# AshishKumar4/FlaxDiff

Measured on AMD Instinct MI355X. Metric: train images/sec/node (64x64 uncond EDM UNet, bs=256), higher is better.
Workload: dtype bf16; 1 GPU; model=unet_64px_[64,128,256,512]_res2_heads4, global_batch=256, resolution=64, parallelism=dp1, schedule=EDM + KarrasPredictionTransform(sigma_data=0.5)

## Files before the change

### flaxdiff_amd/models/common.py

```python
from __future__ import annotations

import math
from typing import Callable, Optional

import torch
import torch.nn as nn
import torch.nn.functional as F

from .. import ops


_TRUNC_STD_CORRECTION = 0.87962566103423978


def variance_scaling_(tensor: torch.Tensor, fan_in: int, fan_out: int,
                      scale: float = 1.0, mode: str = "fan_in") -> torch.Tensor:
    if mode == "fan_in":
        denom = max(1, fan_in)
    elif mode == "fan_out":
        denom = max(1, fan_out)
    else:
        denom = max(1.0, (fan_in + fan_out) / 2)
    std = math.sqrt(max(scale, 1e-10) / denom) / _TRUNC_STD_CORRECTION
    with torch.no_grad():
        tensor.normal_(0.0, std)
        tensor.clamp_(-2 * std, 2 * std)
    return tensor


class _ShadowCast(torch.autograd.Function):

    @staticmethod
    def forward(ctx, p):
        return p._shadow_bf16

    @staticmethod
    def backward(ctx, dy):
        return dy.float()


def _cast(p: Optional[torch.Tensor], dtype) -> Optional[torch.Tensor]:
    if p is None:
        return None
    if p.dtype == dtype:
        return p
    if dtype == torch.bfloat16 and getattr(p, "_shadow_bf16", None) is not None:
        return _ShadowCast.apply(p)
    return p.to(dtype)



class Dense(nn.Module):
    def __init__(self, in_features: int, out_features: int, use_bias: bool = True,
                 kernel_scale: float = 1.0, zero_init: bool = False):
        super().__init__()
        self.in_features = in_features
        self.out_features = out_features
        w = torch.empty(in_features, out_features)
        if zero_init:
            nn.init.zeros_(w)
        else:
            variance_scaling_(w, in_features, out_features, scale=kernel_scale)
        self.weight = nn.Parameter(w)
        self.bias = nn.Parameter(torch.zeros(out_features)) if use_bias else None

    def forward(self, x: torch.Tensor, add: torch.Tensor = None) -> torch.Tensor:
        if x.is_cuda and x.dtype == torch.bfloat16:
            return ops.dense(x, self.weight, self.bias, add=add)
        return ops.dense(x, _cast(self.weight, x.dtype),
                         _cast(self.bias, x.dtype), add=add)



class GroupNorm(nn.Module):

    def __init__(self, num_groups: int, num_channels: int, eps: float = 1e-5):
        super().__init__()
        assert num_channels % num_groups == 0, (num_groups, num_channels)
        self.num_groups = num_groups
        self.eps = eps
        self.weight = nn.Parameter(torch.ones(num_channels))
        self.bias = nn.Parameter(torch.zeros(num_channels))

    def forward(self, x: torch.Tensor, silu: bool = False) -> torch.Tensor:
        if x.is_cuda:
            return ops.group_norm(x, self.num_groups, self.weight, self.bias,
                                  self.eps, silu)
        return ops.group_norm(x, self.num_groups, _cast(self.weight, x.dtype),
                              _cast(self.bias, x.dtype), self.eps, silu)

    def forward_fork(self, x: torch.Tensor, silu: bool = False):
        if x.is_cuda:
            return ops.group_norm_fork(x, self.num_groups, self.weight,
                                       self.bias, self.eps, silu)
        return self.forward(x, silu), x


class RMSNorm(nn.Module):
    def __init__(self, dim: int, eps: float = 1e-5):
        super().__init__()
        self.eps = eps
        self.weight = nn.Parameter(torch.ones(dim))

    def forward(self, x: torch.Tensor) -> torch.Tensor:
        if x.is_cuda:
            return ops.rms_norm(x, self.weight, self.eps)
        return ops.rms_norm(x, _cast(self.weight, x.dtype), self.eps)



class TimeEmbedding(nn.Module):

    def __init__(self, features: int, max_positions: int = 10000):
        super().__init__()
        self.features = features
        self.max_positions = max_positions

    def forward(self, t: torch.Tensor) -> torch.Tensor:
        return ops.sinusoidal_time_embedding(t, self.features, self.max_positions)


class FourierEmbedding(nn.Module):

    def __init__(self, features: int, scale: float = 16.0):
        super().__init__()
        g = torch.Generator().manual_seed(42)
        freqs = torch.randn(features // 2, generator=g) * scale
        self.register_buffer("freqs", freqs, persistent=True)

    def forward(self, t: torch.Tensor) -> torch.Tensor:
        return ops.fourier_time_embedding(t, self.freqs)


class TimeProjection(nn.Module):

    def __init__(self, in_features: int, features: int):
        super().__init__()
        self.dense1 = Dense(in_features, features)
        self.dense2 = Dense(features, features)

    def forward(self, x: torch.Tensor) -> torch.Tensor:
        x = F.gelu(self.dense1(x))
        x = F.gelu(self.dense2(x))
        return x



class Conv(nn.Module):

    def __init__(self, in_features: int, features: int, kernel_size=(3, 3),
                 strides=(1, 1), use_bias: bool = True):
        super().__init__()
        kh, kw = kernel_size if isinstance(kernel_size, (tuple, list)) \
            else (kernel_size, kernel_size)
        self.stride = strides[0] if isinstance(strides, (tuple, list)) else strides
        w = torch.empty(kh, kw, in_features, features)
        variance_scaling_(w, kh * kw * in_features, kh * kw * features)
        self.weight = nn.Parameter(w)
        self.bias = nn.Parameter(torch.zeros(features)) if use_bias else None

    def forward(self, x: torch.Tensor, add: torch.Tensor = None,
                badd: torch.Tensor = None) -> torch.Tensor:
        if x.is_cuda and x.dtype == torch.bfloat16:
            return ops.conv2d(x, self.weight, self.bias, stride=self.stride,
                              add=add, badd=badd)
        return ops.conv2d(x, _cast(self.weight, x.dtype), _cast(self.bias, x.dtype),
                          stride=self.stride, add=add, badd=badd)


class ConvTranspose(nn.Module):
    def __init__(self, in_features: int, features: int, kernel_size=(3, 3), strides=(2, 2)):
        super().__init__()
        kh, kw = kernel_size
        self.stride = strides[0]
        w = torch.empty(kh, kw, in_features, features)
        variance_scaling_(w, kh * kw * in_features, kh * kw * features)
        self.weight = nn.Parameter(w)
        self.bias = nn.Parameter(torch.zeros(features))

    def forward(self, x):
        return ops.conv2d_transpose(x, _cast(self.weight, x.dtype),
                                    _cast(self.bias, x.dtype), stride=self.stride)


class SeparableConv(nn.Module):

    def __init__(self, in_features: int, features: int, kernel_size=(3, 3),
                 strides=(1, 1), use_bias: bool = False):
        super().__init__()
        kh, kw = kernel_size
        self.stride = strides[0] if isinstance(strides, (tuple, list)) else strides
        dw = torch.empty(kh, kw, in_features, 1)
        variance_scaling_(dw, kh * kw, kh * kw)
        self.depthwise = nn.Parameter(dw)
        pw = torch.empty(1, 1, in_features, features)
        variance_scaling_(pw, in_features, features)
        self.pointwise = nn.Parameter(pw)
        self.bias = nn.Parameter(torch.zeros(features)) if use_bias else None

    def forward(self, x):
        x = ops.depthwise_conv2d(x, _cast(self.depthwise, x.dtype), None, self.stride)
        return ops.conv2d(x, _cast(self.pointwise, x.dtype), _cast(self.bias, x.dtype), 1)


class WeightStandardizedConv(nn.Module):

    def __init__(self, in_features: int, features: int, kernel_size=(3, 3), strides=(1, 1)):
        super().__init__()
        kh, kw = kernel_size
        self.stride = strides[0] if isinstance(strides, (tuple, list)) else strides
        w = torch.empty(kh, kw, in_features, features)
        variance_scaling_(w, kh * kw * in_features, kh * kw * features)
        self.weight = nn.Parameter(w)
        self.bias = nn.Parameter(torch.zeros(features))

    def forward(self, x):
        w = self.weight
        eps = 1e-5 if x.dtype == torch.float32 else 1e-3
        mean = w.mean(dim=(0, 1, 2), keepdim=True)
        var = w.var(dim=(0, 1, 2), unbiased=False, keepdim=True)
        w = (w - mean) / torch.sqrt(var + eps)
        return ops.conv2d(x, _cast(w, x.dtype), _cast(self.bias, x.dtype), self.stride)


def ConvLayer(conv_type: str, in_features: int, features: int, kernel_size=(3, 3),
              strides=(1, 1)) -> nn.Module:
    if conv_type == "conv":
        return Conv(in_features, features, kernel_size, strides)
    if conv_type == "w_conv":
        return WeightStandardizedConv(in_features, features, kernel_size, strides)
    if conv_type == "separable":
        return SeparableConv(in_features, features, kernel_size, strides)
    if conv_type == "conv_transpose":
        return ConvTranspose(in_features, features, kernel_size, strides)
    raise ValueError(f"unknown conv_type {conv_type}")


class PixelShuffle(nn.Module):

    def __init__(self, scale: int):
        super().__init__()
        self.scale = scale

    def forward(self, x):
        B, H, W, C = x.shape
        s = self.scale
        c = C // (s * s)
        x = x.reshape(B, H, W, s, s, c)
        x = x.permute(0, 1, 3, 2, 4, 5)
        return x.reshape(B, H * s, W * s, c)


class Upsample(nn.Module):

    def __init__(self, in_features: int, features: int, scale: int = 2,
                 activation: Callable = F.silu):
        super().__init__()
        assert scale == 2
        self.conv = Conv(in_features, features, (3, 3), (1, 1))

    def forward(self, x, residual=None):
        if x.is_cuda and x.dtype == torch.bfloat16:
            out = ops.conv2d_upsample2x(x, self.conv.weight, self.conv.bias)
        else:
            out = self.conv(ops.nearest_upsample_2x(x))
        if residual is not None:
            out = ops.cat_channels(out, residual)
        return out


class Downsample(nn.Module):

    def __init__(self, in_features: int, features: int, scale: int = 2,
                 activation: Callable = F.silu):
        super().__init__()
        assert scale == 2
        self.conv = Conv(in_features, features, (3, 3), (2, 2))

    def forward(self, x, residual=None):
        out = self.conv(x)
        if residual is not None:
            if residual.shape[1] > out.shape[1]:
                residual = ops.avg_pool_2x(residual)
            out = ops.cat_channels(out, residual)
        return out



class ResidualBlock(nn.Module):

    def __init__(self, conv_type: str, in_features: int, features: int,
                 temb_features: int, kernel_size=(3, 3), strides=(1, 1),
                 activation: Callable = F.silu, norm_groups: int = 8,
                 norm_epsilon: float = 1e-4):
        super().__init__()
        self.features = features
        self.activation = activation
        self._fused_silu = activation in (F.silu, torch.nn.functional.silu)
        if norm_groups > 0:
            self.norm1 = GroupNorm(norm_groups, in_features, eps=norm_epsilon)
            self.norm2 = GroupNorm(norm_groups, features, eps=norm_epsilon)
        else:
            self.norm1 = RMSNorm(in_features, eps=norm_epsilon)
            self.norm2 = RMSNorm(features, eps=norm_epsilon)
        self.conv1 = ConvLayer(conv_type, in_features, features, kernel_size, strides)
        self.temb_projection = Dense(temb_features, features)
        self.conv2 = ConvLayer(conv_type, features, features, kernel_size, strides)
        self.residual_conv = (ConvLayer(conv_type, in_features, features, (1, 1), (1, 1))
                              if in_features != features else None)

    def _norm_act(self, norm, x):
        if isinstance(norm, GroupNorm) and self._fused_silu:
            return norm(x, silu=True)
        return self.activation(norm(x))

    def forward(self, x: torch.Tensor, temb: torch.Tensor,
                textemb: torch.Tensor = None, extra_features: torch.Tensor = None):
        if isinstance(self.norm1, GroupNorm):
            out, residual = self.norm1.forward_fork(x, silu=self._fused_silu)
            if not self._fused_silu:
                out = self.activation(out)
        else:
            residual = x
            out = self._norm_act(self.norm1, x)
        t = self.temb_projection(temb.to(out.dtype))
        if isinstance(self.conv1, Conv):
            out = self.conv1(out, badd=t)
        else:
            out = self.conv1(out) + t[:, None, None, :]

        out = self._norm_act(self.norm2, out)
        if self.residual_conv is not None:
            residual = self.residual_conv(residual)
        if isinstance(self.conv2, Conv) and residual.shape[-1] == self.features:
            out = self.conv2(out, add=residual)
        else:
            out = self.conv2(out) + residual

        if extra_features is not None:
            out = ops.cat_channels(out, extra_features)
        return out


def l2norm(t: torch.Tensor, dim=1, eps=1e-6):
    return t / torch.clamp(t.norm(p=2, dim=dim, keepdim=True), min=eps)
```

### flaxdiff_amd/models/unet.py

```python
from __future__ import annotations

from typing import Callable, List, Optional, Sequence

import torch
import torch.nn as nn
import torch.nn.functional as F

from .. import ops
from .attention import TransformerBlock
from .common import (ConvLayer, Downsample, FourierEmbedding, GroupNorm,
                     RMSNorm, ResidualBlock, TimeProjection, Upsample)


def _make_attention(dim: int, attention_config: dict, context_dim: int,
                    default_fp32_softmax: bool = False) -> TransformerBlock:
    heads = attention_config["heads"]
    return TransformerBlock(
        in_channels=dim,
        heads=heads,
        dim_head=dim // heads,
        use_projection=attention_config.get("use_projection", False),
        use_self_and_cross=attention_config.get("use_self_and_cross", True),
        only_pure_attention=attention_config.get("only_pure_attention", True),
        force_fp32_for_softmax=attention_config.get("force_fp32_for_softmax",
                                                    default_fp32_softmax),
        norm_inputs=attention_config.get("norm_inputs", True),
        explicitly_add_residual=attention_config.get("explicitly_add_residual", True),
        context_dim=context_dim,
    )


class Unet(nn.Module):
    def __init__(self,
                 output_channels: int = 3,
                 in_channels: int = 3,
                 emb_features: int = 64 * 4,
                 feature_depths: Sequence[int] = (64, 128, 256, 512),
                 attention_configs: Sequence[Optional[dict]] = ({"heads": 8},) * 4,
                 num_res_blocks: int = 2,
                 num_middle_res_blocks: int = 1,
                 activation: Callable = F.silu,
                 norm_groups: int = 8,
                 context_dim: int = 768,
                 conv_type: str = "conv"):
        super().__init__()
        self.output_channels = output_channels
        self.emb_features = emb_features
        self.feature_depths = list(feature_depths)
        self.attention_configs = list(attention_configs)
        self.num_res_blocks = num_res_blocks
        self.num_middle_res_blocks = num_middle_res_blocks
        self.activation = activation
        self.norm_groups = norm_groups

        self.time_embed = FourierEmbedding(features=emb_features)
        self.time_proj = TimeProjection(emb_features, emb_features)

        f0 = self.feature_depths[0]
        self.conv_in = ConvLayer(conv_type, in_channels, f0, (3, 3), (1, 1))

        def res_block(cin, cout):
            return ResidualBlock(conv_type, cin, cout, emb_features,
                                 kernel_size=(3, 3), strides=(1, 1),
                                 activation=activation, norm_groups=norm_groups)

        ch = f0
        skip_channels: List[int] = [f0]
        self.down_blocks = nn.ModuleList()
        for i, (dim_out, att_cfg) in enumerate(zip(self.feature_depths, self.attention_configs)):
            dim_in = ch
            level = nn.ModuleDict()
            res_list = nn.ModuleList()
            attn_list = nn.ModuleList()
            for j in range(num_res_blocks):
                res_list.append(res_block(dim_in, dim_in))
                if att_cfg is not None and j == num_res_blocks - 1:
                    attn_list.append(_make_attention(dim_in, att_cfg, context_dim))
                else:
                    attn_list.append(nn.Identity())
                skip_channels.append(dim_in)
            level["res"] = res_list
            level["attn"] = attn_list
            if i != len(self.feature_depths) - 1:
                level["down"] = Downsample(dim_in, dim_out, scale=2, activation=activation)
                ch = dim_out
            self.down_blocks.append(level)

        middle_dim = self.feature_depths[-1]
        middle_att = self.attention_configs[-1]
        self.middle_res1 = nn.ModuleList()
        self.middle_attn = nn.ModuleList()
        self.middle_res2 = nn.ModuleList()
        for j in range(num_middle_res_blocks):
            self.middle_res1.append(res_block(ch, middle_dim))
            ch = middle_dim
            if middle_att is not None and j == num_middle_res_blocks - 1:
                cfg = dict(middle_att)
                cfg.setdefault("use_self_and_cross", False)
                self.middle_attn.append(_make_attention(middle_dim, cfg, context_dim))
            else:
                self.middle_attn.append(nn.Identity())
            self.middle_res2.append(res_block(middle_dim, middle_dim))

        self.up_blocks = nn.ModuleList()
        rev_depths = list(reversed(self.feature_depths))
        rev_attn = list(reversed(self.attention_configs))
        skips = list(skip_channels)
        for i, (dim_out, att_cfg) in enumerate(zip(rev_depths, rev_attn)):
            level = nn.ModuleDict()
            res_list = nn.ModuleList()
            attn_list = nn.ModuleList()
            for j in range(num_res_blocks):
                skip_ch = skips.pop()
                res_list.append(res_block(ch + skip_ch, dim_out))
                ch = dim_out
                if att_cfg is not None and j == num_res_blocks - 1:
                    attn_list.append(_make_attention(dim_out, att_cfg, context_dim))
                else:
                    attn_list.append(nn.Identity())
            level["res"] = res_list
            level["attn"] = attn_list
            if i != len(self.feature_depths) - 1:
                up_features = self.feature_depths[-i] if i > 0 else self.feature_depths[0]
                level["up"] = Upsample(ch, up_features, scale=2, activation=activation)
                ch = up_features
            self.up_blocks.append(level)

        self.conv_mid = ConvLayer(conv_type, ch, f0, (3, 3), (1, 1))
        final_skip = skips.pop()
        assert not skips
        self.final_residual = res_block(f0 + final_skip, f0)
        if norm_groups > 0:
            self.conv_out_norm = GroupNorm(norm_groups, f0, eps=1e-5)
        else:
            self.conv_out_norm = RMSNorm(f0, eps=1e-5)
        self.conv_out = ConvLayer(conv_type, f0, output_channels, (3, 3), (1, 1))

    def forward(self, x: torch.Tensor, temb: torch.Tensor,
                textcontext: torch.Tensor) -> torch.Tensor:
        temb = self.time_embed(temb).to(x.dtype)
        temb = self.time_proj(temb)

        x = self.conv_in(x)
        downs = [x]

        for level in self.down_blocks:
            for res, attn in zip(level["res"], level["attn"]):
                x = res(x, temb)
                if not isinstance(attn, nn.Identity):
                    x = attn(x, textcontext)
                downs.append(x)
            if "down" in level:
                x = level["down"](x)

        for res1, attn, res2 in zip(self.middle_res1, self.middle_attn, self.middle_res2):
            x = res1(x, temb)
            if not isinstance(attn, nn.Identity):
                x = attn(x, textcontext)
            x = res2(x, temb)

        for level in self.up_blocks:
            for res, attn in zip(level["res"], level["attn"]):
                x = ops.cat_channels(x, downs.pop())
                x = res(x, temb)
                if not isinstance(attn, nn.Identity):
                    x = attn(x, textcontext)
            if "up" in level:
                x = level["up"](x)

        x = self.conv_mid(x)
        x = ops.cat_channels(x, downs.pop())
        x = self.final_residual(x, temb)

        if isinstance(self.conv_out_norm, GroupNorm):
            x = self.conv_out_norm(x, silu=True)
        else:
            x = self.activation(self.conv_out_norm(x))
        return self.conv_out(x)
```

### flaxdiff_amd/ops/__init__.py

```python
from __future__ import annotations

import os
import weakref
from typing import Optional

import torch

from . import reference

_EXT = None
_EXT_ERR: Optional[str] = None


def _load_ext():
    global _EXT, _EXT_ERR
    if _EXT is not None or _EXT_ERR is not None:
        return _EXT
    try:
        from .hip import build as hip_build
        _EXT = hip_build.load_extension()
    except Exception as e:
        _EXT_ERR = f"{type(e).__name__}: {e}"
        _EXT = None
    return _EXT


def hip_available() -> bool:
    return _load_ext() is not None


def _require_ext():
    ext = _load_ext()
    if ext is None:
        raise RuntimeError(
            "flaxdiff_amd HIP extension is not available on a GPU tensor path "
            f"(build error: {_EXT_ERR}). Run __graft_entry__.build() / "
            "python -m flaxdiff_amd.ops.hip.build first — the GPU path never "
            "silently falls back to stock torch ops.")
    return ext


_FORCE_TORCH = os.environ.get("FLAXDIFF_FORCE_TORCH_OPS", "0") == "1"
_GEMM_LIB = os.environ.get("FD_GEMM_LIB", "0") == "1"


def _use_hip(x: torch.Tensor) -> bool:
    return x.is_cuda and not _FORCE_TORCH



_GRAD_HOOK_OWNERS: "weakref.WeakSet" = weakref.WeakSet()


def register_grad_hook_owner(owner) -> None:
    _GRAD_HOOK_OWNERS.add(owner)


def _sink_kinds() -> str:
    v = os.environ.get("FD_GRAD_SINK", "1")
    if v == "0":
        return ""
    return "wbgr" if v == "all" else "bgr"


def grad_sinks_active() -> bool:
    if not _sink_kinds():
        return False
    return not any(o.hooks_live for o in _GRAD_HOOK_OWNERS)


def _grad_sink(p: Optional[torch.Tensor], kind: str) -> Optional[torch.Tensor]:
    if p is None or kind not in _sink_kinds():
        return None
    sink = getattr(p, "_grad_sink", None)
    if sink is None or sink.dtype != torch.float32 or not grad_sinks_active():
        return None
    owner = getattr(p, "_grad_sink_owner", None)
    g = (p if owner is None else owner).grad
    if g is None or g.data_ptr() != sink.data_ptr() \
            or g.numel() != sink.numel() or not sink.is_contiguous():
        return None
    return sink



def _gn_save(ctx, x, gamma, beta, mean, rstd, groups, silu):
    ctx.save_for_backward(x, gamma, mean, rstd)
    ctx.groups = groups
    ctx.silu = silu
    ctx.beta = beta
    ctx.gamma_param = gamma


def _gn_backward(ctx, dy, add):
    x, gamma, mean, rstd = ctx.saved_tensors
    ext = _require_ext()
    has_beta = ctx.beta is not None
    beta = ctx.beta if has_beta else torch.zeros_like(gamma)
    if has_beta and ctx.needs_input_grad[1] and ctx.needs_input_grad[2]:
        sg, sb = _grad_sink(ctx.gamma_param, "g"), _grad_sink(ctx.beta, "g")
        if sg is not None and sb is not None:
            (dx,) = ext.gn_silu_bwd(dy.contiguous(), x, gamma, beta, mean,
                                    rstd, ctx.groups, ctx.silu, sg, sb, add)
            return dx, None, None
    dx, dgamma, dbeta = ext.gn_silu_bwd(dy.contiguous(), x, gamma, beta, mean,
                                        rstd, ctx.groups, ctx.silu,
                                        None, None, add)
    return dx, dgamma, (dbeta if has_beta else None)


class _GroupNormSiLUFn(torch.autograd.Function):
    @staticmethod
    def forward(ctx, x, gamma, beta, groups, eps, silu):
        ext = _require_ext()
        y, mean, rstd = ext.gn_silu_fwd(x, gamma, beta, groups, eps, silu)
        _gn_save(ctx, x, gamma, beta, mean, rstd, groups, silu)
        return y

    @staticmethod
    def backward(ctx, dy):
        return (*_gn_backward(ctx, dy, None), None, None, None)


def group_norm(x: torch.Tensor, groups: int, gamma: torch.Tensor,
               beta: torch.Tensor, eps: float = 1e-5, silu: bool = False) -> torch.Tensor:
    if _use_hip(x):
        return _GroupNormSiLUFn.apply(x.contiguous(), gamma, beta, groups, eps, silu)
    return reference.group_norm_nhwc(x, groups, gamma, beta, eps, silu)


class _GroupNormForkFn(torch.autograd.Function):

    @staticmethod
    def forward(ctx, x, gamma, beta, groups, eps, silu):
        ext = _require_ext()
        ctx.set_materialize_grads(False)
        y, mean, rstd = ext.gn_silu_fwd(x, gamma, beta, groups, eps, silu)
        _gn_save(ctx, x, gamma, beta, mean, rstd, groups, silu)
        return y, x

    @staticmethod
    def backward(ctx, dy, dx_pass):
        if dy is None:
            return dx_pass, None, None, None, None, None
        add = None
        if dx_pass is not None:
            add = dx_pass.to(ctx.saved_tensors[0].dtype).contiguous()
        return (*_gn_backward(ctx, dy, add), None, None, None)


def group_norm_fork_enabled() -> bool:
    return os.environ.get("FD_GN_FORK_ADD", "1") != "0"


def group_norm_fork(x: torch.Tensor, groups: int, gamma: torch.Tensor,
                    beta: torch.Tensor, eps: float = 1e-5, silu: bool = False):
    if _use_hip(x) and beta is not None and group_norm_fork_enabled():
        return _GroupNormForkFn.apply(x.contiguous(), gamma, beta, groups, eps, silu)
    return group_norm(x, groups, gamma, beta, eps, silu), x



class _RMSNormFn(torch.autograd.Function):
    @staticmethod
    def forward(ctx, x, gamma, eps):
        ext = _require_ext()
        y, rrms = ext.rms_norm_fwd(x, gamma, eps)
        ctx.save_for_backward(x, gamma, rrms)
        ctx.gamma_param = gamma
        return y

    @staticmethod
    def backward(ctx, dy):
        x, gamma, rrms = ctx.saved_tensors
        ext = _require_ext()
        sink = _grad_sink(ctx.gamma_param, "r") if ctx.needs_input_grad[1] else None
        if sink is not None:
            (dx,) = ext.rms_norm_bwd(dy.contiguous(), x, gamma, rrms, sink)
            return dx, None, None
        dx, dgamma = ext.rms_norm_bwd(dy.contiguous(), x, gamma, rrms)
        return dx, dgamma, None


def rms_norm(x: torch.Tensor, gamma: torch.Tensor, eps: float = 1e-5) -> torch.Tensor:
    if _use_hip(x):
        return _RMSNormFn.apply(x.contiguous(), gamma, eps)
    return reference.rms_norm(x, gamma, eps)



def _kernel_view(p: torch.Tensor) -> torch.Tensor:
    if p.dtype == torch.bfloat16:
        return p
    sh = getattr(p, "_shadow_bf16", None)
    if sh is not None:
        return sh
    return p.to(torch.bfloat16)


def _kernel_view_t(p: torch.Tensor) -> torch.Tensor:
    t = getattr(p, "_shadow_bf16_t", None)
    if t is not None:
        return t
    return _kernel_view(p).t().contiguous()


def transpose_shadows(src_flat, dst_flat, tiles):
    _require_ext().transpose_shadows(src_flat, dst_flat, tiles)


def _routable_param(p: Optional[torch.Tensor]) -> bool:
    return p is None or p.dtype == torch.bfloat16 or \
        getattr(p, "_shadow_bf16", None) is not None


def _save_params(ctx, w, b):
    ctx.has_bias = b is not None
    ctx.w_dtype = w.dtype
    ctx.b_dtype = b.dtype if b is not None else None
    ctx.w_param, ctx.b_param = w, b


def _param_grads(ctx, ext, dy, x, kh, kw, stride):
    dw = db = None
    b_param = ctx.b_param if ctx.has_bias and ctx.needs_input_grad[2] \
        else None
    if ctx.needs_input_grad[1]:
        dw, db = _wgrad(ext, dy, x, kh, kw, stride,
                        ctx.w_param, ctx.w_dtype, b_param, ctx.b_dtype)
    elif ctx.has_bias:
        db = _bias_grad(dy, b_param, ctx.b_dtype)
    return dw, db


class _Conv2dFn(torch.autograd.Function):
    @staticmethod
    def forward(ctx, x, w, b, stride, add, badd):
        ext = _require_ext()
        wk = _kernel_view(w)
        y = ext.conv2d_fwd(x, wk, b if b is not None else torch.Tensor(),
                           stride,
                           add if add is not None else torch.Tensor(),
                           badd if badd is not None else torch.Tensor())
        ctx.save_for_backward(x, wk)
        ctx.stride = stride
        ctx.has_add = add is not None
        ctx.has_badd = badd is not None
        _save_params(ctx, w, b)
        return y

    @staticmethod
    def backward(ctx, dy):
        x, wk = ctx.saved_tensors
        ext = _require_ext()
        dy = dy.contiguous()
        dx = ext.conv2d_dgrad(dy, wk, ctx.stride, x.shape[1], x.shape[2]) \
            if ctx.needs_input_grad[0] else None
        dw, db = _param_grads(ctx, ext, dy, x, wk.shape[0], wk.shape[1],
                              ctx.stride)
        dadd = dy if ctx.has_add else None
        dbadd = None
        if ctx.has_badd:
            B = dy.shape[0]
            dbadd = dy.reshape(B, -1, dy.shape[-1]).sum(1)
        return dx, dw, db, None, dadd, dbadd


class _DenseFn(torch.autograd.Function):

    @staticmethod
    def forward(ctx, x2d, w2d, b, add):
        wk = _kernel_view(w2d)
        if not _GEMM_LIB and x2d.shape[1] % 64 == 0:
            ext = _require_ext()
            bf = b if b is not None else torch.Tensor()
            if bf.numel() and bf.dtype != torch.float32:
                bf = bf.float()
            y = ext.gemm_nt(x2d, _kernel_view_t(w2d), bf,
                            add if add is not None else torch.Tensor())
        else:
            y = torch.matmul(x2d, wk)
            if b is not None:
                y = y + _kernel_view(b)
            if add is not None:
                y = y + add
        ctx.save_for_backward(x2d, wk)
        ctx.has_add = add is not None
        _save_params(ctx, w2d, b)
        return y

    @staticmethod
    def backward(ctx, dy):
        x2d, wk = ctx.saved_tensors
        dy = dy.contiguous()
        ext = _require_ext()
        if ctx.needs_input_grad[0]:
            if not _GEMM_LIB and dy.shape[1] % 64 == 0:
                dx = ext.gemm_dx(dy, wk)
            else:
                dx = torch.matmul(dy, wk.t())
        else:
            dx = None
        M = x2d.shape[0]
        dw, db = _param_grads(ctx, ext, dy.view(M, 1, 1, dy.shape[1]),
                              x2d.view(M, 1, 1, x2d.shape[1]), 1, 1, 1)
        if dw is not None:
            dw = dw.view(x2d.shape[1], dy.shape[1])
        dadd = dy if ctx.has_add else None
        return dx, dw, db, dadd


def dense(x: torch.Tensor, w: torch.Tensor, b: Optional[torch.Tensor] = None,
          add: Optional[torch.Tensor] = None) -> torch.Tensor:
    if _use_hip(x) and x.dtype == torch.bfloat16 and _routable_param(w) \
            and _routable_param(b):
        lead = x.shape[:-1]
        add2 = None
        if add is not None and add.dtype == torch.bfloat16:
            add2 = add.reshape(-1, w.shape[1]).contiguous()
        y = _DenseFn.apply(x.reshape(-1, x.shape[-1]).contiguous(), w, b, add2)
        y = y.reshape(*lead, w.shape[1])
        if add is not None and add2 is None:
            y = y + add
        return y
    if w.dtype != x.dtype:
        w = w.to(x.dtype)
    y = torch.matmul(x, w)
    if b is not None:
        y = y + b.to(y.dtype)
    if add is not None:
        y = y + add.to(y.dtype)
    return y


class _WL2LossFn(torch.autograd.Function):

    @staticmethod
    def forward(ctx, pred, target, wb):
        ctx.save_for_backward(pred, target, wb)
        return _require_ext().wl2_loss_fwd(pred, target, wb)

    @staticmethod
    def backward(ctx, go):
        pred, target, wb = ctx.saved_tensors
        dpred = _require_ext().wl2_loss_bwd(pred, target, wb,
                                            go.reshape(1).float())
        return dpred, None, None


def weighted_l2_loss(pred: torch.Tensor, target: torch.Tensor,
                     weights: torch.Tensor) -> torch.Tensor:
    if _use_hip(pred) and pred.dtype == torch.bfloat16 \
            and target.dtype == torch.bfloat16:
        wb = weights.reshape(weights.shape[0]).float().contiguous()
        return _WL2LossFn.apply(pred.contiguous(), target.contiguous(), wb)
    return (0.5 * (pred.float() - target.float()) ** 2
            * weights.to(torch.float32)).mean()


class _ConvUp2xFn(torch.autograd.Function):

    @staticmethod
    def forward(ctx, x, w, b):
        ext = _require_ext()
        wk = _kernel_view(w)
        y = ext.conv2d_fwd_up2x(x, wk, b if b is not None else torch.Tensor())
        if y is None or y.numel() == 0:
            raise _ConvUpIneligibleError
        ctx.save_for_backward(x, wk)
        _save_params(ctx, w, b)
        return y

    @staticmethod
    def backward(ctx, dy):
        x, wk = ctx.saved_tensors
        ext = _require_ext()
        dy = dy.contiguous()
        H2, W2 = x.shape[1] * 2, x.shape[2] * 2
        dx = None
        if ctx.needs_input_grad[0]:
            dx_up = ext.conv2d_dgrad(dy, wk, 1, H2, W2)
            dx = ext.upsample2x_bwd(dx_up)
        x_up = ext.upsample2x_fwd(x) if ctx.needs_input_grad[1] else None
        dw, db = _param_grads(ctx, ext, dy, x_up, 3, 3, 1)
        return dx, dw, db


class _ConvUpIneligibleError(Exception):
    pass


def conv2d_upsample2x(x: torch.Tensor, w: torch.Tensor,
                      b: Optional[torch.Tensor] = None) -> torch.Tensor:
    if _use_hip(x) and x.dtype == torch.bfloat16 and _routable_param(w) \
            and w.shape[0] == 3 and w.shape[1] == 3:
        try:
            return _ConvUp2xFn.apply(
                x.contiguous(), w.contiguous(),
                b.contiguous() if b is not None else None)
        except _ConvUpIneligibleError:
            pass
    return conv2d(nearest_upsample_2x(x), w, b, stride=1)


class _GEGLUFn(torch.autograd.Function):

    @staticmethod
    def forward(ctx, h):
        ctx.save_for_backward(h)
        return _require_ext().geglu_fwd(h)

    @staticmethod
    def backward(ctx, dy):
        (h,) = ctx.saved_tensors
        return _require_ext().geglu_bwd(dy.contiguous(), h)


def geglu(h: torch.Tensor) -> torch.Tensor:
    if _use_hip(h) and h.dtype == torch.bfloat16 and h.shape[-1] % 16 == 0:
        return _GEGLUFn.apply(h.contiguous())
    a, b = h.chunk(2, dim=-1)
    return a * torch.nn.functional.gelu(b)


class _Cat2Fn(torch.autograd.Function):

    @staticmethod
    def forward(ctx, a, b):
        ctx.ca = a.shape[-1]
        ctx.cb = b.shape[-1]
        return _require_ext().cat2_lastdim(a, b)

    @staticmethod
    def backward(ctx, dy):
        da, db = _require_ext().split2_lastdim(dy.contiguous(), ctx.ca, ctx.cb)
        return da, db


def cat_channels(a: torch.Tensor, b: torch.Tensor) -> torch.Tensor:
    if _use_hip(a) and a.dtype == torch.bfloat16 and b.dtype == torch.bfloat16 \
            and (a.shape[-1] + b.shape[-1]) % 8 == 0:
        return _Cat2Fn.apply(a.contiguous(), b.contiguous())
    return torch.cat([a, b], dim=-1)


def _wgrad(ext, dy, x, kh, kw, stride, w_param, w_dtype,
           b_param=None, b_dtype=None):
    want_db = b_dtype is not None
    w_sink = _grad_sink(w_param, "w") if w_dtype == torch.float32 else None
    b_sink = _grad_sink(b_param, "b") if b_dtype == torch.float32 else None
    dw, db, folded = ext.conv2d_wgrad(dy, x, kh, kw, stride, w_sink,
                                      want_db, b_sink)
    if dw is not None and w_dtype != torch.float32:
        dw = dw.to(w_dtype)
    if want_db and not folded:
        db = _bias_grad(dy, b_param, b_dtype)
    elif db is not None and b_dtype != torch.float32:
        db = db.to(b_dtype)
    return dw, db


def _bias_grad(dy: torch.Tensor, b_param: Optional[torch.Tensor] = None,
               b_dtype=torch.float32) -> Optional[torch.Tensor]:
    d2 = dy.reshape(-1, dy.shape[-1])
    C = d2.shape[1]
    if d2.is_cuda and d2.dtype == torch.bfloat16 and C % 8 == 0 and C <= 2048:
        sink = _grad_sink(b_param, "b") if b_dtype == torch.float32 else None
        db = _require_ext().colsum(d2.contiguous(), sink)
        if sink is not None:
            return None
    else:
        db = d2.float().sum(0)
    return db if b_dtype == torch.float32 else db.to(b_dtype)


def conv2d(x: torch.Tensor, w: torch.Tensor, b: Optional[torch.Tensor] = None,
           stride: int = 1, add: Optional[torch.Tensor] = None,
           badd: Optional[torch.Tensor] = None) -> torch.Tensor:
    kh, kw = w.shape[0], w.shape[1]
    if kh == 1 and kw == 1 and stride == 1:
        w2 = w.reshape(w.shape[2], w.shape[3])
        sh = getattr(w, "_shadow_bf16", None)
        if sh is not None and w.dtype != torch.bfloat16:
            w2._shadow_bf16 = sh.reshape(w.shape[2], w.shape[3])
            sht = getattr(w, "_shadow_bf16_t", None)
            if sht is not None:
                w2._shadow_bf16_t = sht
            sink = getattr(w, "_grad_sink", None)
            if sink is not None:
                w2._grad_sink = sink.reshape(w.shape[2], w.shape[3])
                w2._grad_sink_owner = w
        y = dense(x.reshape(-1, w.shape[2]), w2, b)
        y = y.reshape(*x.shape[:-1], w.shape[3])
        if badd is not None:
            y = y + badd[:, None, None, :].to(y.dtype)
        return y if add is None else y + add
    if _use_hip(x) and x.dtype == torch.bfloat16 and _routable_param(w):
        if add is not None and add.dtype != torch.bfloat16:
            add_in, add_out = None, add
        else:
            add_in, add_out = add, None
        if badd is not None and badd.dtype != torch.bfloat16:
            badd_in, badd_out = None, badd
        else:
            badd_in, badd_out = badd, None
        out = _Conv2dFn.apply(
            x.contiguous(), w.contiguous(),
            b.contiguous() if b is not None else None, stride,
            add_in.contiguous() if add_in is not None else None,
            badd_in.contiguous() if badd_in is not None else None)
        if badd_out is not None:
            out = out + badd_out[:, None, None, :].to(out.dtype)
        if add_out is not None:
            out = out + add_out
        return out
    if w.dtype != x.dtype:
        w = w.to(x.dtype)
    if b is not None and b.dtype != x.dtype:
        b = b.to(x.dtype)
    y = reference.conv2d_nhwc(x, w, b, stride=stride, padding="same")
    if badd is not None:
        y = y + badd[:, None, None, :].to(y.dtype)
    return y if add is None else y + add


class _ConvTransposeFn(torch.autograd.Function):

    @staticmethod
    def forward(ctx, x, wf, stride):
        ext = _require_ext()
        H2 = x.shape[1] * stride
        W2 = x.shape[2] * stride
        y = ext.conv2d_dgrad(x, wf, stride, H2, W2)
        ctx.save_for_backward(x, wf)
        ctx.stride = stride
        return y

    @staticmethod
    def backward(ctx, dout):
        x, wf = ctx.saved_tensors
        ext = _require_ext()
        dout = dout.contiguous()
        dx = ext.conv2d_fwd(dout, wf, torch.Tensor(), ctx.stride,
                            torch.Tensor(), torch.Tensor()) \
            if ctx.needs_input_grad[0] else None
        dwf = None
        if ctx.needs_input_grad[1]:
            dwf = ext.conv2d_wgrad(x, dout, wf.shape[0], wf.shape[1],
                                   ctx.stride)[0].to(wf.dtype)
        return dx, dwf, None


def conv2d_transpose(x: torch.Tensor, w: torch.Tensor, b: Optional[torch.Tensor] = None,
                     stride: int = 2) -> torch.Tensor:
    kh, kw = w.shape[0], w.shape[1]
    if _use_hip(x) and stride == 2 and kh == 3 and kw == 3:
        wf = w.permute(0, 1, 3, 2).contiguous()
        out = _ConvTransposeFn.apply(x.contiguous(), wf, stride)
        if b is not None:
            out = out + b
        return out
    return reference.conv2d_transpose_nhwc(x, w, b, stride)


class _DepthwiseConvFn(torch.autograd.Function):

    @staticmethod
    def forward(ctx, x, w, stride, dilation):
        ext = _require_ext()
        y = ext.dwconv_fwd(x, w, None, stride, dilation)
        ctx.save_for_backward(x, w)
        ctx.stride = stride
        ctx.dilation = dilation
        return y

    @staticmethod
    def backward(ctx, dy):
        x, w = ctx.saved_tensors
        ext = _require_ext()
        dy = dy.contiguous()
        dx = ext.dwconv_dgrad(dy, w, x.shape[1], x.shape[2],
                              ctx.stride, ctx.dilation)
        dw = ext.dwconv_wgrad(dy, x, ctx.stride, ctx.dilation)
        return dx, dw.to(w.dtype), None, None


def depthwise_conv2d(x: torch.Tensor, w: torch.Tensor, b: Optional[torch.Tensor] = None,
                     stride: int = 1, dilation: int = 1) -> torch.Tensor:
    if (_use_hip(x) and x.dtype == torch.bfloat16 and b is None
            and w.shape[0] == 3 and w.shape[1] == 3 and x.shape[-1] % 8 == 0):
        w3 = w.reshape(3, 3, -1).contiguous()
        return _DepthwiseConvFn.apply(x, w3, stride, dilation)
    return reference.depthwise_conv2d_nhwc(x, w, b, stride, dilation)



def _attn_view_ok(t: torch.Tensor) -> bool:
    if t.dim() != 4:
        return False
    if t.is_contiguous():
        return True
    if t.stride(3) != 1 or t.data_ptr() % 16 or t.stride(2) >= 2 ** 31:
        return False
    return all(st > 0 and st % 8 == 0 for st in t.stride()[:3])


def _attn_strided(q: torch.Tensor, k: torch.Tensor) -> bool:
    if os.environ.get("FD_ATTN_STRIDED", "1") == "0":
        return False
    if os.environ.get("FD_ATTN_BWD_V1"):
        return False
    return k.shape[2] <= 128 and q.shape[3] <= 64


def _attn_operand(t: torch.Tensor, strided: bool) -> torch.Tensor:
    return t if strided and _attn_view_ok(t) else t.contiguous()


class _AttentionFn(torch.autograd.Function):
    @staticmethod
    def forward(ctx, q, k, v, scale):
        ext = _require_ext()
        o, lse = ext.attn_fwd(q, k, v, scale)
        ctx.save_for_backward(q, k, v, lse)
        ctx.scale = scale
        return o

    @staticmethod
    def backward(ctx, do):
        q, k, v, lse = ctx.saved_tensors
        scale = ctx.scale
        use_v1 = os.environ.get("FD_ATTN_BWD_V1")
        dmax = 32 if use_v1 else 64
        if k.shape[2] <= 128 and q.shape[3] <= dmax:
            ext = _require_ext()
            fn = ext.attn_bwd_smallkv if use_v1 else ext.attn_bwd_smallkv_v2
            do = _attn_operand(do, not use_v1 and _attn_strided(q, k))
            dq, dk, dv = fn(q, k, v, do, lse, scale)
            return dq, dk, dv, None
        qf, kf, vf, dof = q.float(), k.float(), v.float(), do.float()
        s = torch.einsum("bhqd,bhkd->bhqk", qf, kf) * scale
        p = torch.exp(s - lse.unsqueeze(-1))
        dv = torch.einsum("bhqk,bhqd->bhkd", p, dof)
        dp = torch.einsum("bhqd,bhkd->bhqk", dof, vf)
        dsum = (dp * p).sum(-1, keepdim=True)
        ds = (dp - dsum) * p * scale
        dq = torch.einsum("bhqk,bhkd->bhqd", ds, kf)
        dk = torch.einsum("bhqk,bhqd->bhkd", ds, qf)
        return dq.to(q.dtype), dk.to(k.dtype), dv.to(v.dtype), None


def attention(q: torch.Tensor, k: torch.Tensor, v: torch.Tensor,
              scale: Optional[float] = None) -> torch.Tensor:
    if scale is None:
        scale = q.shape[-1] ** -0.5
    if _use_hip(q):
        D = q.shape[-1]
        if D % 8 == 0 and D <= 128:
            strided = _attn_strided(q, k)
            return _AttentionFn.apply(_attn_operand(q, strided),
                                      _attn_operand(k, strided),
                                      _attn_operand(v, strided), scale)
    return reference.attention(q, k, v, scale)



def forward_diffusion(x0, eps, signal_rate, noise_rate):
    if _use_hip(x0):
        ext = _require_ext()
        return ext.fwd_diffusion(x0, eps, signal_rate.reshape(-1).float().contiguous(),
                                 noise_rate.reshape(-1).float().contiguous())
    return reference.forward_diffusion(x0, eps, signal_rate, noise_rate)


def nearest_upsample_2x(x: torch.Tensor) -> torch.Tensor:
    if _use_hip(x):
        return _Upsample2xFn.apply(x.contiguous())
    return reference.nearest_upsample_2x_nhwc(x)


class _Upsample2xFn(torch.autograd.Function):
    @staticmethod
    def forward(ctx, x):
        ext = _require_ext()
        return ext.upsample2x_fwd(x)

    @staticmethod
    def backward(ctx, dy):
        ext = _require_ext()
        return ext.upsample2x_bwd(dy.contiguous())


def avg_pool_2x(x: torch.Tensor) -> torch.Tensor:
    return reference.avg_pool_2x_nhwc(x)


def sinusoidal_time_embedding(t: torch.Tensor, features: int,
                              max_positions: int = 10000) -> torch.Tensor:
    if _use_hip(t):
        ext = _require_ext()
        return ext.time_embed(t, torch.Tensor(), features, float(max_positions))
    return reference.sinusoidal_time_embedding(t, features, max_positions)


def fourier_time_embedding(t: torch.Tensor, freqs: torch.Tensor) -> torch.Tensor:
    if _use_hip(t):
        ext = _require_ext()
        return ext.time_embed(t, freqs, freqs.numel() * 2, 0.0)
    return reference.fourier_time_embedding(t, freqs)



class _S5ScanFn(torch.autograd.Function):

    @staticmethod
    def forward(ctx, a_ri, bu_ri):
        ext = _require_ext()
        x = ext.s5_scan_fwd(a_ri.contiguous(), bu_ri.contiguous())
        ctx.save_for_backward(a_ri, x)
        return x

    @staticmethod
    def backward(ctx, dx):
        a_ri, x = ctx.saved_tensors
        ext = _require_ext()
        dbu, dap = ext.s5_scan_bwd(a_ri.contiguous(), x, dx.contiguous())
        return dap.sum(dim=0), dbu


def s5_scan(a: torch.Tensor, bu: torch.Tensor) -> torch.Tensor:
    if bu.is_cuda and not _FORCE_TORCH:
        a_ri = torch.view_as_real(a.contiguous()).float()
        bu_ri = torch.view_as_real(bu.contiguous()).float()
        x = _S5ScanFn.apply(a_ri, bu_ri)
        return torch.view_as_complex(x)
    from ..models.ssm_dit import associative_scan_diag
    return associative_scan_diag(a.reshape(1, 1, -1).expand_as(bu), bu)


def fused_adamw_ema(params_f32, grads, exp_avg, exp_avg_sq, ema_f32, params_bf16,
                    *, lr, beta1, beta2, eps, weight_decay, step, ema_decay,
                    grad_scale: float = 1.0, scale_dev=None, skip_ctr=None,
                    step_dev=None):
    ext = _require_ext()
    ext.fused_adamw_ema(params_f32, grads, exp_avg, exp_avg_sq, ema_f32,
                        params_bf16 if params_bf16 is not None else torch.Tensor(),
                        lr, beta1, beta2, eps, weight_decay, step, ema_decay,
                        grad_scale, scale_dev, skip_ctr, step_dev)
```

### flaxdiff_amd/ops/hip/bindings.cpp

```cpp
#include <torch/extension.h>
#include <tuple>
#include <vector>

std::vector<torch::Tensor> gn_silu_fwd(torch::Tensor x, torch::Tensor gamma,
                                       torch::Tensor beta, long groups,
                                       double eps, bool silu);
std::vector<torch::Tensor> gn_silu_bwd(torch::Tensor dy, torch::Tensor x,
                                       torch::Tensor gamma, torch::Tensor beta,
                                       torch::Tensor mean, torch::Tensor rstd,
                                       long groups, bool silu,
                                       c10::optional<torch::Tensor> dgamma_sink,
                                       c10::optional<torch::Tensor> dbeta_sink,
                                       c10::optional<torch::Tensor> add);
std::vector<torch::Tensor> rms_norm_fwd(torch::Tensor x, torch::Tensor gamma,
                                        double eps);
std::vector<torch::Tensor> rms_norm_bwd(torch::Tensor dy, torch::Tensor x,
                                        torch::Tensor gamma, torch::Tensor rrms,
                                        c10::optional<torch::Tensor> dgamma_sink);
torch::Tensor conv2d_fwd(torch::Tensor x, torch::Tensor w, torch::Tensor bias,
                         long stride, torch::Tensor add, torch::Tensor badd);
torch::Tensor conv2d_fwd_up2x(torch::Tensor x, torch::Tensor w,
                              torch::Tensor bias);
torch::Tensor conv2d_dgrad(torch::Tensor dy, torch::Tensor w, long stride,
                           long H, long W);
std::tuple<torch::Tensor, torch::Tensor, bool>
conv2d_wgrad(torch::Tensor dy, torch::Tensor x, long kh, long kw, long stride,
             c10::optional<torch::Tensor> dw_sink, bool want_db,
             c10::optional<torch::Tensor> db_sink);
torch::Tensor dwconv_fwd(torch::Tensor x, torch::Tensor w,
                         c10::optional<torch::Tensor> bias,
                         int64_t stride, int64_t dilation);
torch::Tensor dwconv_dgrad(torch::Tensor dy, torch::Tensor w,
                           int64_t H, int64_t W, int64_t stride, int64_t dilation);
torch::Tensor dwconv_wgrad(torch::Tensor dy, torch::Tensor x,
                           int64_t stride, int64_t dilation);
std::vector<torch::Tensor> attn_fwd(torch::Tensor q, torch::Tensor k,
                                    torch::Tensor v, double scale);
std::vector<torch::Tensor> attn_bwd_smallkv(torch::Tensor q, torch::Tensor k,
                                            torch::Tensor v, torch::Tensor dout,
                                            torch::Tensor lse, double scale);
std::vector<torch::Tensor> attn_bwd_smallkv_v2(torch::Tensor q, torch::Tensor k,
                                               torch::Tensor v, torch::Tensor dout,
                                               torch::Tensor lse, double scale);
torch::Tensor fwd_diffusion(torch::Tensor x0, torch::Tensor eps,
                            torch::Tensor a, torch::Tensor s);
torch::Tensor upsample2x_fwd(torch::Tensor x);
torch::Tensor time_embed(torch::Tensor t, torch::Tensor freqs, long features,
                         double max_positions);
torch::Tensor upsample2x_bwd(torch::Tensor dy);
torch::Tensor colsum(torch::Tensor x, c10::optional<torch::Tensor> sink);
torch::Tensor cat2_lastdim(torch::Tensor a, torch::Tensor b);
std::vector<torch::Tensor> split2_lastdim(torch::Tensor dy, long Ca, long Cb);
torch::Tensor geglu_fwd(torch::Tensor h);
torch::Tensor geglu_bwd(torch::Tensor dy, torch::Tensor h);
torch::Tensor wl2_loss_fwd(torch::Tensor pred, torch::Tensor target,
                           torch::Tensor wb);
torch::Tensor wl2_loss_bwd(torch::Tensor pred, torch::Tensor target,
                           torch::Tensor wb, torch::Tensor go);
torch::Tensor s5_scan_fwd(torch::Tensor a, torch::Tensor bu);
std::vector<torch::Tensor> s5_scan_bwd(torch::Tensor a, torch::Tensor x,
                                       torch::Tensor dx);
torch::Tensor gemm_fwd(torch::Tensor x, torch::Tensor w, torch::Tensor bias);
torch::Tensor gemm_dx(torch::Tensor dy, torch::Tensor w);
torch::Tensor gemm_nt(torch::Tensor x, torch::Tensor wt, torch::Tensor bias,
                      torch::Tensor add);
void transpose_shadows(torch::Tensor src_flat, torch::Tensor dst_flat,
                       torch::Tensor tiles);
void fused_adamw_ema(torch::Tensor p, torch::Tensor g, torch::Tensor m,
                     torch::Tensor v, torch::Tensor ema, torch::Tensor p_bf16,
                     double lr, double beta1, double beta2, double eps,
                     double weight_decay, long step, double ema_decay,
                     double grad_scale,
                     c10::optional<torch::Tensor> scale_dev,
                     c10::optional<torch::Tensor> skip_ctr,
                     c10::optional<torch::Tensor> step_dev);

PYBIND11_MODULE(TORCH_EXTENSION_NAME, m) {
    m.def("gn_silu_fwd", &gn_silu_fwd, "fused GroupNorm+SiLU forward (NHWC)");
    m.def("gn_silu_bwd", &gn_silu_bwd, "fused GroupNorm+SiLU backward",
          py::arg("dy"), py::arg("x"), py::arg("gamma"), py::arg("beta"),
          py::arg("mean"), py::arg("rstd"), py::arg("groups"), py::arg("silu"),
          py::arg("dgamma_sink") = py::none(), py::arg("dbeta_sink") = py::none(),
          py::arg("add") = py::none());
    m.def("rms_norm_fwd", &rms_norm_fwd, "RMSNorm forward");
    m.def("rms_norm_bwd", &rms_norm_bwd, "RMSNorm backward",
          py::arg("dy"), py::arg("x"), py::arg("gamma"), py::arg("rrms"),
          py::arg("dgamma_sink") = py::none());
    m.def("conv2d_fwd", &conv2d_fwd, "implicit-GEMM NHWC conv forward");
    m.def("conv2d_fwd_up2x", &conv2d_fwd_up2x, "fused nearest-2x upsample + conv forward");
    m.def("conv2d_dgrad", &conv2d_dgrad, "implicit-GEMM NHWC conv dgrad");
    m.def("conv2d_wgrad", &conv2d_wgrad,
          "split-M NHWC conv wgrad (+ folded bias grad): (dw, db, folded)",
          py::arg("dy"), py::arg("x"), py::arg("kh"), py::arg("kw"),
          py::arg("stride"), py::arg("dw_sink") = py::none(),
          py::arg("want_db") = false, py::arg("db_sink") = py::none());
    m.def("dwconv_fwd", &dwconv_fwd, "3x3 depthwise NHWC conv forward");
    m.def("dwconv_dgrad", &dwconv_dgrad, "3x3 depthwise NHWC conv dgrad");
    m.def("dwconv_wgrad", &dwconv_wgrad, "3x3 depthwise NHWC conv wgrad (fp32)");
    m.def("attn_fwd", &attn_fwd, "flash attention forward (bf16, fp32 softmax)");
    m.def("attn_bwd_smallkv", &attn_bwd_smallkv,
          "fused attention backward for Skv<=128, D<=32");
    m.def("attn_bwd_smallkv_v2", &attn_bwd_smallkv_v2,
          "vectorized-LDS attention backward for Skv<=128, D<=64");
    m.def("fwd_diffusion", &fwd_diffusion, "forward-diffusion axpy");
    m.def("upsample2x_fwd", &upsample2x_fwd, "nearest 2x upsample");
    m.def("time_embed", &time_embed, "fused sinusoidal/Fourier time embedding");
    m.def("upsample2x_bwd", &upsample2x_bwd, "nearest 2x upsample backward");
    m.def("colsum", &colsum, "coalesced column sum (bias grads)",
          py::arg("x"), py::arg("sink") = py::none());
    m.def("cat2_lastdim", &cat2_lastdim, "fused last-dim 2-tensor concat");
    m.def("split2_lastdim", &split2_lastdim, "one-pass last-dim split (cat backward)");
    m.def("geglu_fwd", &geglu_fwd, "fused GEGLU forward");
    m.def("geglu_bwd", &geglu_bwd, "fused GEGLU backward");
    m.def("wl2_loss_fwd", &wl2_loss_fwd, "fused weighted L2 loss forward");
    m.def("wl2_loss_bwd", &wl2_loss_bwd, "fused weighted L2 loss backward");
    m.def("s5_scan_fwd", &s5_scan_fwd, "S5 diagonal scan forward");
    m.def("s5_scan_bwd", &s5_scan_bwd, "S5 diagonal scan backward");
    m.def("gemm_fwd", &gemm_fwd, "MFMA bf16 GEMM y = x@w (+bias)");
    m.def("gemm_dx", &gemm_dx, "MFMA bf16 GEMM dx = dy@w^T");
    m.def("gemm_nt", &gemm_nt, "MFMA bf16 GEMM y = x@wt^T (+bias)");
    m.def("transpose_shadows", &transpose_shadows,
          "batched 64x64 bf16 transpose (dense-weight shadow refresh)");
    m.def("fused_adamw_ema", &fused_adamw_ema, "fused AdamW + EMA flat step");
}
```

### flaxdiff_amd/ops/hip/conv2d_wgrad.hip

```cpp
#include <torch/extension.h>
#include <ATen/hip/HIPContext.h>
#include "common.h"
#include "host_util.h"

typedef __bf16 bf16v8w __attribute__((ext_vector_type(8)));

#define WG_TC 64
#define WG_TM 64
#define WG_ROW (WG_TM + 8)
#define WG_NTH 256
#define WG_MAXKW 3

union WBF8 { bf16v8w v; ushort u[8]; uint4 q; };

__device__ __forceinline__ int wg_swz(int col, int rkey) {
    return (col & 7) | ((((col >> 3) ^ rkey) & 7) << 3);
}

template <int TKW, bool DB>
__global__ __launch_bounds__(WG_NTH, 2)
void conv2d_wgrad_kernel(const ushort* __restrict__ X,
                         const ushort* __restrict__ dY,
                         float* __restrict__ dB,
                         float* __restrict__ WS,
                         const int H, const int W,
                         const int OH, const int OW,
                         const int KH, const int KW,
                         const int Ci, const int Co,
                         const int stride, const int pt, const int pl,
                         const long M, const long m_per_block,
                         const int nci, const int nco,
                         const FastDiv fdOW, const FastDiv fdOH) {
    __shared__ __attribute__((aligned(16))) ushort lds[(DB ? 2 : 1) * (1 + WG_MAXKW) * WG_TC * WG_ROW];
    ushort* YT = lds;
    ushort* XT = lds + WG_TC * WG_ROW;

    const int ci0 = (blockIdx.x % nci) * WG_TC;
    const int co0 = (blockIdx.x / nci) * WG_TC;
    const int r = blockIdx.y;
    const long m_lo = (long)blockIdx.z * m_per_block;
    const long m_hi = min(m_lo + m_per_block, M);

    const int tid = threadIdx.x;
    const int lane = tid & 63;
    const int wid = tid >> 6;
    const int wi = wid >> 1;
    const int wj = wid & 1;
    const int l31 = lane & 31;
    const int half = lane >> 5;

    f32x16 acc[TKW] = {};

    const bool do_bias = (dB != nullptr) && (r == 0) && (ci0 == 0);
    float db8[8] = {};

    if (DB && TKW == 3 && stride == 1) {
        constexpr int NREP = (WG_TM * WG_TC) / (WG_NTH * 8);
        WBF8 rY[NREP], rC[NREP], rE0, rE2;
        int owv[NREP];
        int e2mloc = -1;
        bool mv[NREP], e0v = false, e2v = false;

        auto load_tile = [&](long m0) {
            #pragma unroll
            for (int rep = 0; rep < NREP; ++rep) {
                const int lin = tid + rep * WG_NTH;
                const int mloc = lin >> 3;
                const int cov = (lin & 7) * 8;
                const int civ = cov;
                WBF8 vy; vy.q = make_uint4(0, 0, 0, 0);
                const long m = m0 + mloc;
                if (m < m_hi && co0 + cov < Co) {
                    const long srcY = m * Co + co0 + cov;
                    if (co0 + cov + 8 <= Co)
                        vy.q = *reinterpret_cast<const uint4*>(dY + srcY);
                    else
                        for (int j = 0; j < 8 && co0 + cov + j < Co; ++j)
                            vy.u[j] = dY[srcY + j];
                }
                rY[rep] = vy;
                WBF8 vc; vc.q = make_uint4(0, 0, 0, 0);
                int ow = 0;
                bool ih_ok = false;
                long rowbase = 0;
                if (m < m_hi) {
                    const unsigned mu = (unsigned)m;
                    const unsigned q1 = fd_div(mu, fdOW);
                    ow = (int)fd_mod(mu, q1, fdOW);
                    const unsigned q2 = fd_div(q1, fdOH);
                    const int oh = (int)fd_mod(q1, q2, fdOH);
                    const long b = (long)q2;
                    const int ih = oh + r - pt;
                    ih_ok = ih >= 0 && ih < H && ci0 + civ < Ci;
                    rowbase = ((b * H + ih) * (long)W) * Ci + ci0 + civ;
                    if (ih_ok) {
                        const long srcX = rowbase + (long)ow * Ci;
                        if (ci0 + civ + 8 <= Ci)
                            vc.q = *reinterpret_cast<const uint4*>(X + srcX);
                        else
                            for (int j = 0; j < 8 && ci0 + civ + j < Ci; ++j)
                                vc.u[j] = X[srcX + j];
                    }
                }
                rC[rep] = vc;
                owv[rep] = ow;
                mv[rep] = m < m_hi;
                if (rep == 0 && mloc == 0) {
                    e0v = mv[0] && ow >= 1;
                    rE0.q = make_uint4(0, 0, 0, 0);
                    if (e0v && ih_ok) {
                        const long srcX = rowbase + (long)(ow - 1) * Ci;
                        if (ci0 + civ + 8 <= Ci)
                            rE0.q = *reinterpret_cast<const uint4*>(X + srcX);
                        else
                            for (int j = 0; j < 8 && ci0 + civ + j < Ci; ++j)
                                rE0.u[j] = X[srcX + j];
                    }
                }
                const bool is_edge2 = (m == m_hi - 1) ||
                                      (mloc == WG_TM - 1 && m < m_hi);
                if (is_edge2) {
                    e2mloc = mloc;
                    e2v = ow + 1 < W;
                    rE2.q = make_uint4(0, 0, 0, 0);
                    if (e2v && ih_ok) {
                        const long srcX = rowbase + (long)(ow + 1) * Ci;
                        if (ci0 + civ + 8 <= Ci)
                            rE2.q = *reinterpret_cast<const uint4*>(X + srcX);
                        else
                            for (int j = 0; j < 8 && ci0 + civ + j < Ci; ++j)
                                rE2.u[j] = X[srcX + j];
                    }
                }
            }
        };

        auto store_tile = [&](ushort* YTb, ushort* XTb, long m0) {
            #pragma unroll
            for (int rep = 0; rep < NREP; ++rep) {
                const int lin = tid + rep * WG_NTH;
                const int mloc = lin >> 3;
                const int cov = (lin & 7) * 8;
                const int civ = cov;
                const int key = lin & 7;
                const int sm = wg_swz(mloc, key);
                #pragma unroll
                for (int j = 0; j < 8; ++j)
                    YTb[(cov + j) * WG_ROW + sm] = rY[rep].u[j];
                ushort* xt0 = XTb;
                ushort* xt1 = XTb + WG_TC * WG_ROW;
                ushort* xt2 = XTb + 2 * WG_TC * WG_ROW;
                const int ow = owv[rep];
                #pragma unroll
                for (int j = 0; j < 8; ++j)
                    xt1[(civ + j) * WG_ROW + sm] = rC[rep].u[j];
                if (mloc + 1 < WG_TM && ow + 1 < W) {
                    const int smp = wg_swz(mloc + 1, key);
                    #pragma unroll
                    for (int j = 0; j < 8; ++j)
                        xt0[(civ + j) * WG_ROW + smp] = rC[rep].u[j];
                }
                if (ow == 0) {
                    #pragma unroll
                    for (int j = 0; j < 8; ++j)
                        xt0[(civ + j) * WG_ROW + sm] = 0;
                }
                if (ow == W - 1) {
                    #pragma unroll
                    for (int j = 0; j < 8; ++j)
                        xt2[(civ + j) * WG_ROW + sm] = 0;
                }
                if (mloc >= 1 && ow >= 1) {
                    const int smm = wg_swz(mloc - 1, key);
                    #pragma unroll
                    for (int j = 0; j < 8; ++j)
                        xt2[(civ + j) * WG_ROW + smm] = rC[rep].u[j];
                }
                if (mloc == 0 && e0v) {
                    #pragma unroll
                    for (int j = 0; j < 8; ++j)
                        xt0[(civ + j) * WG_ROW + (key << 3)] = rE0.u[j];
                }
                if (mloc == e2mloc && e2v) {
                    #pragma unroll
                    for (int j = 0; j < 8; ++j)
                        xt2[(civ + j) * WG_ROW + sm] = rE2.u[j];
                }
            }
        };

        auto mfma_tile = [&](const ushort* YTb, const ushort* XTb) {
            const int keyY = (wj * 32 + l31) >> 3;
            const int keyX = (wi * 32 + l31) >> 3;
            #pragma unroll
            for (int kk = 0; kk < WG_TM / 16; ++kk) {
                const int k0 = kk * 16 + half * 8;
                bf16v8w b = reinterpret_cast<const WBF8*>(
                    YTb + (wj * 32 + l31) * WG_ROW + wg_swz(k0, keyY))->v;
                #pragma unroll
                for (int s = 0; s < TKW; ++s) {
                    bf16v8w a = reinterpret_cast<const WBF8*>(
                        XTb + s * WG_TC * WG_ROW + (wi * 32 + l31) * WG_ROW
                        + wg_swz(k0, keyX))->v;
                    acc[s] = __builtin_amdgcn_mfma_f32_32x32x16_bf16(a, b, acc[s], 0, 0, 0);
                }
            }
        };

        const int BUFSZ = (1 + WG_MAXKW) * WG_TC * WG_ROW;
        int buf = 0;
        long m0 = m_lo;
        if (m0 < m_hi) load_tile(m0);
        while (m0 < m_hi) {
            ushort* base = lds + buf * BUFSZ;
            store_tile(base, base + WG_TC * WG_ROW, m0);
            __syncthreads();
            const long m_next = m0 + WG_TM;
            e2mloc = -1; e2v = false; e0v = false;
            if (m_next < m_hi) load_tile(m_next);
            mfma_tile(base, base + WG_TC * WG_ROW);
            buf ^= 1;
            m0 = m_next;
        }
    } else {
    for (long m0 = m_lo; m0 < m_hi; m0 += WG_TM) {
        __syncthreads();
        #pragma unroll
        for (int rep = 0; rep < (WG_TM * WG_TC) / (WG_NTH * 8); ++rep) {
            const int lin = tid + rep * WG_NTH;
            const int mloc = lin >> 3;
            const int cov = (lin & 7) * 8;
            WBF8 val; val.q = make_uint4(0, 0, 0, 0);
            const long m = m0 + mloc;
            if (m < m_hi && co0 + cov < Co) {
                const long src = m * Co + co0 + cov;
                if (co0 + cov + 8 <= Co) {
                    val.q = *reinterpret_cast<const uint4*>(dY + src);
                } else {
                    for (int j = 0; j < 8 && co0 + cov + j < Co; ++j)
                        val.u[j] = dY[src + j];
                }
            }
            if (do_bias) {
                #pragma unroll
                for (int j = 0; j < 8; ++j)
                    db8[j] += bf2f(val.u[j]);
            }
            const int sm = wg_swz(mloc, lin & 7);
            #pragma unroll
            for (int j = 0; j < 8; ++j)
                YT[(cov + j) * WG_ROW + sm] = val.u[j];
        }
        if (TKW == 3 && stride == 1) {
            #pragma unroll
            for (int rep = 0; rep < (WG_TM * WG_TC) / (WG_NTH * 8); ++rep) {
                const int lin = tid + rep * WG_NTH;
                const int mloc = lin >> 3;
                const int civ = (lin & 7) * 8;
                WBF8 val; val.q = make_uint4(0, 0, 0, 0);
                WBF8 zero; zero.q = make_uint4(0, 0, 0, 0);
                const long m = m0 + mloc;
                int ow = 0;
                bool ih_ok = false;
                long rowbase = 0;
                if (m < m_hi) {
                    const unsigned mu = (unsigned)m;
                    const unsigned q1 = fd_div(mu, fdOW);
                    ow = (int)fd_mod(mu, q1, fdOW);
                    const unsigned q2 = fd_div(q1, fdOH);
                    const int oh = (int)fd_mod(q1, q2, fdOH);
                    const long b = (long)q2;
                    const int ih = oh + r - pt;
                    ih_ok = ih >= 0 && ih < H && ci0 + civ < Ci;
                    rowbase = ((b * H + ih) * (long)W) * Ci + ci0 + civ;
                    if (ih_ok) {
                        const long src = rowbase + (long)ow * Ci;
                        if (ci0 + civ + 8 <= Ci) {
                            val.q = *reinterpret_cast<const uint4*>(X + src);
                        } else {
                            for (int j = 0; j < 8 && ci0 + civ + j < Ci; ++j)
                                val.u[j] = X[src + j];
                        }
                    }
                }
                ushort* xt0 = XT;
                ushort* xt1 = XT + WG_TC * WG_ROW;
                ushort* xt2 = XT + 2 * WG_TC * WG_ROW;
                const int key = lin & 7;
                const int sm = wg_swz(mloc, key);
                #pragma unroll
                for (int j = 0; j < 8; ++j)
                    xt1[(civ + j) * WG_ROW + sm] = val.u[j];
                if (mloc + 1 < WG_TM && ow + 1 < W) {
                    const int smp = wg_swz(mloc + 1, key);
                    #pragma unroll
                    for (int j = 0; j < 8; ++j)
                        xt0[(civ + j) * WG_ROW + smp] = val.u[j];
                }
                if (ow == 0) {
                    #pragma unroll
                    for (int j = 0; j < 8; ++j)
                        xt0[(civ + j) * WG_ROW + sm] = 0;
                }
                if (ow == W - 1) {
                    #pragma unroll
                    for (int j = 0; j < 8; ++j)
                        xt2[(civ + j) * WG_ROW + sm] = 0;
                }
                if (mloc >= 1 && ow >= 1) {
                    const int smm = wg_swz(mloc - 1, key);
                    #pragma unroll
                    for (int j = 0; j < 8; ++j)
                        xt2[(civ + j) * WG_ROW + smm] = val.u[j];
                }
                if (mloc == 0 && m < m_hi && ow >= 1) {
                    WBF8 v2 = zero;
                    if (ih_ok) {
                        const long src = rowbase + (long)(ow - 1) * Ci;
                        if (ci0 + civ + 8 <= Ci)
                            v2.q = *reinterpret_cast<const uint4*>(X + src);
                        else
                            for (int j = 0; j < 8 && ci0 + civ + j < Ci; ++j)
                                v2.u[j] = X[src + j];
                    }
                    #pragma unroll
                    for (int j = 0; j < 8; ++j)
                        xt0[(civ + j) * WG_ROW + (key << 3)] = v2.u[j];
                }
                if ((mloc == WG_TM - 1 || m == m_hi - 1) && m < m_hi && ow + 1 < W) {
                    WBF8 v2 = zero;
                    if (ih_ok) {
                        const long src = rowbase + (long)(ow + 1) * Ci;
                        if (ci0 + civ + 8 <= Ci)
                            v2.q = *reinterpret_cast<const uint4*>(X + src);
                        else
                            for (int j = 0; j < 8 && ci0 + civ + j < Ci; ++j)
                                v2.u[j] = X[src + j];
                    }
                    #pragma unroll
                    for (int j = 0; j < 8; ++j)
                        xt2[(civ + j) * WG_ROW + sm] = v2.u[j];
                }
            }
        } else {
        #pragma unroll
        for (int s = 0; s < TKW; ++s) {
            ushort* xt = XT + s * WG_TC * WG_ROW;
            #pragma unroll
            for (int rep = 0; rep < (WG_TM * WG_TC) / (WG_NTH * 8); ++rep) {
                const int lin = tid + rep * WG_NTH;
                const int mloc = lin >> 3;
                const int civ = (lin & 7) * 8;
                WBF8 val; val.q = make_uint4(0, 0, 0, 0);
                const long m = m0 + mloc;
                if (m < m_hi) {
                    const unsigned mu = (unsigned)m;
                    const unsigned q1 = fd_div(mu, fdOW);
                    const int ow = (int)fd_mod(mu, q1, fdOW);
                    const unsigned q2 = fd_div(q1, fdOH);
                    const int oh = (int)fd_mod(q1, q2, fdOH);
                    const long b = (long)q2;
                    const int ih = oh * stride + r - pt;
                    const int iw = ow * stride + s - pl;
                    if (ih >= 0 && ih < H && iw >= 0 && iw < W && ci0 + civ < Ci) {
                        const long src = ((b * H + ih) * (long)W + iw) * Ci + ci0 + civ;
                        if (ci0 + civ + 8 <= Ci) {
                            val.q = *reinterpret_cast<const uint4*>(X + src);
                        } else {
                            for (int j = 0; j < 8 && ci0 + civ + j < Ci; ++j)
                                val.u[j] = X[src + j];
                        }
                    }
                }
                const int sm = wg_swz(mloc, lin & 7);
                #pragma unroll
                for (int j = 0; j < 8; ++j)
                    xt[(civ + j) * WG_ROW + sm] = val.u[j];
            }
        }
        }
        __syncthreads();

        const int keyY = (wj * 32 + l31) >> 3;
        const int keyX = (wi * 32 + l31) >> 3;
        #pragma unroll
        for (int kk = 0; kk < WG_TM / 16; ++kk) {
            const int k0 = kk * 16 + half * 8;
            bf16v8w b = reinterpret_cast<const WBF8*>(
                YT + (wj * 32 + l31) * WG_ROW + wg_swz(k0, keyY))->v;
            #pragma unroll
            for (int s = 0; s < TKW; ++s) {
                bf16v8w a = reinterpret_cast<const WBF8*>(
                    XT + s * WG_TC * WG_ROW + (wi * 32 + l31) * WG_ROW
                    + wg_swz(k0, keyX))->v;
                acc[s] = __builtin_amdgcn_mfma_f32_32x32x16_bf16(a, b, acc[s], 0, 0, 0);
            }
        }
    }

    }

    if (do_bias) {
        const int cov = co0 + (tid & 7) * 8;
        #pragma unroll
        for (int j = 0; j < 8; ++j)
            if (cov + j < Co && db8[j] != 0.f)
                atomicAdd(dB + cov + j, db8[j]);
    }

    const long tileC = (long)nci * WG_TC * nco * WG_TC;
    const int co = wj * 32 + l31;
    #pragma unroll
    for (int s = 0; s < TKW; ++s) {
        float* slot = WS + ((long)blockIdx.z * KH * KW + r * KW + s) * tileC
                    + (long)(ci0) * (nco * WG_TC) + co0 + co;
        #pragma unroll
        for (int reg = 0; reg < 16; ++reg) {
            const int ci = wi * 32 + (reg & 3) + 8 * (reg >> 2) + 4 * half;
            slot[(long)ci * (nco * WG_TC)] = acc[s][reg];
        }
    }
}

#define WRED_ZCHUNK 32

__global__ void wgrad_reduce_kernel(const float* __restrict__ WS,
                                    float* __restrict__ dW,
                                    const int Z, const int taps,
                                    const int Ci, const int Co,
                                    const int nci, const int nco,
                                    const bool accum_w,
                                    const float* __restrict__ WSB,
                                    float* __restrict__ dB,
                                    const bool accum_b) {
    const int padCo = nco * WG_TC;
    const long tileC = (long)nci * WG_TC * padCo;
    const long total = (long)taps * Ci * Co;
    const long items = total + (WSB != nullptr ? Co : 0);
    const int nzc = (Z + WRED_ZCHUNK - 1) / WRED_ZCHUNK;
    const long work = items * nzc;
    for (long w = (long)blockIdx.x * blockDim.x + threadIdx.x; w < work;
         w += (long)gridDim.x * blockDim.x) {
        const long i = w % items;
        const int zc = (int)(w / items);
        const int z0 = zc * WRED_ZCHUNK;
        const int z1 = min(Z, z0 + WRED_ZCHUNK);
        float v = 0.f;
        if (i < total) {
            const int co = (int)(i % Co);
            const int ci = (int)((i / Co) % Ci);
            const int t = (int)(i / ((long)Ci * Co));
            const long src = (long)t * tileC + (long)ci * padCo + co;
            for (int z = z0; z < z1; ++z)
                v += WS[(long)z * taps * tileC + src];
            if (nzc == 1)
                dW[i] = accum_w ? dW[i] + v : v;
            else
                atomicAdd(dW + i, v);
        } else {
            const int co = (int)(i - total);
            for (int z = z0; z < z1; ++z)
                v += WSB[(long)z * padCo + co];
            if (nzc == 1)
                dB[co] = accum_b ? dB[co] + v : v;
            else
                atomicAdd(dB + co, v);
        }
    }
}

typedef long Tr16Plan(int B, int H, int W, int Ci, int Co, int nci, int nco);
typedef void Tr16Launch(const void* x, const void* dy, float* ws, float* wsb,
                        int B, int H, int W, int Ci, int Co, int nci, int nco,
                        long Z, hipStream_t stream);
Tr16Plan dense_wgrad_v3_plan, conv2d_wgrad_w8_plan, conv2d_wgrad_v3_plan;
Tr16Launch dense_wgrad_v3_launch, conv2d_wgrad_w8_launch, conv2d_wgrad_v3_launch;

#define WG_FOLD_V3 1
#define WG_FOLD_DENSE 2
#define WG_FOLD_W8 4
#define WG_FOLD_DEFAULT (WG_FOLD_V3 | WG_FOLD_DENSE | WG_FOLD_W8)
static bool wgrad_fold_enabled(int family) {
    static const int mask = [] {
        const char* e = std::getenv("FD_WGRAD_BIAS_FOLD");
        return e ? atoi(e) : WG_FOLD_DEFAULT;
    }();
    return (mask & family) != 0;
}

struct WgradWs {
    torch::Tensor buf;
    float* ws;
    float* wsb;
};
static WgradWs wgrad_alloc_ws(const torch::Tensor& x, long Z, int taps,
                              int nci, int nco, bool fold) {
    const long main = Z * taps * (long)nci * WG_TC * nco * WG_TC;
    WgradWs w;
    w.buf = torch::empty({main + (fold ? Z * (long)nco * WG_TC : 0L)},
                         x.options().dtype(at::kFloat));
    w.ws = w.buf.data_ptr<float>();
    w.wsb = fold ? w.ws + main : nullptr;
    return w;
}

static std::tuple<torch::Tensor, torch::Tensor, bool>
wgrad_reduce_into(const WgradWs& w, long Z, int KH, int KW, int Ci, int Co,
                  int nci, int nco,
                  const c10::optional<torch::Tensor>& dw_sink,
                  const c10::optional<torch::Tensor>& db_sink,
                  hipStream_t stream) {
    const int taps = KH * KW;
    const long nzc = (Z + WRED_ZCHUNK - 1) / WRED_ZCHUNK;
    const bool fold = w.wsb != nullptr;
    auto opt = w.buf.options();
    auto fresh = [&](at::IntArrayRef shape) {
        return nzc == 1 ? torch::empty(shape, opt) : torch::zeros(shape, opt);
    };
    torch::Tensor dw, db;
    float* dwp;
    float* dbp = nullptr;
    if (fd_has(dw_sink)) {
        dwp = dw_sink->data_ptr<float>();
    } else {
        dw = fresh({KH, KW, Ci, Co});
        dwp = dw.data_ptr<float>();
    }
    if (fold && fd_has(db_sink)) {
        dbp = db_sink->data_ptr<float>();
    } else if (fold) {
        db = fresh({Co});
        dbp = db.data_ptr<float>();
    }
    const long total = ((long)taps * Ci * Co + (fold ? Co : 0)) * nzc;
    const int blocks = (int)std::min<long>((total + 255) / 256, 8192);
    hipLaunchKernelGGL(wgrad_reduce_kernel, dim3(blocks), dim3(256), 0, stream,
                       w.ws, dwp, (int)Z, taps, Ci, Co, nci, nco,
                       fd_has(dw_sink), w.wsb, dbp, fold && fd_has(db_sink));
    FD_CHECK_LAUNCH();
    return {dw, db, fold};
}

std::tuple<torch::Tensor, torch::Tensor, bool>
conv2d_wgrad(torch::Tensor dy, torch::Tensor x,
             long kh_, long kw_, long stride_,
             c10::optional<torch::Tensor> dw_sink, bool want_db,
             c10::optional<torch::Tensor> db_sink) {
    FD_FLUSH_STALE();
    TORCH_CHECK(x.is_cuda() && x.is_contiguous() && dy.is_contiguous());
    TORCH_CHECK(x.scalar_type() == at::kBFloat16 && dy.scalar_type() == at::kBFloat16);
    const int B = x.size(0), H = x.size(1), W = x.size(2), Ci = x.size(3);
    const int OH = dy.size(1), OW = dy.size(2), Co = dy.size(3);
    const int KH = (int)kh_, KW = (int)kw_;
    TORCH_CHECK(KW <= WG_MAXKW, "conv2d_wgrad supports KW<=3, got ", KW);
    const int stride = (int)stride_;
    fd_check_sink(dw_sink, (long)KH * KW * Ci * Co, x, "conv2d_wgrad: dw");
    fd_check_sink(db_sink, Co, x, "conv2d_wgrad: db");
    TORCH_CHECK(want_db || !fd_has(db_sink),
                "conv2d_wgrad: db sink given without want_db");

    const int nci = (Ci + WG_TC - 1) / WG_TC;
    const int nco = (Co + WG_TC - 1) / WG_TC;
    const int taps = KH * KW;
    auto stream = at::hip::getCurrentHIPStream();

    static const bool use_v3 = std::getenv("FD_WGRAD_NO_V3") == nullptr;
    const bool same = OH == H && OW == W;
    const bool k1 = KH == 1 && KW == 1 && same;
    const bool k3same = KH == 3 && KW == 3 && same;
    const struct { bool shape_ok; int fold_bit; Tr16Plan* plan; Tr16Launch* launch; }
    families[] = {
        {k1, WG_FOLD_DENSE, dense_wgrad_v3_plan, dense_wgrad_v3_launch},
        {k3same, WG_FOLD_W8, conv2d_wgrad_w8_plan, conv2d_wgrad_w8_launch},
        {k3same, WG_FOLD_V3, conv2d_wgrad_v3_plan, conv2d_wgrad_v3_launch},
    };
    for (const auto& f : families) {
        if (!(use_v3 && stride == 1 && f.shape_ok)) continue;
        const long Z = f.plan(B, H, W, Ci, Co, nci, nco);
        if (Z == 0) continue;
        auto w = wgrad_alloc_ws(x, Z, taps, nci, nco,
                                want_db && wgrad_fold_enabled(f.fold_bit));
        f.launch(x.data_ptr(), dy.data_ptr(), w.ws, w.wsb,
                 B, H, W, Ci, Co, nci, nco, Z, stream);
        return wgrad_reduce_into(w, Z, KH, KW, Ci, Co, nci, nco,
                                 dw_sink, db_sink, stream);
    }

    const int pt = std::max((OH - 1) * stride + KH - H, 0) / 2;
    const int pl = std::max((OW - 1) * stride + KW - W, 0) / 2;
    const long M = (long)B * OH * OW;

    long splitm = std::max<long>(1, 1024 / std::max(1, nci * nco * KH));
    splitm = std::min(splitm, (M + WG_TM - 1) / WG_TM);
    long m_per_block = (M + splitm - 1) / splitm;
    m_per_block = ((m_per_block + WG_TM - 1) / WG_TM) * WG_TM;
    splitm = (M + m_per_block - 1) / m_per_block;

    auto w = wgrad_alloc_ws(x, splitm, taps, nci, nco, false);
    float* db_ptr = nullptr;

    dim3 grid(nci * nco, KH, (unsigned)splitm);
    TORCH_CHECK(M < (1ll << 31), "M must fit in 32 bits");
    auto launch = [&](auto kern) {
        hipLaunchKernelGGL(kern, grid, dim3(WG_NTH), 0, stream,
                           (const ushort*)x.data_ptr(), (const ushort*)dy.data_ptr(),
                           db_ptr, w.ws,
                           H, W, OH, OW, KH, KW, Ci, Co,
                           stride, pt, pl, M, m_per_block, nci, nco,
                           make_fastdiv(OW), make_fastdiv(OH));
    };
    static const bool use_db = std::getenv("FD_WGRAD_NO_DB") == nullptr;
    if (KW == 3 && stride == 1 && use_db) launch(conv2d_wgrad_kernel<3, true>);
    else if (KW == 3) launch(conv2d_wgrad_kernel<3, false>);
    else if (KW == 2) launch(conv2d_wgrad_kernel<2, false>);
    else launch(conv2d_wgrad_kernel<1, false>);
    FD_CHECK_LAUNCH();

    return wgrad_reduce_into(w, splitm, KH, KW, Ci, Co, nci, nco,
                             dw_sink, db_sink, stream);
}
```

### flaxdiff_amd/ops/hip/conv2d_wgrad_v3.hip

```cpp
#include <torch/extension.h>
#include <ATen/hip/HIPContext.h>
#include "common.h"
#include "host_util.h"

typedef __bf16 bf16v8g __attribute__((ext_vector_type(8)));
typedef __attribute__((__vector_size__(4 * sizeof(__bf16)))) __bf16 bf16x4g;

#define WGV3_NTH 256

union GFRAG { bf16v8g v8; bf16x4g v4[2]; };

__device__ __forceinline__ bf16x4g wgv3_tr(const ushort* p) {
    return __builtin_amdgcn_ds_read_tr16_b64_v4bf16(
        (__attribute__((address_space(3))) bf16x4g*)p);
}

__device__ __forceinline__ void wgv3_glds16(const ushort* src, ushort* dst) {
    __builtin_amdgcn_global_load_lds(
        (const __attribute__((address_space(1))) void*)src,
        (__attribute__((address_space(3))) void*)dst, 16, 0, 0);
}

__device__ __forceinline__ void wgv3_glds4(const ushort* src, ushort* dst) {
    __builtin_amdgcn_global_load_lds(
        (const __attribute__((address_space(1))) void*)src,
        (__attribute__((address_space(3))) void*)dst, 4, 0, 0);
}

__device__ __forceinline__ bf16v8g wgv3_ones() {
    bf16v8g o;
    #pragma unroll
    for (int j = 0; j < 8; ++j) o[j] = (__bf16)1.0f;
    return o;
}

static __host__ __device__ constexpr int wgv3_npos(int n) {
    return n + ((12 - (n & 7)) & 7);
}

template <int W, int RPT, int LOOK, bool BIAS>
__global__ __launch_bounds__(WGV3_NTH, 2)
void conv2d_wgrad_v3_kernel(
        const ushort* __restrict__ X,
        const ushort* __restrict__ dY,
        float* __restrict__ WS,
        float* __restrict__ WSB,
        const int H,
        const int Ci, const int Co,
        const int nci, const int nco,
        const long BH,
        const long rows_per_block) {
    constexpr int MT = RPT * W;
    constexpr int NPOS_X = wgv3_npos(W + 2);
    constexpr int NPOS_Y = wgv3_npos(MT);
    constexpr int PS_X = NPOS_X * 16;
    constexpr int PS_Y = NPOS_Y * 16;
    constexpr int SLAB = 4 * PS_X;
    constexpr int YTILE = 4 * PS_Y;
    constexpr int RING = RPT * (LOOK + 1) + 2;
    constexpr int DBUF = LOOK + 1;
    constexpr int G_X = (W >= 32) ? (W / 32) : 2;
    constexpr int G_Y = MT / 32;
    constexpr int NG = RPT * G_X + G_Y;
    constexpr int KQ = W / 16;

    extern __shared__ __attribute__((aligned(16))) ushort ldsv3[];
    ushort* Xr = ldsv3;
    ushort* Yr = ldsv3 + RING * SLAB;

    const int tid = threadIdx.x;
    const int lane = tid & 63;
    const int wid = tid >> 6;
    const int wi = wid >> 1;
    const int wj = wid & 1;
    const int ci0 = (blockIdx.x % nci) * 64;
    const int co0 = (blockIdx.x / nci) * 64;

    const long row_lo = (long)blockIdx.z * rows_per_block;
    const long row_hi = (row_lo + rows_per_block < BH) ? row_lo + rows_per_block : BH;
    const int ntiles = (int)((row_hi - row_lo) / RPT);

    for (int i = tid; i < RING * 4 * 2 * 16; i += WGV3_NTH) {
        const int c = i & 15;
        const int e = (i >> 4) & 1;
        const int p = (i >> 5) & 3;
        const int sl = i >> 7;
        Xr[sl * SLAB + p * PS_X + (e ? (W + 1) : 0) * 16 + c] = 0;
    }
    __syncthreads();

    auto issue_slab = [&](long g) {
        const long gc = g < 0 ? 0 : (g >= BH ? BH - 1 : g);
        ushort* dst0 = Xr + (int)(gc % RING) * SLAB + wid * PS_X + 16;
        const ushort* src0 = X + (gc * W) * (long)Ci + ci0 + wid * 16;
        if (W >= 32) {
            #pragma unroll
            for (int c = 0; c < G_X; ++c) {
                const ushort* s = src0 + (long)(c * 32 + (lane >> 1)) * Ci
                                + (lane & 1) * 8;
                wgv3_glds16(s, dst0 + c * 32 * 16);
            }
        } else {
            #pragma unroll
            for (int c = 0; c < 2; ++c) {
                const ushort* s = src0 + (long)(c * 8 + (lane >> 3)) * Ci
                                + (lane & 7) * 2;
                wgv3_glds4(s, dst0 + c * 8 * 16);
            }
        }
    };
    auto issue_ytile = [&](int t) {
        const int tc = t >= ntiles ? ntiles - 1 : t;
        ushort* dst0 = Yr + (tc % DBUF) * YTILE + wid * PS_Y;
        const ushort* src0 = dY + (row_lo + (long)tc * RPT) * W * (long)Co
                           + co0 + wid * 16;
        #pragma unroll
        for (int c = 0; c < G_Y; ++c) {
            const ushort* s = src0 + (long)(c * 32 + (lane >> 1)) * Co
                            + (lane & 1) * 8;
            wgv3_glds16(s, dst0 + c * 32 * 16);
        }
    };

    {
        const long b0 = row_lo;
        for (int i = 0; i < RPT + 2; ++i) issue_slab(b0 - 1 + i);
        issue_ytile(0);
        #pragma unroll
        for (int l = 1; l < LOOK; ++l) {
            #pragma unroll
            for (int k = 0; k < RPT; ++k)
                issue_slab(b0 - 1 + (RPT + 2) + (long)(l - 1) * RPT + k);
            issue_ytile(l);
        }
    }

    const int ltrX = ((lane >> 4) & 1) * PS_X + ((lane >> 5) << 3) * 16
                   + (lane & 15) * 4;
    const int ltrY = ((lane >> 4) & 1) * PS_Y + ((lane >> 5) << 3) * 16
                   + (lane & 15) * 4;
    const int abase_w = wi * 2 * PS_X + ltrX;
    const int bbase_w = wj * 2 * PS_Y + ltrY;

    f32x16 acc[9] = {};
    const bool do_bias = BIAS && ci0 == 0 && wi == 0;
    f32x16 accb = {};
    const bf16v8g ones = wgv3_ones();

    for (int t = 0; t < ntiles; ++t) {
        asm volatile("s_waitcnt vmcnt(%0)" :: "i"((LOOK - 1) * NG) : "memory");
        __builtin_amdgcn_s_barrier();

        {
            const long bL = row_lo + (long)(t + LOOK) * RPT;
            #pragma unroll
            for (int k = 0; k < RPT; ++k) issue_slab(bL + 1 + k);
            issue_ytile(t + LOOK);
        }

        const long base = row_lo + (long)t * RPT;
        const int oh0 = (int)(base % H);
        const int ybuf = (t % DBUF) * YTILE;

        #pragma unroll
        for (int rr = 0; rr < RPT; ++rr) {
            const int oh = oh0 + rr;
            const long g = base + rr;
            const int slot_m = (int)((g - 1 + RING) % RING) * SLAB;
            const int slot_c = (int)(g % RING) * SLAB;
            const int slot_p = (int)((g + 1) % RING) * SLAB;
            const bool r0ok = oh > 0;
            const bool r2ok = oh < H - 1;
            #pragma unroll
            for (int kq = 0; kq < KQ; ++kq) {
                GFRAG b;
                {
                    const ushort* bp = Yr + ybuf + bbase_w
                                     + (rr * W + kq * 16) * 16;
                    b.v4[0] = wgv3_tr(bp);
                    b.v4[1] = wgv3_tr(bp + 64);
                }
                if (BIAS && do_bias)
                    accb = __builtin_amdgcn_mfma_f32_32x32x16_bf16(
                        ones, b.v8, accb, 0, 0, 0);
                #pragma unroll
                for (int r = 0; r < 3; ++r) {
                    if (r == 0 && !r0ok) continue;
                    if (r == 2 && !r2ok) continue;
                    const int slot = (r == 0) ? slot_m
                                  : (r == 1) ? slot_c : slot_p;
                    #pragma unroll
                    for (int s = 0; s < 3; ++s) {
                        GFRAG a;
                        const ushort* ap = Xr + slot + abase_w
                                         + (kq * 16 + s) * 16;
                        a.v4[0] = wgv3_tr(ap);
                        a.v4[1] = wgv3_tr(ap + 64);
                        acc[r * 3 + s] = __builtin_amdgcn_mfma_f32_32x32x16_bf16(
                            a.v8, b.v8, acc[r * 3 + s], 0, 0, 0);
                    }
                }
            }
        }
    }
    asm volatile("s_waitcnt vmcnt(0)" ::: "memory");

    const long tileC = (long)nci * 64 * nco * 64;
    const int l31 = lane & 31;
    const int half = lane >> 5;
    const int co = wj * 32 + l31;
    #pragma unroll
    for (int tap = 0; tap < 9; ++tap) {
        float* slot = WS + ((long)blockIdx.z * 9 + tap) * tileC
                    + (long)ci0 * (nco * 64) + co0 + co;
        #pragma unroll
        for (int reg = 0; reg < 16; ++reg) {
            const int ci = wi * 32 + (reg & 3) + 8 * (reg >> 2) + 4 * half;
            slot[(long)ci * (nco * 64)] = acc[tap][reg];
        }
    }
    if (BIAS && do_bias && half == 0)
        WSB[(long)blockIdx.z * (nco * 64) + co0 + co] = accb[0];
}

template <int W, int RPT, int LOOK>
static size_t wgv3_smem() {
    constexpr int MT = RPT * W;
    constexpr int RING = RPT * (LOOK + 1) + 2;
    constexpr int DBUF = LOOK + 1;
    return (size_t)(RING * 4 * wgv3_npos(W + 2) * 16
                  + DBUF * 4 * wgv3_npos(MT) * 16) * sizeof(ushort);
}

static int wgv3_rpt(int W) {
    switch (W) {
        case 16: return 4;
        case 32: return 2;
        case 64: return 1;
        case 128: return 1;
        default: return 0;
    }
}


template <auto KernNoBias, auto KernBias, typename... Args>
static void wgv3_launch_fold(bool fold, dim3 grid, size_t smem,
                             hipStream_t stream, Args... args) {
    if (fold)
        fd_launch_lds<KernBias>(grid, dim3(WGV3_NTH), smem, stream, args...);
    else
        fd_launch_lds<KernNoBias>(grid, dim3(WGV3_NTH), smem, stream, args...);
    FD_CHECK_LAUNCH();
}

static long wgv3_split(long target, int nci, int nco, long ntiles) {
    long splitm = std::max<long>(1, target / std::max(1, nci * nco));
    splitm = std::min(splitm, ntiles);
    const long tiles_per_block = (ntiles + splitm - 1) / splitm;
    return (ntiles + tiles_per_block - 1) / tiles_per_block;
}

long conv2d_wgrad_v3_plan(int B, int H, int W, int Ci, int Co,
                          int nci, int nco) {
    if (Ci % 64 || Co % 64) return 0;
    const int rpt = wgv3_rpt(W);
    if (!rpt) return 0;
    if (H % rpt || ((long)B * H) % rpt) return 0;
    static const long target = [] {
        const char* e = std::getenv("FD_WGRAD_SPLIT");
        return e ? atol(e) : 512L;
    }();
    return wgv3_split(target, nci, nco, (long)B * H / rpt);
}

void conv2d_wgrad_v3_launch(const void* x, const void* dy, float* ws,
                            float* wsb, int B, int H, int W, int Ci, int Co,
                            int nci, int nco, long splitm, hipStream_t stream) {
    FD_FLUSH_STALE();
    const int rpt = wgv3_rpt(W);
    const long BH = (long)B * H;
    const long ntiles = BH / rpt;
    const long tiles_per_block = (ntiles + splitm - 1) / splitm;
    const long rows_per_block = tiles_per_block * rpt;
    dim3 grid((unsigned)(nci * nco), 1, (unsigned)splitm);
    #define WGV3_CASE(W_, RPT_, LOOK_)                                        \
        case W_:                                                              \
            wgv3_launch_fold<conv2d_wgrad_v3_kernel<W_, RPT_, LOOK_, false>,  \
                             conv2d_wgrad_v3_kernel<W_, RPT_, LOOK_, true>>(  \
                wsb != nullptr, grid, wgv3_smem<W_, RPT_, LOOK_>(), stream,   \
                (const ushort*)x, (const ushort*)dy, ws, wsb,                 \
                H, Ci, Co, nci, nco, BH, rows_per_block);                     \
            break
    switch (W) {
        WGV3_CASE(16, 4, 2);
        WGV3_CASE(32, 2, 2);
        WGV3_CASE(64, 1, 2);
        WGV3_CASE(128, 1, 1);
    }
    #undef WGV3_CASE
}


template <int LOOK, bool BIAS>
__global__ __launch_bounds__(WGV3_NTH, 2)
void dense_wgrad_v3_kernel(
        const ushort* __restrict__ X,
        const ushort* __restrict__ dY,
        float* __restrict__ WS,
        float* __restrict__ WSB,
        const int Ci, const int Co,
        const int nci, const int nco,
        const long M, const long m_per_block) {
    constexpr int MT = 64;
    constexpr int NPOS = wgv3_npos(MT);
    constexpr int PS = NPOS * 16;
    constexpr int TILE = 4 * PS;
    constexpr int DBUF = LOOK + 2;
    constexpr int NG = 4;

    extern __shared__ __attribute__((aligned(16))) ushort dlds[];
    ushort* Xr = dlds;
    ushort* Yr = dlds + DBUF * TILE;

    const int tid = threadIdx.x;
    const int lane = tid & 63;
    const int wid = tid >> 6;
    const int wi = wid >> 1;
    const int wj = wid & 1;
    const int ci0 = (blockIdx.x % nci) * 64;
    const int co0 = (blockIdx.x / nci) * 64;

    const long m_lo = (long)blockIdx.z * m_per_block;
    const long m_hi = (m_lo + m_per_block < M) ? m_lo + m_per_block : M;
    const int ntiles = (int)((m_hi - m_lo) / MT);

    auto issue = [&](int t) {
        const int tc = t >= ntiles ? ntiles - 1 : t;
        const long mb = m_lo + (long)tc * MT;
        ushort* dx0 = Xr + (tc % DBUF) * TILE + wid * PS;
        ushort* dy0 = Yr + (tc % DBUF) * TILE + wid * PS;
        const ushort* sx = X + mb * Ci + ci0 + wid * 16;
        const ushort* sy = dY + mb * Co + co0 + wid * 16;
        #pragma unroll
        for (int c = 0; c < 2; ++c) {
            wgv3_glds16(sx + (long)(c * 32 + (lane >> 1)) * Ci + (lane & 1) * 8,
                        dx0 + c * 32 * 16);
            wgv3_glds16(sy + (long)(c * 32 + (lane >> 1)) * Co + (lane & 1) * 8,
                        dy0 + c * 32 * 16);
        }
    };

    #pragma unroll
    for (int l = 0; l < LOOK; ++l) issue(l);

    const int ltr = ((lane >> 4) & 1) * PS + ((lane >> 5) << 3) * 16
                  + (lane & 15) * 4;
    const int abase = wi * 2 * PS + ltr;
    const int bbase = wj * 2 * PS + ltr;

    f32x16 acc = {};
    const bool do_bias = BIAS && ci0 == 0 && wi == 0;
    f32x16 accb = {};
    const bf16v8g ones = wgv3_ones();
    for (int t = 0; t < ntiles; ++t) {
        asm volatile("s_waitcnt vmcnt(%0)" :: "i"((LOOK - 1) * NG) : "memory");
        __builtin_amdgcn_s_barrier();
        issue(t + LOOK);
        const int xb = (t % DBUF) * TILE;
        const int yb = xb;
        #pragma unroll
        for (int kq = 0; kq < MT / 16; ++kq) {
            GFRAG a, b;
            const ushort* ap = Xr + xb + abase + kq * 16 * 16;
            const ushort* bp = Yr + yb + bbase + kq * 16 * 16;
            a.v4[0] = wgv3_tr(ap);
            a.v4[1] = wgv3_tr(ap + 64);
            b.v4[0] = wgv3_tr(bp);
            b.v4[1] = wgv3_tr(bp + 64);
            acc = __builtin_amdgcn_mfma_f32_32x32x16_bf16(a.v8, b.v8, acc, 0, 0, 0);
            if (BIAS && do_bias)
                accb = __builtin_amdgcn_mfma_f32_32x32x16_bf16(
                    ones, b.v8, accb, 0, 0, 0);
        }
    }
    asm volatile("s_waitcnt vmcnt(0)" ::: "memory");

    const long tileC = (long)nci * 64 * nco * 64;
    const int l31 = lane & 31;
    const int half = lane >> 5;
    const int co = wj * 32 + l31;
    float* slot = WS + (long)blockIdx.z * tileC
                + (long)ci0 * (nco * 64) + co0 + co;
    #pragma unroll
    for (int reg = 0; reg < 16; ++reg) {
        const int ci = wi * 32 + (reg & 3) + 8 * (reg >> 2) + 4 * half;
        slot[(long)ci * (nco * 64)] = acc[reg];
    }
    if (BIAS && do_bias && half == 0)
        WSB[(long)blockIdx.z * (nco * 64) + co0 + co] = accb[0];
}

long dense_wgrad_v3_plan(int B, int H, int W, int Ci, int Co, int nci, int nco) {
    const long M = (long)B * H * W;
    if (Ci % 64 || Co % 64 || M % 64) return 0;
    return wgv3_split(1024, nci, nco, M / 64);
}

void dense_wgrad_v3_launch(const void* x, const void* dy, float* ws,
                           float* wsb, int B, int H, int W, int Ci, int Co,
                           int nci, int nco, long splitm, hipStream_t stream) {
    FD_FLUSH_STALE();
    constexpr int LOOK = 2;
    const long M = (long)B * H * W;
    const long ntiles = M / 64;
    const long tiles_per_block = (ntiles + splitm - 1) / splitm;
    const long m_per_block = tiles_per_block * 64;
    constexpr size_t smem = (size_t)2 * (LOOK + 2) * 4 * wgv3_npos(64) * 16
                          * sizeof(ushort);
    dim3 grid((unsigned)(nci * nco), 1, (unsigned)splitm);
    wgv3_launch_fold<dense_wgrad_v3_kernel<LOOK, false>,
                     dense_wgrad_v3_kernel<LOOK, true>>(
        wsb != nullptr, grid, smem, stream, (const ushort*)x,
        (const ushort*)dy, ws, wsb, Ci, Co, nci, nco, M, m_per_block);
}


#define W8_KPOS 112
#define W8_GUARD 12
#define W8_NPX 140
#define W8_NPY 116

template <int LOOK, bool BIAS>
__global__ __launch_bounds__(WGV3_NTH, 2)
void conv2d_wgrad_w8_kernel(
        const ushort* __restrict__ X,
        const ushort* __restrict__ dY,
        float* __restrict__ WS,
        float* __restrict__ WSB,
        const int Ci, const int Co,
        const int nci, const int nco,
        const long NIMG, const long imgs_per_block) {
    constexpr int PS_X = W8_NPX * 16;
    constexpr int PS_Y = W8_NPY * 16;
    constexpr int XTILE = 4 * PS_X;
    constexpr int YTILE = 4 * PS_Y;
    constexpr int DBUF = LOOK + 1;
    constexpr int NG = 16;

    extern __shared__ __attribute__((aligned(16))) ushort w8lds[];
    ushort* Xr = w8lds;
    ushort* Yr = w8lds + DBUF * XTILE;

    const int tid = threadIdx.x;
    const int lane = tid & 63;
    const int wid = tid >> 6;
    const int wi = wid >> 1;
    const int wj = wid & 1;
    const int ci0 = (blockIdx.x % nci) * 64;
    const int co0 = (blockIdx.x / nci) * 64;

    const long img_lo = (long)blockIdx.z * imgs_per_block;
    const long img_hi = (img_lo + imgs_per_block < NIMG)
                      ? img_lo + imgs_per_block : NIMG;
    const int ntiles = (int)(img_hi - img_lo);

    for (int i = tid; i < DBUF * (XTILE + YTILE); i += WGV3_NTH)
        w8lds[i] = 0;
    __syncthreads();

    auto issue = [&](int t) {
        const int tc = t >= ntiles ? ntiles - 1 : t;
        const long img = img_lo + tc;
        ushort* dx0 = Xr + (tc % DBUF) * XTILE + wid * PS_X;
        ushort* dy0 = Yr + (tc % DBUF) * YTILE + wid * PS_Y;
        const ushort* sx = X + img * 64 * (long)Ci + ci0 + wid * 16;
        const ushort* sy = dY + img * 64 * (long)Co + co0 + wid * 16;
        #pragma unroll
        for (int r = 0; r < 8; ++r) {
            const int pos = (r + 1) * 10 + 1;
            const ushort* sxr = sx + (long)(r * 8 + (lane >> 3)) * Ci
                              + (lane & 7) * 2;
            const ushort* syr = sy + (long)(r * 8 + (lane >> 3)) * Co
                              + (lane & 7) * 2;
            wgv3_glds4(sxr, dx0 + (W8_GUARD + pos) * 16);
            wgv3_glds4(syr, dy0 + pos * 16);
        }
    };

    #pragma unroll
    for (int l = 0; l < LOOK; ++l) issue(l);

    const int ltrX = ((lane >> 4) & 1) * PS_X + ((lane >> 5) << 3) * 16
                   + (lane & 15) * 4;
    const int ltrY = ((lane >> 4) & 1) * PS_Y + ((lane >> 5) << 3) * 16
                   + (lane & 15) * 4;
    const int abase_w = wi * 2 * PS_X + ltrX + W8_GUARD * 16;
    const int bbase_w = wj * 2 * PS_Y + ltrY;

    f32x16 acc[9] = {};
    const bool do_bias = BIAS && ci0 == 0 && wi == 0;
    f32x16 accb = {};
    const bf16v8g ones = wgv3_ones();
    for (int t = 0; t < ntiles; ++t) {
        asm volatile("s_waitcnt vmcnt(%0)" :: "i"((LOOK - 1) * NG) : "memory");
        __builtin_amdgcn_s_barrier();
        issue(t + LOOK);
        const int xb = (t % DBUF) * XTILE;
        const int yb = (t % DBUF) * YTILE;
        #pragma unroll
        for (int kq = 0; kq < W8_KPOS / 16; ++kq) {
            GFRAG b;
            const ushort* bp = Yr + yb + bbase_w + kq * 16 * 16;
            b.v4[0] = wgv3_tr(bp);
            b.v4[1] = wgv3_tr(bp + 64);
            if (BIAS && do_bias)
                accb = __builtin_amdgcn_mfma_f32_32x32x16_bf16(
                    ones, b.v8, accb, 0, 0, 0);
            #pragma unroll
            for (int r = 0; r < 3; ++r) {
                #pragma unroll
                for (int s = 0; s < 3; ++s) {
                    const int off = (r - 1) * 10 + (s - 1);
                    GFRAG a;
                    const ushort* ap = Xr + xb + abase_w
                                     + (kq * 16 + off) * 16;
                    a.v4[0] = wgv3_tr(ap);
                    a.v4[1] = wgv3_tr(ap + 64);
                    acc[r * 3 + s] = __builtin_amdgcn_mfma_f32_32x32x16_bf16(
                        a.v8, b.v8, acc[r * 3 + s], 0, 0, 0);
                }
            }
        }
    }
    asm volatile("s_waitcnt vmcnt(0)" ::: "memory");

    const long tileC = (long)nci * 64 * nco * 64;
    const int l31 = lane & 31;
    const int half = lane >> 5;
    const int co = wj * 32 + l31;
    #pragma unroll
    for (int tap = 0; tap < 9; ++tap) {
        float* slot = WS + ((long)blockIdx.z * 9 + tap) * tileC
                    + (long)ci0 * (nco * 64) + co0 + co;
        #pragma unroll
        for (int reg = 0; reg < 16; ++reg) {
            const int ci = wi * 32 + (reg & 3) + 8 * (reg >> 2) + 4 * half;
            slot[(long)ci * (nco * 64)] = acc[tap][reg];
        }
    }
    if (BIAS && do_bias && half == 0)
        WSB[(long)blockIdx.z * (nco * 64) + co0 + co] = accb[0];
}

long conv2d_wgrad_w8_plan(int B, int H, int W, int Ci, int Co, int nci, int nco) {
    if (H != 8 || W != 8) return 0;
    if (Ci % 64 || Co % 64) return 0;
    return wgv3_split(512, nci, nco, B);
}

void conv2d_wgrad_w8_launch(const void* x, const void* dy, float* ws,
                            float* wsb, int B, int H, int W, int Ci, int Co,
                            int nci, int nco, long splitm, hipStream_t stream) {
    FD_FLUSH_STALE();
    constexpr int LOOK = 1;
    const long NIMG = B;
    const long ipb = (NIMG + splitm - 1) / splitm;
    constexpr size_t smem = (size_t)(LOOK + 1) * 4 * (W8_NPX + W8_NPY) * 16
                          * sizeof(ushort);
    dim3 grid((unsigned)(nci * nco), 1, (unsigned)splitm);
    wgv3_launch_fold<conv2d_wgrad_w8_kernel<LOOK, false>,
                     conv2d_wgrad_w8_kernel<LOOK, true>>(
        wsb != nullptr, grid, smem, stream, (const ushort*)x,
        (const ushort*)dy, ws, wsb, Ci, Co, nci, nco, NIMG, ipb);
}
```

### flaxdiff_amd/ops/hip/gemm_bf16.hip

```cpp
#include <torch/extension.h>
#include <ATen/hip/HIPContext.h>
#include "common.h"
#include "host_util.h"

typedef __bf16 bf16v8m __attribute__((ext_vector_type(8)));
typedef __attribute__((__vector_size__(4 * sizeof(__bf16)))) __bf16 bf16x4m;

#define GM_NTH 256
#define GM_BK 64

union MBF8 { bf16v8m v; ushort u[8]; uint4 q; ushort4 h4[2]; };

__device__ __forceinline__ void gm_glds16(const ushort* src, ushort* dst) {
    __builtin_amdgcn_global_load_lds(
        (const __attribute__((address_space(1))) void*)src,
        (__attribute__((address_space(3))) void*)dst, 16, 0, 0);
}

__device__ __forceinline__ bf16x4m gm_tr(const ushort* p) {
    return __builtin_amdgcn_ds_read_tr16_b64_v4bf16(
        (__attribute__((address_space(3))) bf16x4m*)p);
}

template <bool BT, int BMT, int BNT, int LOOK>
__global__ __launch_bounds__(GM_NTH, 2)
void gemm_bf16_kernel(const ushort* __restrict__ X,
                      const ushort* __restrict__ W,
                      const float* __restrict__ bias,
                      const ushort* __restrict__ addp,
                      ushort* __restrict__ Y,
                      const long M, const int N, const int K,
                      const long mt_lo_stride) {
    constexpr int WMW = BMT / 64;
    constexpr int XTILE = BMT * GM_BK;
    constexpr int KP = (BNT == 128) ? 68 : 64;
    constexpr int WTILE = BT ? (BNT * GM_BK) : ((BNT / 16) * KP * 16);
    constexpr int DBUF = LOOK + 1;
    constexpr int NGX = BMT / 32;
    constexpr int NGW = BNT / 32;
    constexpr int NG = NGX + NGW;

    extern __shared__ __attribute__((aligned(16))) ushort gmlds[];
    ushort* Xr = gmlds;
    ushort* Wr = gmlds + DBUF * XTILE;

    const int tid = threadIdx.x;
    const int lane = tid & 63;
    const int wid = tid >> 6;
    const int wn = wid / WMW;
    const int wm = wid % WMW;
    const int half = lane >> 5;
    const int l31 = lane & 31;
    const int n_base = blockIdx.y * BNT;
    const int ksl = K / GM_BK;

    const long mt0 = (long)blockIdx.x * mt_lo_stride;
    const long mtiles = (M + BMT - 1) / BMT;
    const long mt1 = (mt0 + mt_lo_stride < mtiles) ? mt0 + mt_lo_stride : mtiles;
    const int nsteps = (int)(mt1 - mt0) * ksl;
    if (nsteps <= 0) return;

    auto issue = [&](int f) {
        const int fc = f >= nsteps ? nsteps - 1 : f;
        const long mb = (mt0 + fc / ksl) * BMT;
        const int k0 = (fc % ksl) * GM_BK;
        const int buf = fc % DBUF;
        ushort* xd = Xr + buf * XTILE;
        #pragma unroll
        for (int i = 0; i < NGX; ++i) {
            const int row0 = (wid + i * 4) * 8;
            const int r8 = lane >> 3;
            long m = mb + row0 + r8;
            m = m < M ? m : M - 1;
            const int key = (row0 + r8) & 7;
            gm_glds16(X + m * K + k0 + (((lane & 7) ^ key) << 3),
                      xd + row0 * GM_BK);
        }
        ushort* wd = Wr + buf * WTILE;
        if (BT) {
            #pragma unroll
            for (int i = 0; i < NGW; ++i) {
                const int row0 = (wid + i * 4) * 8;
                const int r8 = lane >> 3;
                int n = n_base + row0 + r8;
                n = n < N ? n : N - 1;
                const int key = (row0 + r8) & 7;
                gm_glds16(W + (long)n * K + k0 + (((lane & 7) ^ key) << 3),
                          wd + row0 * GM_BK);
            }
        } else {
            #pragma unroll
            for (int i = 0; i < NGW; ++i) {
                const int pi = wid + i * 4;
                const int p = pi >> 1;
                const int kr0 = (pi & 1) * 32;
                int nc = n_base + p * 16 + (lane & 1) * 8;
                if (nc + 8 > N) nc = N - 8;
                gm_glds16(W + (long)(k0 + kr0 + (lane >> 1)) * N + nc,
                          wd + p * KP * 16 + kr0 * 16);
            }
        }
    };

    #pragma unroll
    for (int l = 0; l < LOOK; ++l) issue(l);

    const int ltr = ((lane >> 4) & 1) * KP * 16 + ((lane >> 5) << 3) * 16
                  + (lane & 15) * 4;

    constexpr int NFN = 2;
    f32x16 acc[NFN][2] = {};

    long cur_mt = mt0;
    for (int f = 0; f < nsteps; ++f) {
        asm volatile("s_waitcnt vmcnt(%0)" :: "i"((LOOK - 1) * NG) : "memory");
        __builtin_amdgcn_s_barrier();
        issue(f + LOOK);
        const int buf = f % DBUF;
        const ushort* Xb = Xr + buf * XTILE;
        const ushort* Wb = Wr + buf * WTILE;

        #pragma unroll
        for (int kk = 0; kk < GM_BK / 16; ++kk) {
            const int k0 = kk * 16 + half * 8;
            const int ch = k0 >> 3;
            MBF8 a0, a1;
            if (BT) {
                const int ar0 = wn * 64 + l31;
                a0 = *reinterpret_cast<const MBF8*>(
                    Wb + ar0 * GM_BK + ((ch ^ (ar0 & 7)) << 3));
                if (NFN == 2) {
                    const int ar1 = ar0 + 32;
                    a1 = *reinterpret_cast<const MBF8*>(
                        Wb + ar1 * GM_BK + ((ch ^ (ar1 & 7)) << 3));
                }
            } else {
                const ushort* ap = Wb + wn * 4 * KP * 16 + ltr + kk * 16 * 16;
                bf16x4m t0 = gm_tr(ap), t1 = gm_tr(ap + 64);
                a0.h4[0] = *reinterpret_cast<ushort4*>(&t0);
                a0.h4[1] = *reinterpret_cast<ushort4*>(&t1);
                if (NFN == 2) {
                    const ushort* ap2 = ap + 2 * KP * 16;
                    bf16x4m t2 = gm_tr(ap2), t3 = gm_tr(ap2 + 64);
                    a1.h4[0] = *reinterpret_cast<ushort4*>(&t2);
                    a1.h4[1] = *reinterpret_cast<ushort4*>(&t3);
                }
            }
            const int br0 = wm * 64 + l31;
            const int br1 = br0 + 32;
            const bf16v8m b0 = reinterpret_cast<const MBF8*>(
                Xb + br0 * GM_BK + ((ch ^ (br0 & 7)) << 3))->v;
            const bf16v8m b1 = reinterpret_cast<const MBF8*>(
                Xb + br1 * GM_BK + ((ch ^ (br1 & 7)) << 3))->v;
            acc[0][0] = __builtin_amdgcn_mfma_f32_32x32x16_bf16(a0.v, b0, acc[0][0], 0, 0, 0);
            acc[0][1] = __builtin_amdgcn_mfma_f32_32x32x16_bf16(a0.v, b1, acc[0][1], 0, 0, 0);
            if (NFN == 2) {
                acc[1][0] = __builtin_amdgcn_mfma_f32_32x32x16_bf16(a1.v, b0, acc[1][0], 0, 0, 0);
                acc[1][1] = __builtin_amdgcn_mfma_f32_32x32x16_bf16(a1.v, b1, acc[1][1], 0, 0, 0);
            }
        }

        if ((f % ksl) == ksl - 1) {
            const long m_base = cur_mt * BMT;
            #pragma unroll
            for (int fm = 0; fm < 2; ++fm) {
                const long m = m_base + wm * 64 + fm * 32 + l31;
                if (m < M) {
                    ushort* yrow = Y + m * N;
                    #pragma unroll
                    for (int fn = 0; fn < NFN; ++fn) {
                        #pragma unroll
                        for (int qq = 0; qq < 4; ++qq) {
                            const int n0 = n_base + wn * 64 + fn * 32 + qq * 8
                                         + half * 4;
                            if (n0 >= N) continue;
                            float v0 = acc[fn][fm][qq * 4 + 0];
                            float v1 = acc[fn][fm][qq * 4 + 1];
                            float v2 = acc[fn][fm][qq * 4 + 2];
                            float v3 = acc[fn][fm][qq * 4 + 3];
                            if (bias) {
                                v0 += bias[n0];
                                v1 += (n0 + 1 < N) ? bias[n0 + 1] : 0.f;
                                v2 += (n0 + 2 < N) ? bias[n0 + 2] : 0.f;
                                v3 += (n0 + 3 < N) ? bias[n0 + 3] : 0.f;
                            }
                            if (addp && n0 + 4 <= N) {
                                const ushort4 av = *reinterpret_cast<
                                    const ushort4*>(addp + m * N + n0);
                                v0 += bf2f(av.x); v1 += bf2f(av.y);
                                v2 += bf2f(av.z); v3 += bf2f(av.w);
                            } else if (addp) {
                                for (int j = 0; j < 4 && n0 + j < N; ++j) {
                                    const float av = bf2f(addp[m * N + n0 + j]);
                                    if (j == 0) v0 += av;
                                    else if (j == 1) v1 += av;
                                    else if (j == 2) v2 += av;
                                    else v3 += av;
                                }
                            }
                            if (n0 + 4 <= N) {
                                ushort4 pk;
                                pk.x = f2bf(v0); pk.y = f2bf(v1);
                                pk.z = f2bf(v2); pk.w = f2bf(v3);
                                *reinterpret_cast<ushort4*>(yrow + n0) = pk;
                            } else {
                                const float vs[4] = {v0, v1, v2, v3};
                                for (int j = 0; j < 4 && n0 + j < N; ++j)
                                    yrow[n0 + j] = f2bf(vs[j]);
                            }
                        }
                    }
                }
            }
            #pragma unroll
            for (int a = 0; a < NFN; ++a) {
                acc[a][0] = (f32x16){};
                acc[a][1] = (f32x16){};
            }
            ++cur_mt;
        }
    }
    asm volatile("s_waitcnt vmcnt(0)" ::: "memory");
}

torch::Tensor gemm_fwd(torch::Tensor x, torch::Tensor w, torch::Tensor bias) {
    FD_FLUSH_STALE();
    TORCH_CHECK(x.is_cuda() && x.is_contiguous() && w.is_contiguous());
    TORCH_CHECK(x.scalar_type() == at::kBFloat16 && w.scalar_type() == at::kBFloat16);
    const long M = x.size(0);
    const int K = x.size(1), N = w.size(1);
    TORCH_CHECK(w.size(0) == K && K % GM_BK == 0);
    auto y = torch::empty({M, (long)N}, x.options());
    const float* bias_ptr = nullptr;
    torch::Tensor bias_f;
    if (bias.defined() && bias.numel()) {
        bias_f = bias.to(at::kFloat).contiguous();
        bias_ptr = bias_f.data_ptr<float>();
    }
    const int bmt = (N <= 64) ? 256 : 128;
    const int bnt = 128 * 128 / bmt;
    const long mtiles = (M + bmt - 1) / bmt;
    const int ntiles = (N + bnt - 1) / bnt;
    long bm = std::max<long>(1, std::min<long>(mtiles, 768 / std::max(1, ntiles)));
    const long tpb = (mtiles + bm - 1) / bm;
    bm = (mtiles + tpb - 1) / tpb;
    auto stream = at::hip::getCurrentHIPStream();
    dim3 grid((unsigned)bm, (unsigned)ntiles);
    if (bmt == 256) {
        constexpr size_t smem = 2 * (256 * 64 + 4 * 64 * 16) * sizeof(ushort);
        fd_launch_lds<gemm_bf16_kernel<false, 256, 64, 1>>(grid, dim3(GM_NTH), smem, stream,
                           (const ushort*)x.data_ptr(), (const ushort*)w.data_ptr(),
                           bias_ptr, nullptr, (ushort*)y.data_ptr(), M, N, K, tpb);
    } else {
        constexpr size_t smem = 2 * (128 * 64 + 8 * 68 * 16) * sizeof(ushort);
        fd_launch_lds<gemm_bf16_kernel<false, 128, 128, 1>>(grid, dim3(GM_NTH), smem, stream,
                           (const ushort*)x.data_ptr(), (const ushort*)w.data_ptr(),
                           bias_ptr, nullptr, (ushort*)y.data_ptr(), M, N, K, tpb);
    }
    FD_CHECK_LAUNCH();
    return y;
}

torch::Tensor gemm_dx(torch::Tensor dy, torch::Tensor w) {
    FD_FLUSH_STALE();
    TORCH_CHECK(dy.is_cuda() && dy.is_contiguous() && w.is_contiguous());
    const long M = dy.size(0);
    const int N = dy.size(1), K = w.size(0);
    TORCH_CHECK(w.size(1) == N && N % GM_BK == 0);
    auto dx = torch::empty({M, (long)K}, dy.options());
    const int bmt = (K <= 64) ? 256 : 128;
    const int bnt = 128 * 128 / bmt;
    const long mtiles = (M + bmt - 1) / bmt;
    const int ntiles = (K + bnt - 1) / bnt;
    long bm = std::max<long>(1, std::min<long>(mtiles, 768 / std::max(1, ntiles)));
    const long tpb = (mtiles + bm - 1) / bm;
    bm = (mtiles + tpb - 1) / tpb;
    auto stream = at::hip::getCurrentHIPStream();
    dim3 grid((unsigned)bm, (unsigned)ntiles);
    if (bmt == 256) {
        constexpr size_t smem = 2 * (256 * 64 + 64 * 64) * sizeof(ushort);
        fd_launch_lds<gemm_bf16_kernel<true, 256, 64, 1>>(grid, dim3(GM_NTH), smem, stream,
                           (const ushort*)dy.data_ptr(), (const ushort*)w.data_ptr(),
                           nullptr, nullptr, (ushort*)dx.data_ptr(), M, K, N, tpb);
    } else {
        constexpr size_t smem = 2 * (128 * 64 + 128 * 64) * sizeof(ushort);
        fd_launch_lds<gemm_bf16_kernel<true, 128, 128, 1>>(grid, dim3(GM_NTH), smem, stream,
                           (const ushort*)dy.data_ptr(), (const ushort*)w.data_ptr(),
                           nullptr, nullptr, (ushort*)dx.data_ptr(), M, K, N, tpb);
    }
    FD_CHECK_LAUNCH();
    return dx;
}

torch::Tensor gemm_nt(torch::Tensor x, torch::Tensor wt, torch::Tensor bias,
                      torch::Tensor addt) {
    FD_FLUSH_STALE();
    TORCH_CHECK(x.is_cuda() && x.is_contiguous() && wt.is_contiguous());
    const long M = x.size(0);
    const int K = x.size(1), N = wt.size(0);
    TORCH_CHECK(wt.size(1) == K && K % GM_BK == 0);
    auto y = torch::empty({M, (long)N}, x.options());
    const float* bias_ptr = nullptr;
    torch::Tensor bias_f;
    if (bias.defined() && bias.numel()) {
        bias_f = bias.to(at::kFloat).contiguous();
        bias_ptr = bias_f.data_ptr<float>();
    }
    const ushort* add_ptr = nullptr;
    if (addt.defined() && addt.numel()) {
        TORCH_CHECK(addt.is_contiguous() && addt.numel() == M * N &&
                    addt.scalar_type() == at::kBFloat16,
                    "gemm_nt add tensor must be bf16 [M, N]");
        add_ptr = (const ushort*)addt.data_ptr();
    }
    const int bmt = (N <= 64) ? 256 : 128;
    const int bnt = 128 * 128 / bmt;
    const long mtiles = (M + bmt - 1) / bmt;
    const int ntiles = (N + bnt - 1) / bnt;
    long bm = std::max<long>(1, std::min<long>(mtiles, 768 / std::max(1, ntiles)));
    const long tpb = (mtiles + bm - 1) / bm;
    bm = (mtiles + tpb - 1) / tpb;
    auto stream = at::hip::getCurrentHIPStream();
    dim3 grid((unsigned)bm, (unsigned)ntiles);
    if (bmt == 256) {
        constexpr size_t smem = 2 * (256 * 64 + 64 * 64) * sizeof(ushort);
        fd_launch_lds<gemm_bf16_kernel<true, 256, 64, 1>>(grid, dim3(GM_NTH), smem, stream,
                           (const ushort*)x.data_ptr(), (const ushort*)wt.data_ptr(),
                           bias_ptr, add_ptr, (ushort*)y.data_ptr(), M, N, K, tpb);
    } else {
        constexpr size_t smem = 2 * (128 * 64 + 128 * 64) * sizeof(ushort);
        fd_launch_lds<gemm_bf16_kernel<true, 128, 128, 1>>(grid, dim3(GM_NTH), smem, stream,
                           (const ushort*)x.data_ptr(), (const ushort*)wt.data_ptr(),
                           bias_ptr, add_ptr, (ushort*)y.data_ptr(), M, N, K, tpb);
    }
    FD_CHECK_LAUNCH();
    return y;
}

__global__ void transpose_shadows_kernel(const ushort* __restrict__ src_base,
                                         ushort* __restrict__ dst_base,
                                         const int* __restrict__ tiles,
                                         const int ntiles2) {
    __shared__ ushort tsm[64][65];
    for (int t = blockIdx.x; t < ntiles2; t += gridDim.x) {
        const int* rec = tiles + (long)t * 4;
        const long soff = (unsigned)rec[0];
        const long doff = (unsigned)rec[1];
        const int N = rec[2];
        const int K = rec[3];
        const int lane = threadIdx.x & 63;
        const int w = threadIdx.x >> 6;
        __syncthreads();
        #pragma unroll
        for (int r = 0; r < 16; ++r) {
            const int row = w * 16 + r;
            tsm[row][lane] = src_base[soff + (long)row * N + lane];
        }
        __syncthreads();
        #pragma unroll
        for (int r = 0; r < 16; ++r) {
            const int row = w * 16 + r;
            dst_base[doff + (long)row * K + lane] = tsm[lane][row];
        }
    }
}

void transpose_shadows(torch::Tensor src_flat, torch::Tensor dst_flat,
                       torch::Tensor tiles) {
    FD_FLUSH_STALE();
    TORCH_CHECK(src_flat.is_cuda() && tiles.scalar_type() == at::kInt);
    const int n = tiles.size(0);
    if (!n) return;
    auto stream = at::hip::getCurrentHIPStream();
    const int blocks = std::min(n, 2048);
    hipLaunchKernelGGL(transpose_shadows_kernel, dim3(blocks), dim3(256), 0,
                       stream, (const ushort*)src_flat.data_ptr(),
                       (ushort*)dst_flat.data_ptr(), tiles.data_ptr<int>(), n);
    FD_CHECK_LAUNCH();
}
```

### flaxdiff_amd/ops/hip/gn_silu.hip

```cpp
#include <torch/extension.h>
#include <ATen/hip/HIPContext.h>
#include "common.h"
#include "host_util.h"

template <typename T, bool SILU>
__global__ void gn_silu_fwd_kernel(const T* __restrict__ x,
                                   const float* __restrict__ gamma,
                                   const float* __restrict__ beta,
                                   T* __restrict__ y,
                                   float* __restrict__ mean_out,
                                   float* __restrict__ rstd_out,
                                   int S, int C, int G, float eps) {
    const int b = blockIdx.x / G;
    const int g = blockIdx.x % G;
    const int Cg = C / G;
    const long base = (long)b * S * C + (long)g * Cg;
    const long n = (long)S * Cg;

    __shared__ float scratch[4];

    float s1 = 0.f, s2 = 0.f;
    for (long i = threadIdx.x; i < n; i += blockDim.x) {
        const int s = i / Cg, c = i % Cg;
        const float v = ElemIO<T>::ld(x + base + (long)s * C + c);
        s1 += v; s2 += v * v;
    }
    s1 = block_reduce_sum<256>(s1, scratch);
    s2 = block_reduce_sum<256>(s2, scratch);
    const float mean = s1 / n;
    const float var = fmaxf(s2 / n - mean * mean, 0.f);
    const float rstd = rsqrtf(var + eps);
    if (threadIdx.x == 0) {
        mean_out[blockIdx.x] = mean;
        rstd_out[blockIdx.x] = rstd;
    }

    for (long i = threadIdx.x; i < n; i += blockDim.x) {
        const int s = i / Cg, c = i % Cg;
        const long idx = base + (long)s * C + c;
        const float xn = (ElemIO<T>::ld(x + idx) - mean) * rstd;
        float z = xn * gamma[g * Cg + c] + beta[g * Cg + c];
        if (SILU) z = z / (1.f + expf(-z));
        ElemIO<T>::st(y + idx, z);
    }
}

template <typename T, bool SILU, bool HAS_ADD>
__global__ void gn_silu_bwd_kernel(const T* __restrict__ dy,
                                   const T* __restrict__ x,
                                   const float* __restrict__ gamma,
                                   const float* __restrict__ beta,
                                   const float* __restrict__ mean_in,
                                   const float* __restrict__ rstd_in,
                                   T* __restrict__ dx,
                                   float* __restrict__ dgamma,
                                   float* __restrict__ dbeta,
                                   const T* __restrict__ add,
                                   int S, int C, int G) {
    const int b = blockIdx.x / G;
    const int g = blockIdx.x % G;
    const int Cg = C / G;
    const long base = (long)b * S * C + (long)g * Cg;
    const long n = (long)S * Cg;
    const float mean = mean_in[blockIdx.x];
    const float rstd = rstd_in[blockIdx.x];

    extern __shared__ __attribute__((aligned(16))) char smem_raw[];
    float* dg_loc = reinterpret_cast<float*>(smem_raw);
    float* db_loc = dg_loc + Cg;
    float* scratch = db_loc + Cg;
    for (int c = threadIdx.x; c < Cg; c += blockDim.x) {
        dg_loc[c] = 0.f; db_loc[c] = 0.f;
    }
    __syncthreads();

    const int nsub = blockDim.x / Cg;
    const bool active = threadIdx.x < nsub * Cg;
    const int c = threadIdx.x % Cg;
    const int s0 = threadIdx.x / Cg;
    const float gam = gamma[g * Cg + c];
    const float bet = SILU ? beta[g * Cg + c] : 0.f;

    float s1 = 0.f, s2 = 0.f, dg_p = 0.f, db_p = 0.f;
    if (active) {
        for (int s = s0; s < S; s += nsub) {
            const long idx = base + (long)s * C + c;
            const float xn = (ElemIO<T>::ld(x + idx) - mean) * rstd;
            float dz = ElemIO<T>::ld(dy + idx);
            if (SILU) {
                const float z = xn * gam + bet;
                const float sig = 1.f / (1.f + expf(-z));
                dz *= sig * (1.f + z * (1.f - sig));
            }
            dg_p += dz * xn;
            db_p += dz;
            const float dzg = dz * gam;
            s1 += dzg;
            s2 += dzg * xn;
        }
    }
    s1 = block_reduce_sum<256>(s1, scratch);
    s2 = block_reduce_sum<256>(s2, scratch);
    const float inv_n = 1.f / n;

    if (active) {
        for (int s = s0; s < S; s += nsub) {
            const long idx = base + (long)s * C + c;
            const float xn = (ElemIO<T>::ld(x + idx) - mean) * rstd;
            float dz = ElemIO<T>::ld(dy + idx);
            if (SILU) {
                const float z = xn * gam + bet;
                const float sig = 1.f / (1.f + expf(-z));
                dz *= sig * (1.f + z * (1.f - sig));
            }
            float dxv = rstd * (dz * gam - (s1 + xn * s2) * inv_n);
            if (HAS_ADD) dxv += ElemIO<T>::ld(add + idx);
            ElemIO<T>::st(dx + idx, dxv);
        }
        atomicAdd(dg_loc + c, dg_p);
        atomicAdd(db_loc + c, db_p);
    }

    __syncthreads();
    for (int cc = threadIdx.x; cc < Cg; cc += blockDim.x) {
        atomicAdd(dgamma + g * Cg + cc, dg_loc[cc]);
        atomicAdd(dbeta + g * Cg + cc, db_loc[cc]);
    }
}

union GNV8 { uint4 q; ushort u[8]; };


#define GN3_NTH 256

template <bool SILU>
__global__ void gn3_fwd_stats_kernel(const ushort* __restrict__ x,
                                     float* __restrict__ sums,
                                     const int S, const int C, const int G,
                                     const int Cg, const int chunk_rows,
                                     const FastDiv fdCg) {
    extern __shared__ float sm[];
    const int b = blockIdx.x;
    const int s0 = blockIdx.y * chunk_rows;
    const int s1lim = min(s0 + chunk_rows, S);
    const int tpr = C >> 3;
    const int nsub = GN3_NTH / tpr;
    const bool active = (int)threadIdx.x < nsub * tpr && nsub > 0;
    const int c8 = (threadIdx.x % tpr) * 8;
    const int srow = threadIdx.x / tpr;
    for (int i = threadIdx.x; i < 2 * G; i += GN3_NTH) sm[i] = 0.f;
    __syncthreads();

    float a1 = 0.f, a2 = 0.f;
    if (active) {
        for (int s = s0 + srow; s < s1lim; s += nsub) {
            GNV8 pk;
            pk.q = *reinterpret_cast<const uint4*>(
                x + ((long)b * S + s) * C + c8);
            #pragma unroll
            for (int j = 0; j < 8; ++j) {
                const float v = bf2f(pk.u[j]);
                a1 += v; a2 += v * v;
            }
        }
        const int g = (int)fd_div((unsigned)c8, fdCg);
        atomicAdd(sm + g * 2 + 0, a1);
        atomicAdd(sm + g * 2 + 1, a2);
    }
    __syncthreads();
    for (int i = threadIdx.x; i < 2 * G; i += GN3_NTH)
        if (sm[i] != 0.f) atomicAdd(sums + (long)b * 2 * G + i, sm[i]);
}

template <bool SILU>
__global__ void gn3_fwd_apply_kernel(const ushort* __restrict__ x,
                                     const float* __restrict__ sums,
                                     const float* __restrict__ gamma,
                                     const float* __restrict__ beta,
                                     ushort* __restrict__ y,
                                     float* __restrict__ mean_out,
                                     float* __restrict__ rstd_out,
                                     const int S, const int C, const int G,
                                     const int Cg, const int chunk_rows,
                                     const float eps, const FastDiv fdCg) {
    extern __shared__ float sm[];
    float* mr = sm;
    float* gam = sm + 2 * G;
    float* bet = gam + C;
    const int b = blockIdx.x;
    const int s0 = blockIdx.y * chunk_rows;
    const int s1lim = min(s0 + chunk_rows, S);
    const long base = ((long)b * S + s0) * C;
    const long n = (long)(s1lim - s0) * C;
    const float inv_n = 1.f / ((long)S * Cg);
    for (int g = threadIdx.x; g < G; g += GN3_NTH) {
        const float m = sums[(long)b * 2 * G + g * 2 + 0] * inv_n;
        const float var = fmaxf(sums[(long)b * 2 * G + g * 2 + 1] * inv_n - m * m, 0.f);
        mr[g * 2 + 0] = m;
        mr[g * 2 + 1] = rsqrtf(var + eps);
        if (blockIdx.y == 0) {
            mean_out[(long)b * G + g] = m;
            rstd_out[(long)b * G + g] = mr[g * 2 + 1];
        }
    }
    for (int c = threadIdx.x; c < C; c += GN3_NTH) {
        gam[c] = gamma[c];
        bet[c] = beta[c];
    }
    __syncthreads();

    unsigned cc = (unsigned)((threadIdx.x * 8) % C);
    const unsigned cstep = (unsigned)((GN3_NTH * 8) % C);
    for (long i = (long)threadIdx.x * 8; i < n; i += GN3_NTH * 8) {
        const unsigned c0 = cc;
        cc += cstep; if (cc >= (unsigned)C) cc -= C;
        const int g = (int)fd_div(c0, fdCg);
        const float m = mr[g * 2 + 0], r = mr[g * 2 + 1];
        GNV8 pk, out;
        pk.q = *reinterpret_cast<const uint4*>(x + base + i);
        #pragma unroll
        for (int j = 0; j < 8; ++j) {
            float z = (bf2f(pk.u[j]) - m) * r * gam[c0 + j] + bet[c0 + j];
            if (SILU) z = z / (1.f + __expf(-z));
            out.u[j] = f2bf(z);
        }
        *reinterpret_cast<uint4*>(y + base + i) = out.q;
    }
}

template <bool SILU>
__global__ void gn3_bwd_stats_kernel(const ushort* __restrict__ dy,
                                     const ushort* __restrict__ x,
                                     const float* __restrict__ gamma,
                                     const float* __restrict__ beta,
                                     const float* __restrict__ mean_in,
                                     const float* __restrict__ rstd_in,
                                     float* __restrict__ gsums,
                                     float* __restrict__ dgamma,
                                     float* __restrict__ dbeta,
                                     const int S, const int C, const int G,
                                     const int Cg, const int chunk_rows,
                                     const FastDiv fdCg) {
    extern __shared__ float sm[];
    float* ss = sm;
    float* dgl = ss + 2 * G;
    float* dbl = dgl + C;
    const int b = blockIdx.x;
    const int s0 = blockIdx.y * chunk_rows;
    const int s1lim = min(s0 + chunk_rows, S);
    const int tpr = C >> 3;
    const int nsub = GN3_NTH / tpr;
    const bool active = (int)threadIdx.x < nsub * tpr && nsub > 0;
    const int c8 = (threadIdx.x % tpr) * 8;
    const int srow = threadIdx.x / tpr;
    for (int i = threadIdx.x; i < 2 * G; i += GN3_NTH) ss[i] = 0.f;
    for (int c = threadIdx.x; c < C; c += GN3_NTH) { dgl[c] = 0.f; dbl[c] = 0.f; }
    __syncthreads();

    if (active) {
        const int g = (int)fd_div((unsigned)c8, fdCg);
        const float m = mean_in[(long)b * G + g];
        const float r = rstd_in[(long)b * G + g];
        float g8[8], b8[8], dg8[8] = {}, db8[8] = {};
        #pragma unroll
        for (int j = 0; j < 8; ++j) {
            g8[j] = gamma[c8 + j];
            b8[j] = SILU ? beta[c8 + j] : 0.f;
        }
        float a1 = 0.f, a2 = 0.f;
        for (int s = s0 + srow; s < s1lim; s += nsub) {
            const long idx = ((long)b * S + s) * C + c8;
            GNV8 xv, dv;
            xv.q = *reinterpret_cast<const uint4*>(x + idx);
            dv.q = *reinterpret_cast<const uint4*>(dy + idx);
            #pragma unroll
            for (int j = 0; j < 8; ++j) {
                const float xn = (bf2f(xv.u[j]) - m) * r;
                float dz = bf2f(dv.u[j]);
                if (SILU) {
                    const float z = xn * g8[j] + b8[j];
                    const float sig = 1.f / (1.f + __expf(-z));
                    dz *= sig * (1.f + z * (1.f - sig));
                }
                dg8[j] += dz * xn;
                db8[j] += dz;
                const float dzg = dz * g8[j];
                a1 += dzg;
                a2 += dzg * xn;
            }
        }
        atomicAdd(ss + g * 2 + 0, a1);
        atomicAdd(ss + g * 2 + 1, a2);
        #pragma unroll
        for (int j = 0; j < 8; ++j) {
            atomicAdd(dgl + c8 + j, dg8[j]);
            atomicAdd(dbl + c8 + j, db8[j]);
        }
    }
    __syncthreads();
    for (int i = threadIdx.x; i < 2 * G; i += GN3_NTH)
        if (ss[i] != 0.f) atomicAdd(gsums + (long)b * 2 * G + i, ss[i]);
    for (int c = threadIdx.x; c < C; c += GN3_NTH) {
        if (dgl[c] != 0.f) atomicAdd(dgamma + c, dgl[c]);
        if (dbl[c] != 0.f) atomicAdd(dbeta + c, dbl[c]);
    }
}

template <bool SILU, bool HAS_ADD>
__global__ void gn3_bwd_apply_kernel(const ushort* __restrict__ dy,
                                     const ushort* __restrict__ x,
                                     const float* __restrict__ gamma,
                                     const float* __restrict__ beta,
                                     const float* __restrict__ mean_in,
                                     const float* __restrict__ rstd_in,
                                     const float* __restrict__ gsums,
                                     const ushort* __restrict__ add,
                                     ushort* __restrict__ dx,
                                     const int S, const int C, const int G,
                                     const int Cg, const int chunk_rows,
                                     const FastDiv fdCg) {
    extern __shared__ float sm[];
    float* mrs = sm;
    float* gam = sm + 4 * G;
    float* bet = gam + C;
    const int b = blockIdx.x;
    const int s0 = blockIdx.y * chunk_rows;
    const int s1lim = min(s0 + chunk_rows, S);
    const long base = ((long)b * S + s0) * C;
    const long n = (long)(s1lim - s0) * C;
    for (int g = threadIdx.x; g < G; g += GN3_NTH) {
        mrs[g * 4 + 0] = mean_in[(long)b * G + g];
        mrs[g * 4 + 1] = rstd_in[(long)b * G + g];
        mrs[g * 4 + 2] = gsums[(long)b * 2 * G + g * 2 + 0];
        mrs[g * 4 + 3] = gsums[(long)b * 2 * G + g * 2 + 1];
    }
    for (int c = threadIdx.x; c < C; c += GN3_NTH) {
        gam[c] = gamma[c];
        bet[c] = SILU ? beta[c] : 0.f;
    }
    __syncthreads();
    const float inv_n = 1.f / ((long)S * Cg);

    unsigned cc = (unsigned)((threadIdx.x * 8) % C);
    const unsigned cstep = (unsigned)((GN3_NTH * 8) % C);
    for (long i = (long)threadIdx.x * 8; i < n; i += GN3_NTH * 8) {
        const unsigned c0 = cc;
        cc += cstep; if (cc >= (unsigned)C) cc -= C;
        const int g = (int)fd_div(c0, fdCg);
        const float m = mrs[g * 4 + 0], r = mrs[g * 4 + 1];
        const float s1 = mrs[g * 4 + 2], s2 = mrs[g * 4 + 3];
        GNV8 xv, dv, av, out;
        xv.q = *reinterpret_cast<const uint4*>(x + base + i);
        dv.q = *reinterpret_cast<const uint4*>(dy + base + i);
        if (HAS_ADD) av.q = *reinterpret_cast<const uint4*>(add + base + i);
        #pragma unroll
        for (int j = 0; j < 8; ++j) {
            const float xn = (bf2f(xv.u[j]) - m) * r;
            float dz = bf2f(dv.u[j]);
            if (SILU) {
                const float z = xn * gam[c0 + j] + bet[c0 + j];
                const float sig = 1.f / (1.f + __expf(-z));
                dz *= sig * (1.f + z * (1.f - sig));
            }
            float dxv = r * (dz * gam[c0 + j] - (s1 + xn * s2) * inv_n);
            if (HAS_ADD) dxv += bf2f(av.u[j]);
            out.u[j] = f2bf(dxv);
        }
        *reinterpret_cast<uint4*>(dx + base + i) = out.q;
    }
}


std::vector<torch::Tensor> gn_silu_fwd(torch::Tensor x, torch::Tensor gamma,
                                       torch::Tensor beta, long groups,
                                       double eps, bool silu) {
    FD_FLUSH_STALE();
    TORCH_CHECK(x.is_cuda() && x.is_contiguous());
    const int B = x.size(0);
    const int C = x.size(-1);
    const long S = x.numel() / ((long)B * C);
    const int G = (int)groups;
    TORCH_CHECK(C % G == 0, "channels not divisible by groups");

    auto y = torch::empty_like(x);
    auto f32opt = x.options().dtype(at::kFloat);
    auto mean = torch::empty({(long)B * G}, f32opt);
    auto rstd = torch::empty({(long)B * G}, f32opt);
    auto gamma_f = gamma.to(at::kFloat).contiguous();
    auto beta_f = beta.to(at::kFloat).contiguous();
    auto stream = at::hip::getCurrentHIPStream();
    dim3 grid(B * G), block(256);

    const int Cg_f = C / G;
    #define LAUNCH_FWD(T, SILU_) \
        hipLaunchKernelGGL((gn_silu_fwd_kernel<T, SILU_>), grid, block, 0, stream, \
            (const T*)x.data_ptr(), gamma_f.data_ptr<float>(), beta_f.data_ptr<float>(), \
            (T*)y.data_ptr(), mean.data_ptr<float>(), rstd.data_ptr<float>(), \
            (int)S, C, G, (float)eps)
    if (x.scalar_type() == at::kBFloat16 && Cg_f % 8 == 0 && C <= 2048) {
        auto sums = torch::zeros({(long)B * 2 * G}, f32opt);
        const int chunk_rows = std::max(1, 32768 / C);
        dim3 g3(B, (S + chunk_rows - 1) / chunk_rows);
        const FastDiv fdCg = make_fastdiv(Cg_f);
        #define L_STATS(SILU_) hipLaunchKernelGGL((gn3_fwd_stats_kernel<SILU_>),             g3, dim3(GN3_NTH), 2 * G * sizeof(float), stream,             (const ushort*)x.data_ptr(), sums.data_ptr<float>(),             (int)S, C, G, Cg_f, chunk_rows, fdCg)
        #define L_APPLY(SILU_) hipLaunchKernelGGL((gn3_fwd_apply_kernel<SILU_>),             g3, dim3(GN3_NTH), (2 * G + 2 * C) * sizeof(float), stream,             (const ushort*)x.data_ptr(), sums.data_ptr<float>(),             gamma_f.data_ptr<float>(), beta_f.data_ptr<float>(),             (ushort*)y.data_ptr(), mean.data_ptr<float>(), rstd.data_ptr<float>(),             (int)S, C, G, Cg_f, chunk_rows, (float)eps, fdCg)
        if (silu) { L_STATS(true); L_APPLY(true); }
        else { L_STATS(false); L_APPLY(false); }
        #undef L_STATS
        #undef L_APPLY
    } else if (x.scalar_type() == at::kBFloat16) {
        if (silu) LAUNCH_FWD(ushort, true); else LAUNCH_FWD(ushort, false);
    } else {
        if (silu) LAUNCH_FWD(float, true); else LAUNCH_FWD(float, false);
    }
    #undef LAUNCH_FWD
    FD_CHECK_LAUNCH();
    return {y, mean, rstd};
}

std::vector<torch::Tensor> gn_silu_bwd(torch::Tensor dy, torch::Tensor x,
                                       torch::Tensor gamma, torch::Tensor beta,
                                       torch::Tensor mean, torch::Tensor rstd,
                                       long groups, bool silu,
                                       c10::optional<torch::Tensor> dgamma_sink,
                                       c10::optional<torch::Tensor> dbeta_sink,
                                       c10::optional<torch::Tensor> add) {
    FD_FLUSH_STALE();
    const int B = x.size(0);
    const int C = x.size(-1);
    const long S = x.numel() / ((long)B * C);
    const int G = (int)groups;
    const int Cg = C / G;
    TORCH_CHECK(Cg <= 256, "gn_silu_bwd: channels-per-group > 256 unsupported");

    const bool has_sink = fd_has(dgamma_sink);
    TORCH_CHECK(has_sink == fd_has(dbeta_sink),
                "gn_silu_bwd: pass both dgamma and dbeta sinks or neither");
    fd_check_sink(dgamma_sink, C, x, "gn_silu_bwd: dgamma");
    fd_check_sink(dbeta_sink, C, x, "gn_silu_bwd: dbeta");

    const bool has_add = fd_has(add);
    if (has_add)
        TORCH_CHECK(add->is_cuda() && add->device() == x.device() &&
                    add->is_contiguous() && add->sizes() == x.sizes() &&
                    add->scalar_type() == x.scalar_type(),
                    "gn_silu_bwd: add must be a contiguous tensor of x's "
                    "shape, dtype and device");
    const void* add_p = has_add ? add->data_ptr() : nullptr;

    auto dx = torch::empty_like(x);
    auto f32opt = x.options().dtype(at::kFloat);
    const long ngs = 2L * x.size(0) * G;
    auto zflat = torch::zeros({(has_sink ? 0L : 2L * C) + ngs}, f32opt);
    auto dgamma = has_sink ? *dgamma_sink : zflat.narrow(0, 0, C);
    auto dbeta = has_sink ? *dbeta_sink : zflat.narrow(0, C, C);
    auto gamma_f = gamma.to(at::kFloat).contiguous();
    auto beta_f = beta.to(at::kFloat).contiguous();
    auto stream = at::hip::getCurrentHIPStream();
    dim3 grid(B * G), block(256);
    const size_t smem = (2 * Cg + 4) * sizeof(float);

    #define LAUNCH_BWD_(T, SILU_, ADD_) \
        hipLaunchKernelGGL((gn_silu_bwd_kernel<T, SILU_, ADD_>), grid, block, smem, stream, \
            (const T*)dy.data_ptr(), (const T*)x.data_ptr(), gamma_f.data_ptr<float>(), \
            beta_f.data_ptr<float>(), mean.data_ptr<float>(), rstd.data_ptr<float>(), \
            (T*)dx.data_ptr(), dgamma.data_ptr<float>(), dbeta.data_ptr<float>(), \
            (const T*)add_p, (int)S, C, G)
    #define LAUNCH_BWD(T, SILU_) \
        do { if (has_add) LAUNCH_BWD_(T, SILU_, true); \
             else LAUNCH_BWD_(T, SILU_, false); } while (0)
    if (x.scalar_type() == at::kBFloat16 && Cg % 8 == 0 && C <= 2048) {
        auto gsums = zflat.narrow(0, has_sink ? 0L : 2L * C, ngs);
        static const long btarget = std::getenv("FD_GN_BLOCKS")
            ? atol(std::getenv("FD_GN_BLOCKS")) : 768L;
        const long bwant = std::max(1L, btarget / std::max(1, B));
        const int chunk_rows = std::max((int)((S + bwant - 1) / bwant),
                                        std::max(1, 32768 / C));
        dim3 g3(B, ((int)S + chunk_rows - 1) / chunk_rows);
        const FastDiv fdCg = make_fastdiv(Cg);
        #define L_BSTATS(SILU_) hipLaunchKernelGGL((gn3_bwd_stats_kernel<SILU_>),             g3, dim3(GN3_NTH), (4 * G + 4 * C) * sizeof(float), stream,             (const ushort*)dy.data_ptr(), (const ushort*)x.data_ptr(),             gamma_f.data_ptr<float>(), beta_f.data_ptr<float>(),             mean.data_ptr<float>(), rstd.data_ptr<float>(),             gsums.data_ptr<float>(), dgamma.data_ptr<float>(), dbeta.data_ptr<float>(),             (int)S, C, G, Cg, chunk_rows, fdCg)
        #define L_BAPPLY(SILU_, ADD_) hipLaunchKernelGGL((gn3_bwd_apply_kernel<SILU_, ADD_>),             g3, dim3(GN3_NTH), (4 * G + 2 * C) * sizeof(float), stream,             (const ushort*)dy.data_ptr(), (const ushort*)x.data_ptr(),             gamma_f.data_ptr<float>(), beta_f.data_ptr<float>(),             mean.data_ptr<float>(), rstd.data_ptr<float>(),             gsums.data_ptr<float>(), (const ushort*)add_p, (ushort*)dx.data_ptr(),             (int)S, C, G, Cg, chunk_rows, fdCg)
        if (silu) {
            L_BSTATS(true);
            if (has_add) L_BAPPLY(true, true); else L_BAPPLY(true, false);
        } else {
            L_BSTATS(false);
            if (has_add) L_BAPPLY(false, true); else L_BAPPLY(false, false);
        }
        #undef L_BSTATS
        #undef L_BAPPLY
    } else if (x.scalar_type() == at::kBFloat16) {
        if (silu) LAUNCH_BWD(ushort, true); else LAUNCH_BWD(ushort, false);
    } else {
        if (silu) LAUNCH_BWD(float, true); else LAUNCH_BWD(float, false);
    }
    #undef LAUNCH_BWD
    #undef LAUNCH_BWD_
    FD_CHECK_LAUNCH();
    if (has_sink) return {dx};
    return {dx, dgamma.to(gamma.scalar_type()), dbeta.to(gamma.scalar_type())};
}
```

Baseline: 5426 images/s.

## Fuse skip concat into GroupNorm and residual 1x1 projection via virtual cat

Decoder residual blocks now receive the skip tensor separately, and the GroupNorm+SiLU and the 1x1 residual projection read the two inputs as one virtual concatenation instead of materializing a channel cat. The backward kernels (GN bwd, dense wgrad) are extended with dual-input pointers, and the upsample conv wgrad now reads the low-resolution input directly instead of materializing the 2x upsample. This removes concat and upsample copy traffic in both passes, at the cost of more kernel variants and fallback paths when shapes are not eligible.

```diff
diff --git a/flaxdiff_amd/models/common.py b/flaxdiff_amd/models/common.py
--- a/flaxdiff_amd/models/common.py
+++ b/flaxdiff_amd/models/common.py
@@ -314,9 +314,30 @@
             return norm(x, silu=True)
         return self.activation(norm(x))
 
+    def _virtual_cat_ok(self, x, skip) -> bool:
+        rc = self.residual_conv
+        return isinstance(self.norm1, GroupNorm) and isinstance(rc, Conv) \
+            and rc.stride == 1 and ops.virtual_cat_eligible(
+                x, skip, self.norm1.num_groups, self.norm1.weight,
+                self.norm1.bias, rc.weight, rc.bias)
+
     def forward(self, x: torch.Tensor, temb: torch.Tensor,
-                textemb: torch.Tensor = None, extra_features: torch.Tensor = None):
-        if isinstance(self.norm1, GroupNorm):
+                textemb: torch.Tensor = None, extra_features: torch.Tensor = None,
+                skip: torch.Tensor = None):
+        residual_done = False
+        if skip is not None and not self._virtual_cat_ok(x, skip):
+            x = ops.cat_channels(x, skip)
+            skip = None
+        if skip is not None:
+            rc = self.residual_conv
+            out, residual = ops.group_norm_cat_dense(
+                x, skip, self.norm1.num_groups, self.norm1.weight,
+                self.norm1.bias, self.norm1.eps, self._fused_silu,
+                rc.weight, rc.bias)
+            residual_done = True
+            if not self._fused_silu:
+                out = self.activation(out)
+        elif isinstance(self.norm1, GroupNorm):
             out, residual = self.norm1.forward_fork(x, silu=self._fused_silu)
             if not self._fused_silu:
                 out = self.activation(out)
@@ -330,7 +351,7 @@
             out = self.conv1(out) + t[:, None, None, :]
 
         out = self._norm_act(self.norm2, out)
-        if self.residual_conv is not None:
+        if self.residual_conv is not None and not residual_done:
             residual = self.residual_conv(residual)
         if isinstance(self.conv2, Conv) and residual.shape[-1] == self.features:
             out = self.conv2(out, add=residual)
diff --git a/flaxdiff_amd/models/unet.py b/flaxdiff_amd/models/unet.py
--- a/flaxdiff_amd/models/unet.py
+++ b/flaxdiff_amd/models/unet.py
@@ -161,16 +161,14 @@
 
         for level in self.up_blocks:
             for res, attn in zip(level["res"], level["attn"]):
-                x = ops.cat_channels(x, downs.pop())
-                x = res(x, temb)
+                x = res(x, temb, skip=downs.pop())
                 if not isinstance(attn, nn.Identity):
                     x = attn(x, textcontext)
             if "up" in level:
                 x = level["up"](x)
 
         x = self.conv_mid(x)
-        x = ops.cat_channels(x, downs.pop())
-        x = self.final_residual(x, temb)
+        x = self.final_residual(x, temb, skip=downs.pop())
 
         if isinstance(self.conv_out_norm, GroupNorm):
             x = self.conv_out_norm(x, silu=True)
diff --git a/flaxdiff_amd/ops/__init__.py b/flaxdiff_amd/ops/__init__.py
--- a/flaxdiff_amd/ops/__init__.py
+++ b/flaxdiff_amd/ops/__init__.py
@@ -221,13 +221,14 @@
     ctx.w_param, ctx.b_param = w, b
 
 
-def _param_grads(ctx, ext, dy, x, kh, kw, stride):
+def _param_grads(ctx, ext, dy, x, kh, kw, stride, x_up2x=False):
     dw = db = None
     b_param = ctx.b_param if ctx.has_bias and ctx.needs_input_grad[2] \
         else None
     if ctx.needs_input_grad[1]:
         dw, db = _wgrad(ext, dy, x, kh, kw, stride,
-                        ctx.w_param, ctx.w_dtype, b_param, ctx.b_dtype)
+                        ctx.w_param, ctx.w_dtype, b_param, ctx.b_dtype,
+                        x_up2x=x_up2x)
     elif ctx.has_bias:
         db = _bias_grad(dy, b_param, ctx.b_dtype)
     return dw, db
@@ -381,8 +382,7 @@
         if ctx.needs_input_grad[0]:
             dx_up = ext.conv2d_dgrad(dy, wk, 1, H2, W2)
             dx = ext.upsample2x_bwd(dx_up)
-        x_up = ext.upsample2x_fwd(x) if ctx.needs_input_grad[1] else None
-        dw, db = _param_grads(ctx, ext, dy, x_up, 3, 3, 1)
+        dw, db = _param_grads(ctx, ext, dy, x, 3, 3, 1, x_up2x=True)
         return dx, dw, db
 
 
@@ -444,13 +444,107 @@
     return torch.cat([a, b], dim=-1)
 
 
+
+def virtual_cat_enabled() -> bool:
+    return os.environ.get("FD_VIRTUAL_CAT", "1") != "0"
+
+
+def virtual_cat_eligible(a: torch.Tensor, b: torch.Tensor, groups: int,
+                         gamma: torch.Tensor, beta: Optional[torch.Tensor],
+                         w: torch.Tensor, bias: Optional[torch.Tensor]) -> bool:
+    if not (virtual_cat_enabled() and group_norm_fork_enabled()
+            and _use_hip(a) and not _GEMM_LIB):
+        return False
+    if a.dtype != torch.bfloat16 or b.dtype != torch.bfloat16 \
+            or a.dim() != 4 or a.shape[:-1] != b.shape[:-1] or beta is None:
+        return False
+    ca, cb = a.shape[-1], b.shape[-1]
+    c = ca + cb
+    if w.dim() != 4 or w.shape[0] != 1 or w.shape[1] != 1 or w.shape[2] != c \
+            or not (_routable_param(w) and _routable_param(bias)):
+        return False
+    return ca % 64 == 0 and cb % 64 == 0 and w.shape[3] % 64 == 0 \
+        and groups > 0 and c % groups == 0 and (c // groups) % 8 == 0 \
+        and c <= 2048 and gamma.numel() == c
+
+
+class _GNCatDenseFn(torch.autograd.Function):
+
+    @staticmethod
+    def forward(ctx, a, b, gamma, beta, groups, eps, silu, w, bias):
+        ext = _require_ext()
+        ctx.set_materialize_grads(False)
+        ca, cb, n = a.shape[-1], b.shape[-1], w.shape[3]
+        h, mean, rstd = ext.gn_silu_fwd(a, gamma, beta, groups, eps, silu, b)
+        bf = bias if bias is not None else torch.Tensor()
+        if bf.numel() and bf.dtype != torch.float32:
+            bf = bf.float()
+        wt = getattr(w, "_shadow_bf16_t", None)
+        if wt is None:
+            wt = _kernel_view(w).reshape(ca + cb, n).t().contiguous()
+        r = ext.gemm_nt(a.view(-1, ca), wt, bf, torch.Tensor(), b.view(-1, cb))
+        ctx.save_for_backward(a, b, gamma, mean, rstd,
+                              _kernel_view(w).reshape(ca + cb, n))
+        ctx.groups, ctx.silu = groups, silu
+        ctx.beta, ctx.gamma_param = beta, gamma
+        _save_params(ctx, w, bias)
+        return h, r.view(*a.shape[:-1], n)
+
+    @staticmethod
+    def backward(ctx, dh, dr):
+        a, b, gamma, mean, rstd, wk = ctx.saved_tensors
+        ext = _require_ext()
+        ca, cb = a.shape[-1], b.shape[-1]
+        M = a.numel() // ca
+        add = dw = dbias = None
+        if dr is not None:
+            dr2 = dr.contiguous().view(M, -1)
+            if ctx.needs_input_grad[0] or ctx.needs_input_grad[1]:
+                add = ext.gemm_dx(dr2, wk).view(*a.shape[:-1], ca + cb)
+            b_param = ctx.b_param if ctx.has_bias and ctx.needs_input_grad[8] \
+                else None
+            if ctx.needs_input_grad[7]:
+                dw, dbias = _wgrad(ext, dr2.view(M, 1, 1, -1),
+                                   a.view(M, 1, 1, ca), 1, 1, 1,
+                                   ctx.w_param, ctx.w_dtype, b_param,
+                                   ctx.b_dtype if b_param is not None else None,
+                                   x2=b.view(M, 1, 1, cb))
+            elif b_param is not None:
+                dbias = _bias_grad(dr2, b_param, ctx.b_dtype)
+        if dh is None:
+            da = db = None
+            if add is not None:
+                da, db = ext.split2_lastdim(add, ca, cb)
+            return da, db, None, None, None, None, None, dw, dbias
+        dh = dh.contiguous()
+        if ctx.needs_input_grad[2] and ctx.needs_input_grad[3]:
+            sg, sb = _grad_sink(ctx.gamma_param, "g"), _grad_sink(ctx.beta, "g")
+            if sg is not None and sb is not None:
+                da, db = ext.gn_silu_bwd(dh, a, gamma, ctx.beta, mean, rstd,
+                                         ctx.groups, ctx.silu, sg, sb, add, b)
+                return da, db, None, None, None, None, None, dw, dbias
+        da, db, dgamma, dbeta = ext.gn_silu_bwd(
+            dh, a, gamma, ctx.beta, mean, rstd, ctx.groups, ctx.silu,
+            None, None, add, b)
+        return da, db, dgamma, dbeta, None, None, None, dw, dbias
+
+
+def group_norm_cat_dense(a: torch.Tensor, b: torch.Tensor, groups: int,
+                         gamma: torch.Tensor, beta: torch.Tensor, eps: float,
+                         silu: bool, w: torch.Tensor,
+                         bias: Optional[torch.Tensor]):
+    return _GNCatDenseFn.apply(a.contiguous(), b.contiguous(), gamma, beta,
+                               groups, eps, silu, w, bias)
+
+
 def _wgrad(ext, dy, x, kh, kw, stride, w_param, w_dtype,
-           b_param=None, b_dtype=None):
+           b_param=None, b_dtype=None, x_up2x=False, x2=None):
     want_db = b_dtype is not None
     w_sink = _grad_sink(w_param, "w") if w_dtype == torch.float32 else None
     b_sink = _grad_sink(b_param, "b") if b_dtype == torch.float32 else None
+    extra = (x_up2x, x2) if x2 is not None else (True,) if x_up2x else ()
     dw, db, folded = ext.conv2d_wgrad(dy, x, kh, kw, stride, w_sink,
-                                      want_db, b_sink)
+                                      want_db, b_sink, *extra)
     if dw is not None and w_dtype != torch.float32:
         dw = dw.to(w_dtype)
     if want_db and not folded:
diff --git a/flaxdiff_amd/ops/hip/bindings.cpp b/flaxdiff_amd/ops/hip/bindings.cpp
--- a/flaxdiff_amd/ops/hip/bindings.cpp
+++ b/flaxdiff_amd/ops/hip/bindings.cpp
@@ -4,14 +4,16 @@
 
 std::vector<torch::Tensor> gn_silu_fwd(torch::Tensor x, torch::Tensor gamma,
                                        torch::Tensor beta, long groups,
-                                       double eps, bool silu);
+                                       double eps, bool silu,
+                                       c10::optional<torch::Tensor> x_b);
 std::vector<torch::Tensor> gn_silu_bwd(torch::Tensor dy, torch::Tensor x,
                                        torch::Tensor gamma, torch::Tensor beta,
                                        torch::Tensor mean, torch::Tensor rstd,
                                        long groups, bool silu,
                                        c10::optional<torch::Tensor> dgamma_sink,
                                        c10::optional<torch::Tensor> dbeta_sink,
-                                       c10::optional<torch::Tensor> add);
+                                       c10::optional<torch::Tensor> add,
+                                       c10::optional<torch::Tensor> x_b);
 std::vector<torch::Tensor> rms_norm_fwd(torch::Tensor x, torch::Tensor gamma,
                                         double eps);
 std::vector<torch::Tensor> rms_norm_bwd(torch::Tensor dy, torch::Tensor x,
@@ -26,7 +28,8 @@
 std::tuple<torch::Tensor, torch::Tensor, bool>
 conv2d_wgrad(torch::Tensor dy, torch::Tensor x, long kh, long kw, long stride,
              c10::optional<torch::Tensor> dw_sink, bool want_db,
-             c10::optional<torch::Tensor> db_sink);
+             c10::optional<torch::Tensor> db_sink, bool x_up2x,
+             c10::optional<torch::Tensor> x2);
 torch::Tensor dwconv_fwd(torch::Tensor x, torch::Tensor w,
                          c10::optional<torch::Tensor> bias,
                          int64_t stride, int64_t dilation);
@@ -63,7 +66,7 @@
 torch::Tensor gemm_fwd(torch::Tensor x, torch::Tensor w, torch::Tensor bias);
 torch::Tensor gemm_dx(torch::Tensor dy, torch::Tensor w);
 torch::Tensor gemm_nt(torch::Tensor x, torch::Tensor wt, torch::Tensor bias,
-                      torch::Tensor add);
+                      torch::Tensor add, c10::optional<torch::Tensor> x2);
 void transpose_shadows(torch::Tensor src_flat, torch::Tensor dst_flat,
                        torch::Tensor tiles);
 void fused_adamw_ema(torch::Tensor p, torch::Tensor g, torch::Tensor m,
@@ -76,12 +79,14 @@
                      c10::optional<torch::Tensor> step_dev);
 
 PYBIND11_MODULE(TORCH_EXTENSION_NAME, m) {
-    m.def("gn_silu_fwd", &gn_silu_fwd, "fused GroupNorm+SiLU forward (NHWC)");
+    m.def("gn_silu_fwd", &gn_silu_fwd, "fused GroupNorm+SiLU forward (NHWC)",
+          py::arg("x"), py::arg("gamma"), py::arg("beta"), py::arg("groups"),
+          py::arg("eps"), py::arg("silu"), py::arg("x_b") = py::none());
     m.def("gn_silu_bwd", &gn_silu_bwd, "fused GroupNorm+SiLU backward",
           py::arg("dy"), py::arg("x"), py::arg("gamma"), py::arg("beta"),
           py::arg("mean"), py::arg("rstd"), py::arg("groups"), py::arg("silu"),
           py::arg("dgamma_sink") = py::none(), py::arg("dbeta_sink") = py::none(),
-          py::arg("add") = py::none());
+          py::arg("add") = py::none(), py::arg("x_b") = py::none());
     m.def("rms_norm_fwd", &rms_norm_fwd, "RMSNorm forward");
     m.def("rms_norm_bwd", &rms_norm_bwd, "RMSNorm backward",
           py::arg("dy"), py::arg("x"), py::arg("gamma"), py::arg("rrms"),
@@ -93,7 +98,8 @@
           "split-M NHWC conv wgrad (+ folded bias grad): (dw, db, folded)",
           py::arg("dy"), py::arg("x"), py::arg("kh"), py::arg("kw"),
           py::arg("stride"), py::arg("dw_sink") = py::none(),
-          py::arg("want_db") = false, py::arg("db_sink") = py::none());
+          py::arg("want_db") = false, py::arg("db_sink") = py::none(),
+          py::arg("x_up2x") = false, py::arg("x2") = py::none());
     m.def("dwconv_fwd", &dwconv_fwd, "3x3 depthwise NHWC conv forward");
     m.def("dwconv_dgrad", &dwconv_dgrad, "3x3 depthwise NHWC conv dgrad");
     m.def("dwconv_wgrad", &dwconv_wgrad, "3x3 depthwise NHWC conv wgrad (fp32)");
@@ -118,7 +124,9 @@
     m.def("s5_scan_bwd", &s5_scan_bwd, "S5 diagonal scan backward");
     m.def("gemm_fwd", &gemm_fwd, "MFMA bf16 GEMM y = x@w (+bias)");
     m.def("gemm_dx", &gemm_dx, "MFMA bf16 GEMM dx = dy@w^T");
-    m.def("gemm_nt", &gemm_nt, "MFMA bf16 GEMM y = x@wt^T (+bias)");
+    m.def("gemm_nt", &gemm_nt, "MFMA bf16 GEMM y = x@wt^T (+bias)",
+          py::arg("x"), py::arg("wt"), py::arg("bias"), py::arg("add"),
+          py::arg("x2") = py::none());
     m.def("transpose_shadows", &transpose_shadows,
           "batched 64x64 bf16 transpose (dense-weight shadow refresh)");
     m.def("fused_adamw_ema", &fused_adamw_ema, "fused AdamW + EMA flat step");
diff --git a/flaxdiff_amd/ops/hip/conv2d_wgrad.hip b/flaxdiff_amd/ops/hip/conv2d_wgrad.hip
--- a/flaxdiff_amd/ops/hip/conv2d_wgrad.hip
+++ b/flaxdiff_amd/ops/hip/conv2d_wgrad.hip
@@ -475,6 +475,13 @@
                         long Z, hipStream_t stream);
 Tr16Plan dense_wgrad_v3_plan, conv2d_wgrad_w8_plan, conv2d_wgrad_v3_plan;
 Tr16Launch dense_wgrad_v3_launch, conv2d_wgrad_w8_launch, conv2d_wgrad_v3_launch;
+Tr16Launch conv2d_wgrad_v3_up_launch;
+torch::Tensor upsample2x_fwd(torch::Tensor x);
+torch::Tensor cat2_lastdim(torch::Tensor a, torch::Tensor b);
+void dense_wgrad_v3_split_launch(const void* x, const void* x2, int Ca,
+                                 const void* dy, float* ws, float* wsb,
+                                 int B, int H, int W, int Ci, int Co,
+                                 int nci, int nco, long Z, hipStream_t stream);
 
 #define WG_FOLD_V3 1
 #define WG_FOLD_DENSE 2
@@ -545,12 +552,55 @@
 conv2d_wgrad(torch::Tensor dy, torch::Tensor x,
              long kh_, long kw_, long stride_,
              c10::optional<torch::Tensor> dw_sink, bool want_db,
-             c10::optional<torch::Tensor> db_sink) {
+             c10::optional<torch::Tensor> db_sink, bool x_up2x,
+             c10::optional<torch::Tensor> x2) {
     FD_FLUSH_STALE();
+    const void* x2_ptr = nullptr;
+    int x2_Ca = 0;
+    if (fd_has(x2)) {
+        TORCH_CHECK(!x_up2x && kh_ == 1 && kw_ == 1 && stride_ == 1,
+                    "conv2d_wgrad: x2 is for the 1x1 stride-1 case");
+        TORCH_CHECK(x2->is_cuda() && x2->is_contiguous() && x.is_contiguous() &&
+                    x2->scalar_type() == at::kBFloat16 && x2->dim() == x.dim() &&
+                    x2->sizes().slice(0, x.dim() - 1) ==
+                        x.sizes().slice(0, x.dim() - 1),
+                    "conv2d_wgrad: x2 must be bf16 with x's leading dims");
+        const int Ca = x.size(3), Cb = x2->size(3);
+        const bool ok = Ca % WG_TC == 0 && Cb % WG_TC == 0
+            && std::getenv("FD_WGRAD_NO_V3") == nullptr
+            && dense_wgrad_v3_plan(x.size(0), x.size(1), x.size(2), Ca + Cb,
+                                   dy.size(3), 1, 1) != 0;
+        if (ok) {
+            x2_ptr = x2->data_ptr();
+            x2_Ca = Ca;
+        } else {
+            x = cat2_lastdim(x, *x2);
+        }
+    }
     TORCH_CHECK(x.is_cuda() && x.is_contiguous() && dy.is_contiguous());
     TORCH_CHECK(x.scalar_type() == at::kBFloat16 && dy.scalar_type() == at::kBFloat16);
-    const int B = x.size(0), H = x.size(1), W = x.size(2), Ci = x.size(3);
+    if (x_up2x) {
+        TORCH_CHECK(x.dim() == 4 && dy.dim() == 4 && dy.size(0) == x.size(0)
+                    && dy.size(1) == 2 * x.size(1) && dy.size(2) == 2 * x.size(2),
+                    "conv2d_wgrad: x_up2x needs dy at twice x's height and width");
+        static const bool remap = [] {
+            const char* e = std::getenv("FD_WGRAD_UP_REMAP");
+            return !(e && atoi(e) == 0);
+        }();
+        const int uB = x.size(0), uH = dy.size(1), uW = dy.size(2);
+        const int uCi = x.size(3), uCo = dy.size(3);
+        const bool v3_ok = remap && kh_ == 3 && kw_ == 3 && stride_ == 1
+            && std::getenv("FD_WGRAD_NO_V3") == nullptr
+            && conv2d_wgrad_v3_plan(uB, uH, uW, uCi, uCo, 1, 1) != 0;
+        if (!v3_ok) {
+            x = upsample2x_fwd(x);
+            x_up2x = false;
+        }
+    }
+    const int B = x.size(0);
+    const int Ci = x.size(3) + (x2_ptr ? (int)x2->size(3) : 0);
     const int OH = dy.size(1), OW = dy.size(2), Co = dy.size(3);
+    const int H = x_up2x ? OH : (int)x.size(1), W = x_up2x ? OW : (int)x.size(2);
     const int KH = (int)kh_, KW = (int)kw_;
     TORCH_CHECK(KW <= WG_MAXKW, "conv2d_wgrad supports KW<=3, got ", KW);
     const int stride = (int)stride_;
@@ -576,16 +626,26 @@
     };
     for (const auto& f : families) {
         if (!(use_v3 && stride == 1 && f.shape_ok)) continue;
+        if (x_up2x && f.launch != conv2d_wgrad_v3_launch) continue;
+        if (x2_ptr && f.launch != dense_wgrad_v3_launch) continue;
         const long Z = f.plan(B, H, W, Ci, Co, nci, nco);
         if (Z == 0) continue;
         auto w = wgrad_alloc_ws(x, Z, taps, nci, nco,
                                 want_db && wgrad_fold_enabled(f.fold_bit));
-        f.launch(x.data_ptr(), dy.data_ptr(), w.ws, w.wsb,
-                 B, H, W, Ci, Co, nci, nco, Z, stream);
+        if (x2_ptr)
+            dense_wgrad_v3_split_launch(x.data_ptr(), x2_ptr, x2_Ca,
+                                        dy.data_ptr(), w.ws, w.wsb, B, H, W,
+                                        Ci, Co, nci, nco, Z, stream);
+        else
+            (x_up2x ? conv2d_wgrad_v3_up_launch : f.launch)(
+                     x.data_ptr(), dy.data_ptr(), w.ws, w.wsb,
+                     B, H, W, Ci, Co, nci, nco, Z, stream);
         return wgrad_reduce_into(w, Z, KH, KW, Ci, Co, nci, nco,
                                  dw_sink, db_sink, stream);
     }
 
+    TORCH_CHECK(!x_up2x && !x2_ptr,
+                "conv2d_wgrad: x_up2x / x2 reached the generic route");
     const int pt = std::max((OH - 1) * stride + KH - H, 0) / 2;
     const int pl = std::max((OW - 1) * stride + KW - W, 0) / 2;
     const long M = (long)B * OH * OW;
diff --git a/flaxdiff_amd/ops/hip/conv2d_wgrad_v3.hip b/flaxdiff_amd/ops/hip/conv2d_wgrad_v3.hip
--- a/flaxdiff_amd/ops/hip/conv2d_wgrad_v3.hip
+++ b/flaxdiff_amd/ops/hip/conv2d_wgrad_v3.hip
@@ -38,7 +38,7 @@
     return n + ((12 - (n & 7)) & 7);
 }
 
-template <int W, int RPT, int LOOK, bool BIAS>
+template <int W, int RPT, int LOOK, bool BIAS, bool UP = false>
 __global__ __launch_bounds__(WGV3_NTH, 2)
 void conv2d_wgrad_v3_kernel(
         const ushort* __restrict__ X,
@@ -92,18 +92,22 @@
     auto issue_slab = [&](long g) {
         const long gc = g < 0 ? 0 : (g >= BH ? BH - 1 : g);
         ushort* dst0 = Xr + (int)(gc % RING) * SLAB + wid * PS_X + 16;
-        const ushort* src0 = X + (gc * W) * (long)Ci + ci0 + wid * 16;
+        const ushort* src0 = X + (UP ? (gc >> 1) * (W / 2) : gc * W) * (long)Ci
+                           + ci0 + wid * 16;
+        constexpr int PSH = UP ? 1 : 0;
         if (W >= 32) {
             #pragma unroll
             for (int c = 0; c < G_X; ++c) {
-                const ushort* s = src0 + (long)(c * 32 + (lane >> 1)) * Ci
+                const ushort* s = src0
+                                + (long)((c * 32 + (lane >> 1)) >> PSH) * Ci
                                 + (lane & 1) * 8;
                 wgv3_glds16(s, dst0 + c * 32 * 16);
             }
         } else {
             #pragma unroll
             for (int c = 0; c < 2; ++c) {
-                const ushort* s = src0 + (long)(c * 8 + (lane >> 3)) * Ci
+                const ushort* s = src0
+                                + (long)((c * 8 + (lane >> 3)) >> PSH) * Ci
                                 + (lane & 7) * 2;
                 wgv3_glds4(s, dst0 + c * 8 * 16);
             }
@@ -273,7 +277,7 @@
     return wgv3_split(target, nci, nco, (long)B * H / rpt);
 }
 
-void conv2d_wgrad_v3_launch(const void* x, const void* dy, float* ws,
+static void wgv3_launch_any(bool up, const void* x, const void* dy, float* ws,
                             float* wsb, int B, int H, int W, int Ci, int Co,
                             int nci, int nco, long splitm, hipStream_t stream) {
     FD_FLUSH_STALE();
@@ -283,13 +287,17 @@
     const long tiles_per_block = (ntiles + splitm - 1) / splitm;
     const long rows_per_block = tiles_per_block * rpt;
     dim3 grid((unsigned)(nci * nco), 1, (unsigned)splitm);
+    #define WGV3_LAUNCH(W_, RPT_, LOOK_, UP_)                                 \
+        wgv3_launch_fold<                                                     \
+            conv2d_wgrad_v3_kernel<W_, RPT_, LOOK_, false, UP_>,              \
+            conv2d_wgrad_v3_kernel<W_, RPT_, LOOK_, true, UP_>>(              \
+            wsb != nullptr, grid, wgv3_smem<W_, RPT_, LOOK_>(), stream,       \
+            (const ushort*)x, (const ushort*)dy, ws, wsb,                     \
+            H, Ci, Co, nci, nco, BH, rows_per_block)
     #define WGV3_CASE(W_, RPT_, LOOK_)                                        \
         case W_:                                                              \
-            wgv3_launch_fold<conv2d_wgrad_v3_kernel<W_, RPT_, LOOK_, false>,  \
-                             conv2d_wgrad_v3_kernel<W_, RPT_, LOOK_, true>>(  \
-                wsb != nullptr, grid, wgv3_smem<W_, RPT_, LOOK_>(), stream,   \
-                (const ushort*)x, (const ushort*)dy, ws, wsb,                 \
-                H, Ci, Co, nci, nco, BH, rows_per_block);                     \
+            if (up) WGV3_LAUNCH(W_, RPT_, LOOK_, true);                       \
+            else WGV3_LAUNCH(W_, RPT_, LOOK_, false);                         \
             break
     switch (W) {
         WGV3_CASE(16, 4, 2);
@@ -298,10 +306,26 @@
         WGV3_CASE(128, 1, 1);
     }
     #undef WGV3_CASE
-}
-
-
-template <int LOOK, bool BIAS>
+    #undef WGV3_LAUNCH
+}
+
+void conv2d_wgrad_v3_launch(const void* x, const void* dy, float* ws,
+                            float* wsb, int B, int H, int W, int Ci, int Co,
+                            int nci, int nco, long splitm, hipStream_t stream) {
+    wgv3_launch_any(false, x, dy, ws, wsb, B, H, W, Ci, Co, nci, nco, splitm,
+                    stream);
+}
+
+void conv2d_wgrad_v3_up_launch(const void* x, const void* dy, float* ws,
+                               float* wsb, int B, int H, int W, int Ci, int Co,
+                               int nci, int nco, long splitm,
+                               hipStream_t stream) {
+    wgv3_launch_any(true, x, dy, ws, wsb, B, H, W, Ci, Co, nci, nco, splitm,
+                    stream);
+}
+
+
+template <int LOOK, bool BIAS, bool XSPLIT = false>
 __global__ __launch_bounds__(WGV3_NTH, 2)
 void dense_wgrad_v3_kernel(
         const ushort* __restrict__ X,
@@ -310,7 +334,9 @@
         float* __restrict__ WSB,
         const int Ci, const int Co,
         const int nci, const int nco,
-        const long M, const long m_per_block) {
+        const long M, const long m_per_block,
+        const ushort* __restrict__ X2,
+        const int Ca) {
     constexpr int MT = 64;
     constexpr int NPOS = wgv3_npos(MT);
     constexpr int PS = NPOS * 16;
@@ -334,16 +360,24 @@
     const long m_hi = (m_lo + m_per_block < M) ? m_lo + m_per_block : M;
     const int ntiles = (int)((m_hi - m_lo) / MT);
 
+    const ushort* xsrc = X + ci0;
+    int xstride = Ci;
+    if (XSPLIT) {
+        const bool second = ci0 >= Ca;
+        xsrc = second ? X2 + (ci0 - Ca) : X + ci0;
+        xstride = second ? Ci - Ca : Ca;
+    }
+
     auto issue = [&](int t) {
         const int tc = t >= ntiles ? ntiles - 1 : t;
         const long mb = m_lo + (long)tc * MT;
         ushort* dx0 = Xr + (tc % DBUF) * TILE + wid * PS;
         ushort* dy0 = Yr + (tc % DBUF) * TILE + wid * PS;
-        const ushort* sx = X + mb * Ci + ci0 + wid * 16;
+        const ushort* sx = xsrc + mb * xstride + wid * 16;
         const ushort* sy = dY + mb * Co + co0 + wid * 16;
         #pragma unroll
         for (int c = 0; c < 2; ++c) {
-            wgv3_glds16(sx + (long)(c * 32 + (lane >> 1)) * Ci + (lane & 1) * 8,
+            wgv3_glds16(sx + (long)(c * 32 + (lane >> 1)) * xstride + (lane & 1) * 8,
                         dx0 + c * 32 * 16);
             wgv3_glds16(sy + (long)(c * 32 + (lane >> 1)) * Co + (lane & 1) * 8,
                         dy0 + c * 32 * 16);
@@ -406,9 +440,11 @@
     return wgv3_split(1024, nci, nco, M / 64);
 }
 
-void dense_wgrad_v3_launch(const void* x, const void* dy, float* ws,
-                           float* wsb, int B, int H, int W, int Ci, int Co,
-                           int nci, int nco, long splitm, hipStream_t stream) {
+void dense_wgrad_v3_split_launch(const void* x, const void* x2, int Ca,
+                                 const void* dy, float* ws, float* wsb,
+                                 int B, int H, int W, int Ci, int Co,
+                                 int nci, int nco, long splitm,
+                                 hipStream_t stream) {
     FD_FLUSH_STALE();
     constexpr int LOOK = 2;
     const long M = (long)B * H * W;
@@ -418,10 +454,25 @@
     constexpr size_t smem = (size_t)2 * (LOOK + 2) * 4 * wgv3_npos(64) * 16
                           * sizeof(ushort);
     dim3 grid((unsigned)(nci * nco), 1, (unsigned)splitm);
-    wgv3_launch_fold<dense_wgrad_v3_kernel<LOOK, false>,
-                     dense_wgrad_v3_kernel<LOOK, true>>(
-        wsb != nullptr, grid, smem, stream, (const ushort*)x,
-        (const ushort*)dy, ws, wsb, Ci, Co, nci, nco, M, m_per_block);
+    if (x2)
+        wgv3_launch_fold<dense_wgrad_v3_kernel<LOOK, false, true>,
+                         dense_wgrad_v3_kernel<LOOK, true, true>>(
+            wsb != nullptr, grid, smem, stream, (const ushort*)x,
+            (const ushort*)dy, ws, wsb, Ci, Co, nci, nco, M, m_per_block,
+            (const ushort*)x2, Ca);
+    else
+        wgv3_launch_fold<dense_wgrad_v3_kernel<LOOK, false>,
+                         dense_wgrad_v3_kernel<LOOK, true>>(
+            wsb != nullptr, grid, smem, stream, (const ushort*)x,
+            (const ushort*)dy, ws, wsb, Ci, Co, nci, nco, M, m_per_block,
+            (const ushort*)nullptr, 0);
+}
+
+void dense_wgrad_v3_launch(const void* x, const void* dy, float* ws,
+                           float* wsb, int B, int H, int W, int Ci, int Co,
+                           int nci, int nco, long splitm, hipStream_t stream) {
+    dense_wgrad_v3_split_launch(x, nullptr, 0, dy, ws, wsb, B, H, W, Ci, Co,
+                                nci, nco, splitm, stream);
 }
 
 
diff --git a/flaxdiff_amd/ops/hip/gemm_bf16.hip b/flaxdiff_amd/ops/hip/gemm_bf16.hip
--- a/flaxdiff_amd/ops/hip/gemm_bf16.hip
+++ b/flaxdiff_amd/ops/hip/gemm_bf16.hip
@@ -22,7 +22,7 @@
         (__attribute__((address_space(3))) bf16x4m*)p);
 }
 
-template <bool BT, int BMT, int BNT, int LOOK>
+template <bool BT, int BMT, int BNT, int LOOK, bool XSPLIT = false>
 __global__ __launch_bounds__(GM_NTH, 2)
 void gemm_bf16_kernel(const ushort* __restrict__ X,
                       const ushort* __restrict__ W,
@@ -30,7 +30,9 @@
                       const ushort* __restrict__ addp,
                       ushort* __restrict__ Y,
                       const long M, const int N, const int K,
-                      const long mt_lo_stride) {
+                      const long mt_lo_stride,
+                      const ushort* __restrict__ X2,
+                      const int Ka) {
     constexpr int WMW = BMT / 64;
     constexpr int XTILE = BMT * GM_BK;
     constexpr int KP = (BNT == 128) ? 68 : 64;
@@ -66,6 +68,13 @@
         const int k0 = (fc % ksl) * GM_BK;
         const int buf = fc % DBUF;
         ushort* xd = Xr + buf * XTILE;
+        const ushort* xs = X + k0;
+        int xstride = K;
+        if (XSPLIT) {
+            const bool second = k0 >= Ka;
+            xs = second ? X2 + (k0 - Ka) : X + k0;
+            xstride = second ? K - Ka : Ka;
+        }
         #pragma unroll
         for (int i = 0; i < NGX; ++i) {
             const int row0 = (wid + i * 4) * 8;
@@ -73,7 +82,7 @@
             long m = mb + row0 + r8;
             m = m < M ? m : M - 1;
             const int key = (row0 + r8) & 7;
-            gm_glds16(X + m * K + k0 + (((lane & 7) ^ key) << 3),
+            gm_glds16(xs + m * xstride + (((lane & 7) ^ key) << 3),
                       xd + row0 * GM_BK);
         }
         ushort* wd = Wr + buf * WTILE;
@@ -250,12 +259,14 @@
         constexpr size_t smem = 2 * (256 * 64 + 4 * 64 * 16) * sizeof(ushort);
         fd_launch_lds<gemm_bf16_kernel<false, 256, 64, 1>>(grid, dim3(GM_NTH), smem, stream,
                            (const ushort*)x.data_ptr(), (const ushort*)w.data_ptr(),
-                           bias_ptr, nullptr, (ushort*)y.data_ptr(), M, N, K, tpb);
+                           bias_ptr, nullptr, (ushort*)y.data_ptr(), M, N, K, tpb,
+                           (const ushort*)nullptr, 0);
     } else {
         constexpr size_t smem = 2 * (128 * 64 + 8 * 68 * 16) * sizeof(ushort);
         fd_launch_lds<gemm_bf16_kernel<false, 128, 128, 1>>(grid, dim3(GM_NTH), smem, stream,
                            (const ushort*)x.data_ptr(), (const ushort*)w.data_ptr(),
-                           bias_ptr, nullptr, (ushort*)y.data_ptr(), M, N, K, tpb);
+                           bias_ptr, nullptr, (ushort*)y.data_ptr(), M, N, K, tpb,
+                           (const ushort*)nullptr, 0);
     }
     FD_CHECK_LAUNCH();
     return y;
@@ -281,23 +292,37 @@
         constexpr size_t smem = 2 * (256 * 64 + 64 * 64) * sizeof(ushort);
         fd_launch_lds<gemm_bf16_kernel<true, 256, 64, 1>>(grid, dim3(GM_NTH), smem, stream,
                            (const ushort*)dy.data_ptr(), (const ushort*)w.data_ptr(),
-                           nullptr, nullptr, (ushort*)dx.data_ptr(), M, K, N, tpb);
+                           nullptr, nullptr, (ushort*)dx.data_ptr(), M, K, N, tpb,
+                           (const ushort*)nullptr, 0);
     } else {
         constexpr size_t smem = 2 * (128 * 64 + 128 * 64) * sizeof(ushort);
         fd_launch_lds<gemm_bf16_kernel<true, 128, 128, 1>>(grid, dim3(GM_NTH), smem, stream,
                            (const ushort*)dy.data_ptr(), (const ushort*)w.data_ptr(),
-                           nullptr, nullptr, (ushort*)dx.data_ptr(), M, K, N, tpb);
+                           nullptr, nullptr, (ushort*)dx.data_ptr(), M, K, N, tpb,
+                           (const ushort*)nullptr, 0);
     }
     FD_CHECK_LAUNCH();
     return dx;
 }
 
 torch::Tensor gemm_nt(torch::Tensor x, torch::Tensor wt, torch::Tensor bias,
-                      torch::Tensor addt) {
+                      torch::Tensor addt, c10::optional<torch::Tensor> x2) {
     FD_FLUSH_STALE();
     TORCH_CHECK(x.is_cuda() && x.is_contiguous() && wt.is_contiguous());
     const long M = x.size(0);
-    const int K = x.size(1), N = wt.size(0);
+    const bool split = fd_has(x2);
+    const int Ka = x.size(1);
+    const ushort* x2_ptr = nullptr;
+    if (split) {
+        TORCH_CHECK(x2->is_cuda() && x2->device() == x.device() &&
+                    x2->is_contiguous() && x2->dim() == 2 && x2->size(0) == M &&
+                    x2->scalar_type() == at::kBFloat16 &&
+                    x.scalar_type() == at::kBFloat16 &&
+                    Ka % GM_BK == 0 && x2->size(1) % GM_BK == 0,
+                    "gemm_nt: x2 must be bf16 [M, Kb] with Ka, Kb % 64 == 0");
+        x2_ptr = (const ushort*)x2->data_ptr();
+    }
+    const int K = Ka + (split ? (int)x2->size(1) : 0), N = wt.size(0);
     TORCH_CHECK(wt.size(1) == K && K % GM_BK == 0);
     auto y = torch::empty({M, (long)N}, x.options());
     const float* bias_ptr = nullptr;
@@ -322,17 +347,21 @@
     bm = (mtiles + tpb - 1) / tpb;
     auto stream = at::hip::getCurrentHIPStream();
     dim3 grid((unsigned)bm, (unsigned)ntiles);
+    #define GM_NT_LAUNCH(BMT_, BNT_, SPLIT_)                                   \
+        fd_launch_lds<gemm_bf16_kernel<true, BMT_, BNT_, 1, SPLIT_>>(          \
+            grid, dim3(GM_NTH),                                                \
+            (size_t)2 * (BMT_ * 64 + BNT_ * 64) * sizeof(ushort), stream,      \
+            (const ushort*)x.data_ptr(), (const ushort*)wt.data_ptr(),         \
+            bias_ptr, add_ptr, (ushort*)y.data_ptr(), M, N, K, tpb,            \
+            x2_ptr, Ka)
     if (bmt == 256) {
-        constexpr size_t smem = 2 * (256 * 64 + 64 * 64) * sizeof(ushort);
-        fd_launch_lds<gemm_bf16_kernel<true, 256, 64, 1>>(grid, dim3(GM_NTH), smem, stream,
-                           (const ushort*)x.data_ptr(), (const ushort*)wt.data_ptr(),
-                           bias_ptr, add_ptr, (ushort*)y.data_ptr(), M, N, K, tpb);
+        if (split) GM_NT_LAUNCH(256, 64, true);
+        else GM_NT_LAUNCH(256, 64, false);
     } else {
-        constexpr size_t smem = 2 * (128 * 64 + 128 * 64) * sizeof(ushort);
-        fd_launch_lds<gemm_bf16_kernel<true, 128, 128, 1>>(grid, dim3(GM_NTH), smem, stream,
-                           (const ushort*)x.data_ptr(), (const ushort*)wt.data_ptr(),
-                           bias_ptr, add_ptr, (ushort*)y.data_ptr(), M, N, K, tpb);
-    }
+        if (split) GM_NT_LAUNCH(128, 128, true);
+        else GM_NT_LAUNCH(128, 128, false);
+    }
+    #undef GM_NT_LAUNCH
     FD_CHECK_LAUNCH();
     return y;
 }
diff --git a/flaxdiff_amd/ops/hip/gn_silu.hip b/flaxdiff_amd/ops/hip/gn_silu.hip
--- a/flaxdiff_amd/ops/hip/gn_silu.hip
+++ b/flaxdiff_amd/ops/hip/gn_silu.hip
@@ -131,14 +131,25 @@
 union GNV8 { uint4 q; ushort u[8]; };
 
 
+
 #define GN3_NTH 256
 
-template <bool SILU>
+template <bool DUAL, typename P>
+__device__ __forceinline__ P* gn3_src(P* xa, P* xb, const long row,
+                                      const int c8, const int C, const int Ca) {
+    if (DUAL)
+        return c8 < Ca ? xa + row * Ca + c8 : xb + row * (C - Ca) + (c8 - Ca);
+    return xa + row * C + c8;
+}
+
+template <bool SILU, bool DUAL = false>
 __global__ void gn3_fwd_stats_kernel(const ushort* __restrict__ x,
                                      float* __restrict__ sums,
                                      const int S, const int C, const int G,
                                      const int Cg, const int chunk_rows,
-                                     const FastDiv fdCg) {
+                                     const FastDiv fdCg,
+                                     const ushort* __restrict__ xb,
+                                     const int Ca) {
     extern __shared__ float sm[];
     const int b = blockIdx.x;
     const int s0 = blockIdx.y * chunk_rows;
@@ -156,7 +167,7 @@
         for (int s = s0 + srow; s < s1lim; s += nsub) {
             GNV8 pk;
             pk.q = *reinterpret_cast<const uint4*>(
-                x + ((long)b * S + s) * C + c8);
+                gn3_src<DUAL>(x, xb, (long)b * S + s, c8, C, Ca));
             #pragma unroll
             for (int j = 0; j < 8; ++j) {
                 const float v = bf2f(pk.u[j]);
@@ -172,7 +183,7 @@
         if (sm[i] != 0.f) atomicAdd(sums + (long)b * 2 * G + i, sm[i]);
 }
 
-template <bool SILU>
+template <bool SILU, bool DUAL = false>
 __global__ void gn3_fwd_apply_kernel(const ushort* __restrict__ x,
                                      const float* __restrict__ sums,
                                      const float* __restrict__ gamma,
@@ -182,7 +193,9 @@
                                      float* __restrict__ rstd_out,
                                      const int S, const int C, const int G,
                                      const int Cg, const int chunk_rows,
-                                     const float eps, const FastDiv fdCg) {
+                                     const float eps, const FastDiv fdCg,
+                                     const ushort* __restrict__ xb,
+                                     const int Ca) {
     extern __shared__ float sm[];
     float* mr = sm;
     float* gam = sm + 2 * G;
@@ -211,13 +224,18 @@
 
     unsigned cc = (unsigned)((threadIdx.x * 8) % C);
     const unsigned cstep = (unsigned)((GN3_NTH * 8) % C);
+    long row = (long)b * S + s0 + (threadIdx.x * 8) / C;
+    const int rstep = (GN3_NTH * 8) / C;
     for (long i = (long)threadIdx.x * 8; i < n; i += GN3_NTH * 8) {
         const unsigned c0 = cc;
+        const long row0 = row;
         cc += cstep; if (cc >= (unsigned)C) cc -= C;
+        if (DUAL) { row += rstep; if (cc < c0 + cstep) ++row; }
         const int g = (int)fd_div(c0, fdCg);
         const float m = mr[g * 2 + 0], r = mr[g * 2 + 1];
         GNV8 pk, out;
-        pk.q = *reinterpret_cast<const uint4*>(x + base + i);
+        pk.q = *reinterpret_cast<const uint4*>(
+            DUAL ? gn3_src<true>(x, xb, row0, (int)c0, C, Ca) : x + base + i);
         #pragma unroll
         for (int j = 0; j < 8; ++j) {
             float z = (bf2f(pk.u[j]) - m) * r * gam[c0 + j] + bet[c0 + j];
@@ -228,7 +246,7 @@
     }
 }
 
-template <bool SILU>
+template <bool SILU, bool DUAL = false>
 __global__ void gn3_bwd_stats_kernel(const ushort* __restrict__ dy,
                                      const ushort* __restrict__ x,
                                      const float* __restrict__ gamma,
@@ -240,7 +258,9 @@
                                      float* __restrict__ dbeta,
                                      const int S, const int C, const int G,
                                      const int Cg, const int chunk_rows,
-                                     const FastDiv fdCg) {
+                                     const FastDiv fdCg,
+                                     const ushort* __restrict__ xb,
+                                     const int Ca) {
     extern __shared__ float sm[];
     float* ss = sm;
     float* dgl = ss + 2 * G;
@@ -271,7 +291,9 @@
         for (int s = s0 + srow; s < s1lim; s += nsub) {
             const long idx = ((long)b * S + s) * C + c8;
             GNV8 xv, dv;
-            xv.q = *reinterpret_cast<const uint4*>(x + idx);
+            xv.q = *reinterpret_cast<const uint4*>(
+                DUAL ? gn3_src<true>(x, xb, (long)b * S + s, c8, C, Ca)
+                     : x + idx);
             dv.q = *reinterpret_cast<const uint4*>(dy + idx);
             #pragma unroll
             for (int j = 0; j < 8; ++j) {
@@ -306,7 +328,7 @@
     }
 }
 
-template <bool SILU, bool HAS_ADD>
+template <bool SILU, bool HAS_ADD, bool DUAL = false>
 __global__ void gn3_bwd_apply_kernel(const ushort* __restrict__ dy,
                                      const ushort* __restrict__ x,
                                      const float* __restrict__ gamma,
@@ -318,7 +340,10 @@
                                      ushort* __restrict__ dx,
                                      const int S, const int C, const int G,
                                      const int Cg, const int chunk_rows,
-                                     const FastDiv fdCg) {
+                                     const FastDiv fdCg,
+                                     const ushort* __restrict__ xb,
+                                     ushort* __restrict__ dxb,
+                                     const int Ca) {
     extern __shared__ float sm[];
     float* mrs = sm;
     float* gam = sm + 4 * G;
@@ -343,14 +368,19 @@
 
     unsigned cc = (unsigned)((threadIdx.x * 8) % C);
     const unsigned cstep = (unsigned)((GN3_NTH * 8) % C);
+    long row = (long)b * S + s0 + (threadIdx.x * 8) / C;
+    const int rstep = (GN3_NTH * 8) / C;
     for (long i = (long)threadIdx.x * 8; i < n; i += GN3_NTH * 8) {
         const unsigned c0 = cc;
+        const long row0 = row;
         cc += cstep; if (cc >= (unsigned)C) cc -= C;
+        if (DUAL) { row += rstep; if (cc < c0 + cstep) ++row; }
         const int g = (int)fd_div(c0, fdCg);
         const float m = mrs[g * 4 + 0], r = mrs[g * 4 + 1];
         const float s1 = mrs[g * 4 + 2], s2 = mrs[g * 4 + 3];
         GNV8 xv, dv, av, out;
-        xv.q = *reinterpret_cast<const uint4*>(x + base + i);
+        xv.q = *reinterpret_cast<const uint4*>(
+            DUAL ? gn3_src<true>(x, xb, row0, (int)c0, C, Ca) : x + base + i);
         dv.q = *reinterpret_cast<const uint4*>(dy + base + i);
         if (HAS_ADD) av.q = *reinterpret_cast<const uint4*>(add + base + i);
         #pragma unroll
@@ -366,23 +396,53 @@
             if (HAS_ADD) dxv += bf2f(av.u[j]);
             out.u[j] = f2bf(dxv);
         }
-        *reinterpret_cast<uint4*>(dx + base + i) = out.q;
-    }
-}
-
+        *reinterpret_cast<uint4*>(
+            DUAL ? gn3_src<true>(dx, dxb, row0, (int)c0, C, Ca)
+                 : dx + base + i) = out.q;
+    }
+}
+
+
+static int gn_dual_check(const torch::Tensor& x,
+                         const c10::optional<torch::Tensor>& x_b, long groups,
+                         const char* who) {
+    if (!fd_has(x_b)) return 0;
+    const int Ca = x.size(-1), Cb = x_b->size(-1);
+    const int C = Ca + Cb;
+    TORCH_CHECK(x_b->is_cuda() && x_b->device() == x.device() &&
+                x_b->is_contiguous() && x.is_contiguous() &&
+                x_b->dim() == x.dim() &&
+                x_b->sizes().slice(0, x.dim() - 1) ==
+                    x.sizes().slice(0, x.dim() - 1),
+                who, ": x_b must be contiguous with x's leading dims");
+    TORCH_CHECK(x.scalar_type() == at::kBFloat16 &&
+                x_b->scalar_type() == at::kBFloat16 && Ca % 8 == 0 &&
+                Cb % 8 == 0 && C % groups == 0 && (C / groups) % 8 == 0 &&
+                C <= 2048,
+                who, ": two-source GroupNorm needs bf16, Ca and Cb multiples "
+                "of 8, channels per group a multiple of 8 and C <= 2048");
+    return Cb;
+}
 
 std::vector<torch::Tensor> gn_silu_fwd(torch::Tensor x, torch::Tensor gamma,
                                        torch::Tensor beta, long groups,
-                                       double eps, bool silu) {
+                                       double eps, bool silu,
+                                       c10::optional<torch::Tensor> x_b) {
     FD_FLUSH_STALE();
     TORCH_CHECK(x.is_cuda() && x.is_contiguous());
+    const int Cb = gn_dual_check(x, x_b, groups, "gn_silu_fwd");
+    const bool dual = Cb > 0;
+    const int Ca = x.size(-1);
+    const ushort* xb_p = dual ? (const ushort*)x_b->data_ptr() : nullptr;
     const int B = x.size(0);
-    const int C = x.size(-1);
-    const long S = x.numel() / ((long)B * C);
+    const int C = Ca + Cb;
+    const long S = x.numel() / ((long)B * Ca);
     const int G = (int)groups;
     TORCH_CHECK(C % G == 0, "channels not divisible by groups");
 
-    auto y = torch::empty_like(x);
+    auto ysizes = x.sizes().vec();
+    ysizes.back() = C;
+    auto y = torch::empty(ysizes, x.options());
     auto f32opt = x.options().dtype(at::kFloat);
     auto mean = torch::empty({(long)B * G}, f32opt);
     auto rstd = torch::empty({(long)B * G}, f32opt);
@@ -402,10 +462,26 @@
         const int chunk_rows = std::max(1, 32768 / C);
         dim3 g3(B, (S + chunk_rows - 1) / chunk_rows);
         const FastDiv fdCg = make_fastdiv(Cg_f);
-        #define L_STATS(SILU_) hipLaunchKernelGGL((gn3_fwd_stats_kernel<SILU_>),             g3, dim3(GN3_NTH), 2 * G * sizeof(float), stream,             (const ushort*)x.data_ptr(), sums.data_ptr<float>(),             (int)S, C, G, Cg_f, chunk_rows, fdCg)
-        #define L_APPLY(SILU_) hipLaunchKernelGGL((gn3_fwd_apply_kernel<SILU_>),             g3, dim3(GN3_NTH), (2 * G + 2 * C) * sizeof(float), stream,             (const ushort*)x.data_ptr(), sums.data_ptr<float>(),             gamma_f.data_ptr<float>(), beta_f.data_ptr<float>(),             (ushort*)y.data_ptr(), mean.data_ptr<float>(), rstd.data_ptr<float>(),             (int)S, C, G, Cg_f, chunk_rows, (float)eps, fdCg)
-        if (silu) { L_STATS(true); L_APPLY(true); }
-        else { L_STATS(false); L_APPLY(false); }
+        #define L_STATS(SILU_, DUAL_)                                          \
+            hipLaunchKernelGGL((gn3_fwd_stats_kernel<SILU_, DUAL_>),           \
+                g3, dim3(GN3_NTH), 2 * G * sizeof(float), stream,              \
+                (const ushort*)x.data_ptr(), sums.data_ptr<float>(),           \
+                (int)S, C, G, Cg_f, chunk_rows, fdCg, xb_p, Ca)
+        #define L_APPLY(SILU_, DUAL_)                                          \
+            hipLaunchKernelGGL((gn3_fwd_apply_kernel<SILU_, DUAL_>),           \
+                g3, dim3(GN3_NTH), (2 * G + 2 * C) * sizeof(float), stream,    \
+                (const ushort*)x.data_ptr(), sums.data_ptr<float>(),           \
+                gamma_f.data_ptr<float>(), beta_f.data_ptr<float>(),           \
+                (ushort*)y.data_ptr(), mean.data_ptr<float>(),                 \
+                rstd.data_ptr<float>(), (int)S, C, G, Cg_f, chunk_rows,        \
+                (float)eps, fdCg, xb_p, Ca)
+        if (dual) {
+            if (silu) { L_STATS(true, true); L_APPLY(true, true); }
+            else { L_STATS(false, true); L_APPLY(false, true); }
+        } else {
+            if (silu) { L_STATS(true, false); L_APPLY(true, false); }
+            else { L_STATS(false, false); L_APPLY(false, false); }
+        }
         #undef L_STATS
         #undef L_APPLY
     } else if (x.scalar_type() == at::kBFloat16) {
@@ -424,12 +500,20 @@
                                        long groups, bool silu,
                                        c10::optional<torch::Tensor> dgamma_sink,
                                        c10::optional<torch::Tensor> dbeta_sink,
-                                       c10::optional<torch::Tensor> add) {
+                                       c10::optional<torch::Tensor> add,
+                                       c10::optional<torch::Tensor> x_b) {
     FD_FLUSH_STALE();
+    const int Cb = gn_dual_check(x, x_b, groups, "gn_silu_bwd");
+    const bool dual = Cb > 0;
+    const int Ca = x.size(-1);
+    const ushort* xb_p = dual ? (const ushort*)x_b->data_ptr() : nullptr;
     const int B = x.size(0);
-    const int C = x.size(-1);
-    const long S = x.numel() / ((long)B * C);
+    const int C = Ca + Cb;
+    const long S = x.numel() / ((long)B * Ca);
     const int G = (int)groups;
+    TORCH_CHECK(dy.is_contiguous() && dy.numel() == (long)B * S * C &&
+                dy.scalar_type() == x.scalar_type(),
+                "gn_silu_bwd: dy must be contiguous [.., C] of x's dtype");
     const int Cg = C / G;
     TORCH_CHECK(Cg <= 256, "gn_silu_bwd: channels-per-group > 256 unsupported");
 
@@ -442,13 +526,16 @@
     const bool has_add = fd_has(add);
     if (has_add)
         TORCH_CHECK(add->is_cuda() && add->device() == x.device() &&
-                    add->is_contiguous() && add->sizes() == x.sizes() &&
+                    add->is_contiguous() && add->sizes() == dy.sizes() &&
                     add->scalar_type() == x.scalar_type(),
                     "gn_silu_bwd: add must be a contiguous tensor of x's "
                     "shape, dtype and device");
     const void* add_p = has_add ? add->data_ptr() : nullptr;
 
     auto dx = torch::empty_like(x);
+    torch::Tensor dxb;
+    if (dual) dxb = torch::empty_like(*x_b);
+    ushort* dxb_p = dual ? (ushort*)dxb.data_ptr() : nullptr;
     auto f32opt = x.options().dtype(at::kFloat);
     const long ngs = 2L * x.size(0) * G;
     auto zflat = torch::zeros({(has_sink ? 0L : 2L * C) + ngs}, f32opt);
@@ -478,15 +565,34 @@
                                         std::max(1, 32768 / C));
         dim3 g3(B, ((int)S + chunk_rows - 1) / chunk_rows);
         const FastDiv fdCg = make_fastdiv(Cg);
-        #define L_BSTATS(SILU_) hipLaunchKernelGGL((gn3_bwd_stats_kernel<SILU_>),             g3, dim3(GN3_NTH), (4 * G + 4 * C) * sizeof(float), stream,             (const ushort*)dy.data_ptr(), (const ushort*)x.data_ptr(),             gamma_f.data_ptr<float>(), beta_f.data_ptr<float>(),             mean.data_ptr<float>(), rstd.data_ptr<float>(),             gsums.data_ptr<float>(), dgamma.data_ptr<float>(), dbeta.data_ptr<float>(),             (int)S, C, G, Cg, chunk_rows, fdCg)
-        #define L_BAPPLY(SILU_, ADD_) hipLaunchKernelGGL((gn3_bwd_apply_kernel<SILU_, ADD_>),             g3, dim3(GN3_NTH), (4 * G + 2 * C) * sizeof(float), stream,             (const ushort*)dy.data_ptr(), (const ushort*)x.data_ptr(),             gamma_f.data_ptr<float>(), beta_f.data_ptr<float>(),             mean.data_ptr<float>(), rstd.data_ptr<float>(),             gsums.data_ptr<float>(), (const ushort*)add_p, (ushort*)dx.data_ptr(),             (int)S, C, G, Cg, chunk_rows, fdCg)
-        if (silu) {
-            L_BSTATS(true);
-            if (has_add) L_BAPPLY(true, true); else L_BAPPLY(true, false);
+        #define L_BSTATS(SILU_, DUAL_)                                         \
+            hipLaunchKernelGGL((gn3_bwd_stats_kernel<SILU_, DUAL_>),           \
+                g3, dim3(GN3_NTH), (4 * G + 4 * C) * sizeof(float), stream,    \
+                (const ushort*)dy.data_ptr(), (const ushort*)x.data_ptr(),     \
+                gamma_f.data_ptr<float>(), beta_f.data_ptr<float>(),           \
+                mean.data_ptr<float>(), rstd.data_ptr<float>(),                \
+                gsums.data_ptr<float>(), dgamma.data_ptr<float>(),             \
+                dbeta.data_ptr<float>(), (int)S, C, G, Cg, chunk_rows, fdCg,   \
+                xb_p, Ca)
+        #define L_BAPPLY(SILU_, ADD_, DUAL_)                                   \
+            hipLaunchKernelGGL((gn3_bwd_apply_kernel<SILU_, ADD_, DUAL_>),     \
+                g3, dim3(GN3_NTH), (4 * G + 2 * C) * sizeof(float), stream,    \
+                (const ushort*)dy.data_ptr(), (const ushort*)x.data_ptr(),     \
+                gamma_f.data_ptr<float>(), beta_f.data_ptr<float>(),           \
+                mean.data_ptr<float>(), rstd.data_ptr<float>(),                \
+                gsums.data_ptr<float>(), (const ushort*)add_p,                 \
+                (ushort*)dx.data_ptr(), (int)S, C, G, Cg, chunk_rows, fdCg,    \
+                xb_p, dxb_p, Ca)
+        #define L_BWD3(SILU_, DUAL_)                                           \
+            do { L_BSTATS(SILU_, DUAL_);                                       \
+                 if (has_add) L_BAPPLY(SILU_, true, DUAL_);                    \
+                 else L_BAPPLY(SILU_, false, DUAL_); } while (0)
+        if (dual) {
+            if (silu) L_BWD3(true, true); else L_BWD3(false, true);
         } else {
-            L_BSTATS(false);
-            if (has_add) L_BAPPLY(false, true); else L_BAPPLY(false, false);
-        }
+            if (silu) L_BWD3(true, false); else L_BWD3(false, false);
+        }
+        #undef L_BWD3
         #undef L_BSTATS
         #undef L_BAPPLY
     } else if (x.scalar_type() == at::kBFloat16) {
@@ -497,6 +603,10 @@
     #undef LAUNCH_BWD
     #undef LAUNCH_BWD_
     FD_CHECK_LAUNCH();
-    if (has_sink) return {dx};
-    return {dx, dgamma.to(gamma.scalar_type()), dbeta.to(gamma.scalar_type())};
-}
+    std::vector<torch::Tensor> out = {dx};
+    if (dual) out.push_back(dxb);
+    if (has_sink) return out;
+    out.push_back(dgamma.to(gamma.scalar_type()));
+    out.push_back(dbeta.to(gamma.scalar_type()));
+    return out;
+}
```

Result: faster. 5640 images/s, median of 6 (+3.9%).
